# bacpop/PopPUNK

Measured on AMD Instinct MI355X. Metric: genome-pair distances/sec (10k self, s=1024, k=13-29), higher is better.
Workload: dtype u64

## Files before the change

### include/ppk.h

```cpp
#ifndef PPK_H
#define PPK_H

#include <stddef.h>
#include <stdint.h>

#ifdef __cplusplus
extern "C" {
#endif

#define PPK_OK 0
#define PPK_ERR_ARG 1
#define PPK_ERR_HIP 2
#define PPK_ERR_CAPACITY 3
#define PPK_ERR_STATE 4
#define PPK_ERR_INTERRUPTED 5
#define PPK_REFINE_NOT_NESTED 6

#define PPK_FLAG_RANDOM_CORRECT 1
#define PPK_FLAG_JACCARD 2
#define PPK_FLAG_COUNTS 4

const char *ppk_last_error(void);
int ppk_release_scratch(void);
const char *ppk_version(void);
int ppk_device_count(int *n);

int ppk_set_option(const char *name, long long value);
int ppk_get_option(const char *name, long long *value);

int ppk_set_interrupt_check(int (*check)(void));

typedef struct ppk_db ppk_db;

int ppk_db_create(int device_id, const uint64_t *sk, size_t n, size_t nk,
                  size_t sketchsize64, size_t bbits, const uint16_t *clu,
                  int src_on_device, void *stream, ppk_db **out);
void ppk_db_destroy(ppk_db *db);
size_t ppk_db_size(const ppk_db *db);
int ppk_db_rank_planes(const ppk_db *db);
int ppk_db_rank_read(const ppk_db *db, uint64_t *out, size_t words);
int ppk_db_rank_block_planes(const ppk_db *db, uint8_t *out, size_t cap);
int ppk_db_fold_planes(const ppk_db *db);
int ppk_db_fold_block_planes(const ppk_db *db, uint8_t *out, size_t cap);
int ppk_db_fold_read(const ppk_db *db, int which, uint64_t *out, size_t words);
int ppk_db_fold2_planes(const ppk_db *db);
int ppk_db_fold2_block_planes(const ppk_db *db, uint8_t *out, size_t cap);
int ppk_db_fold2_stream_planes(const ppk_db *db, uint8_t *out, size_t cap);
int ppk_db_fold2_position_order(const ppk_db *db, uint32_t *out, size_t cap);
int ppk_db_fold2_read(const ppk_db *db, int which, uint64_t *out, size_t words);
size_t ppk_db_fold2_events(const ppk_db *db, size_t *n_buckets);
int ppk_db_fold2_events_read(const ppk_db *db, uint32_t *off, size_t n_off, uint16_t *ev, size_t n_ev);
size_t ppk_db_rank_counts(const ppk_db *db, uint32_t *out, size_t cap);
unsigned ppk_db_foldh_holders(const ppk_db *db);
int ppk_db_foldh_stream_planes(const ppk_db *db, uint8_t *out, size_t cap);
int ppk_db_foldh_position_order(const ppk_db *db, uint32_t *out, size_t cap);
int ppk_db_foldh_read(const ppk_db *db, int which, uint64_t *out, size_t words);
size_t ppk_db_foldh_entries(const ppk_db *db, size_t *n_buckets);
int ppk_db_foldh_entries_read(const ppk_db *db, uint32_t *off, size_t n_off, uint32_t *ent, size_t n_ent);

size_t ppk_rows_in_band(size_t n_ref, size_t n_qry, size_t q_begin, size_t q_end);
int ppk_band_split(size_t n_ref, size_t n_qry, int n_parts, size_t *bounds);

int ppk_dist_dev(const ppk_db *ref, const ppk_db *qry, const int32_t *kmers,
                 const float *random_tbl, size_t n_clu, int flags,
                 size_t q_begin, size_t q_end, void *d_out,
                 unsigned long long *d_n_failed, void *stream);

int ppk_dist_edges_dev(const ppk_db *ref, const ppk_db *qry, const int32_t *kmers,
                       const float *random_tbl, size_t n_clu, int flags,
                       size_t q_begin, size_t q_end, int slope, float x_max,
                       float y_max, float scale_x, float scale_y, int inclusive,
                       long long *d_edges, size_t cap,
                       unsigned long long *d_n_edges,
                       unsigned long long *d_n_failed, void *stream);

int ppk_dist_pairs_dev(const ppk_db *ref, const ppk_db *qry, const int32_t *kmers, const float *random_tbl,
                       size_t n_clu, int flags, const long long *d_i, const long long *d_j, size_t stride,
                       size_t n_pairs, long long int_offset, void *d_out, unsigned long long *d_n_failed,
                       void *stream);
int ppk_dist_pairs(const ppk_db *ref, const ppk_db *qry, const int32_t *kmers, const float *random_tbl, size_t n_clu,
                   int flags, const long long *i, const long long *j, size_t n_pairs, long long int_offset, void *out,
                   unsigned long long *n_failed);

#define PPK_WINDOW_HANDLE_BYTES 64
int ppk_window_alloc(int device, size_t bytes, void **d_window);
int ppk_window_free(int device, void *d_window);
int ppk_window_export(int device, const void *d_window, unsigned char handle[PPK_WINDOW_HANDLE_BYTES]);
int ppk_window_open(int device, const unsigned char handle[PPK_WINDOW_HANDLE_BYTES], void **d_window);
int ppk_window_close(int device, void *d_window);

int ppk_assign_threshold_dev(const float *d_dist, size_t n_rows, int slope,
                             float x_max, float y_max, float *d_out, void *stream);

int ppk_edge_threshold_dev(const float *d_dist, size_t n_rows, size_t n_ref,
                           int slope, float x_max, float y_max, int inclusive,
                           long long *d_edges, size_t cap,
                           unsigned long long *d_n_edges, void *stream);

int ppk_generate_tuples_dev(const int32_t *d_assign, size_t n_rows, int within_label,
                            int self, size_t num_ref, long long int_offset,
                            long long *d_edges, size_t cap,
                            unsigned long long *d_n_edges, void *stream);

int ppk_generate_all_tuples_dev(size_t num_ref, size_t num_queries, int self, long long int_offset,
                                long long *d_edges, size_t cap, size_t *n_edges, void *stream);

int ppk_qc_edges_dev(const float *d_dist, size_t n_rows, size_t n_ref, int mode, float max_pi,
                     float max_a, long long *d_edges, size_t cap,
                     unsigned long long *d_n_edges, void *stream);

#define PPK_BGMM_MAX_K 16
typedef struct ppk_bgmm {
  int K;
  int within_label;
  int scale_is_f64;
  int n_jitter;
  float scale_f32[2];
  double scale_f64[2];
  double mean[PPK_BGMM_MAX_K][2];
  double chol[PPK_BGMM_MAX_K][3];
  double inv_diag[PPK_BGMM_MAX_K][2];
  double log_const[PPK_BGMM_MAX_K];
  double lin[PPK_BGMM_MAX_K][5];
  int jitter[PPK_BGMM_MAX_K];
} ppk_bgmm;

int ppk_bgmm_prepare(int K, const double *weights, const double *means, const double *covariances,
                     const double *scale, int scale_is_f64, int within_label, ppk_bgmm *out);

int ppk_bgmm_assign_dev(const float *d_dist, size_t n_rows, const ppk_bgmm *model, int32_t *d_labels,
                        float *d_resp, void *stream);

int ppk_bgmm_edges_dev(const float *d_dist, size_t n_rows, size_t n_ref, const ppk_bgmm *model,
                       long long int_offset, long long *d_edges, size_t cap,
                       unsigned long long *d_n_edges, void *stream);

int ppk_dist_bgmm_edges_dev(const ppk_db *ref, const ppk_db *qry, const int32_t *kmers,
                            const float *random_tbl, size_t n_clu, int flags, size_t q_begin, size_t q_end,
                            const ppk_bgmm *model, long long *d_edges, size_t cap,
                            unsigned long long *d_n_edges, unsigned long long *d_n_failed, void *stream);

int ppk_query_bgmm_edges_dbs(const ppk_db *const *refs, const ppk_db *const *qrys, int n_dev,
                             const int32_t *kmers, const float *random_tbl, size_t n_clu, int flags,
                             const ppk_bgmm *model, long long *ij_out, size_t cap, size_t *n_edges,
                             unsigned long long *n_failed);

int ppk_bgmm_assign(const float *dist, size_t n_rows, const ppk_bgmm *model, int device_id, int32_t *labels,
                    float *resp);

#define PPK_BGMM_FIT_STATS 7
#define PPK_BGMM_FIT_MAX_ITER 1024
#define PPK_BGMM_FIT_MAX_INIT 32
#define PPK_BGMM_KMEANS_MAX_ITER 50
typedef struct ppk_bgmm_fit_params {
  int K;
  int max_iter;
  int n_init;
  int reserved;
  double weight_concentration_prior;
  double mean_precision_prior;
  double mean_prior[2];
  double degrees_of_freedom_prior;
  double reg_covar;
  double tol;
} ppk_bgmm_fit_params;
int ppk_bgmm_fit_params_default(int K, ppk_bgmm_fit_params *out);

typedef struct ppk_bgmm_state {
  int K;
  int reserved;
  double weight_conc_a[PPK_BGMM_MAX_K], weight_conc_b[PPK_BGMM_MAX_K];
  double mean_precision[PPK_BGMM_MAX_K];
  double means[PPK_BGMM_MAX_K][2];
  double dof[PPK_BGMM_MAX_K];
  double covariances[PPK_BGMM_MAX_K][4];
  double chol[PPK_BGMM_MAX_K][3];
  double weights[PPK_BGMM_MAX_K];
  double lin[PPK_BGMM_MAX_K][5];
  double log_const[PPK_BGMM_MAX_K];
} ppk_bgmm_state;

typedef struct ppk_bgmm_fit_result {
  ppk_bgmm_state state;
  int n_iter, converged;
  int best_init, n_init_run;
  unsigned long long n_train;
  double lower_bound;
  double cov_prior[4];
  double train_mean[2];
  double init_lower_bound[PPK_BGMM_FIT_MAX_INIT];
  int init_n_iter[PPK_BGMM_FIT_MAX_INIT];
  int kmeans_iter[PPK_BGMM_FIT_MAX_INIT];
  double lower_bounds[PPK_BGMM_FIT_MAX_ITER];
} ppk_bgmm_fit_result;

int ppk_bgmm_fit_struct_sizes(size_t out[3]);

double ppk_bgmm_digamma(double x);

int ppk_bgmm_mstep(const ppk_bgmm_fit_params *params, const double *stats, const double *pivot,
                   const double *cov_prior, ppk_bgmm_state *state_out, double *lower_bound_out);

int ppk_bgmm_stats_dev(const float *d_rows, size_t n_rows, const long long *d_index, size_t n_index,
                       const float *scale, const ppk_bgmm_state *state, double *d_stats, void *stream);

int ppk_bgmm_kmeans_dev(const float *d_rows, size_t n_rows, const long long *d_index, size_t n_index,
// ... 342 lines not shown
```

### poppunk_amd/_lib.py

```python
import ctypes as C
import os

_HERE = os.path.dirname(os.path.abspath(__file__))
SO_PATH = os.environ.get("PPK_LIBRARY") or os.path.join(_HERE, "csrc", "libppk_hip.so")

OK, ERR_ARG, ERR_HIP, ERR_CAPACITY, ERR_STATE, ERR_INTERRUPTED = 0, 1, 2, 3, 4, 5
REFINE_NOT_NESTED = 6
FLAG_RANDOM_CORRECT, FLAG_JACCARD, FLAG_COUNTS = 1, 2, 4
SKETCH_STRAND_PRESERVED = 1
SKETCH_EXACT = 2

_u64p, _f32p, _i32p, _u16p = (C.POINTER(C.c_uint64), C.POINTER(C.c_float), C.POINTER(C.c_int32),
                              C.POINTER(C.c_uint16))
_llp, _ullp, _szp, _intp = (C.POINTER(C.c_longlong), C.POINTER(C.c_ulonglong),
                            C.POINTER(C.c_size_t), C.POINTER(C.c_int))
_vp, _sz = C.c_void_p, C.c_size_t

BGMM_MAX_K = 16


class Bgmm(C.Structure):
    _fields_ = [("K", C.c_int), ("within_label", C.c_int), ("scale_is_f64", C.c_int), ("n_jitter", C.c_int),
                ("scale_f32", C.c_float * 2), ("scale_f64", C.c_double * 2),
                ("mean", (C.c_double * 2) * BGMM_MAX_K), ("chol", (C.c_double * 3) * BGMM_MAX_K),
                ("inv_diag", (C.c_double * 2) * BGMM_MAX_K), ("log_const", C.c_double * BGMM_MAX_K),
                ("lin", (C.c_double * 5) * BGMM_MAX_K),
                ("jitter", C.c_int * BGMM_MAX_K)]


BGMM_FIT_STATS, BGMM_FIT_MAX_ITER, BGMM_FIT_MAX_INIT, BGMM_KMEANS_MAX_ITER = 7, 1024, 32, 50


class BgmmFitParams(C.Structure):
    _fields_ = [("K", C.c_int), ("max_iter", C.c_int), ("n_init", C.c_int), ("reserved", C.c_int),
                ("weight_concentration_prior", C.c_double), ("mean_precision_prior", C.c_double),
                ("mean_prior", C.c_double * 2), ("degrees_of_freedom_prior", C.c_double), ("reg_covar", C.c_double),
                ("tol", C.c_double)]


class BgmmState(C.Structure):
    _fields_ = [("K", C.c_int), ("reserved", C.c_int),
                ("weight_conc_a", C.c_double * BGMM_MAX_K), ("weight_conc_b", C.c_double * BGMM_MAX_K),
                ("mean_precision", C.c_double * BGMM_MAX_K), ("means", (C.c_double * 2) * BGMM_MAX_K),
                ("dof", C.c_double * BGMM_MAX_K), ("covariances", (C.c_double * 4) * BGMM_MAX_K),
                ("chol", (C.c_double * 3) * BGMM_MAX_K), ("weights", C.c_double * BGMM_MAX_K),
                ("lin", (C.c_double * 5) * BGMM_MAX_K), ("log_const", C.c_double * BGMM_MAX_K)]


class BgmmFitResult(C.Structure):
    _fields_ = [("state", BgmmState), ("n_iter", C.c_int), ("converged", C.c_int), ("best_init", C.c_int),
                ("n_init_run", C.c_int), ("n_train", C.c_ulonglong), ("lower_bound", C.c_double),
                ("cov_prior", C.c_double * 4), ("train_mean", C.c_double * 2),
                ("init_lower_bound", C.c_double * BGMM_FIT_MAX_INIT), ("init_n_iter", C.c_int * BGMM_FIT_MAX_INIT),
                ("kmeans_iter", C.c_int * BGMM_FIT_MAX_INIT), ("lower_bounds", C.c_double * BGMM_FIT_MAX_ITER)]


_bgmmp, _f64p = C.POINTER(Bgmm), C.POINTER(C.c_double)
_fitpp, _statep, _fitrp = C.POINTER(BgmmFitParams), C.POINTER(BgmmState), C.POINTER(BgmmFitResult)

SIGNATURES = {
    "ppk_bgmm_prepare": (C.c_int, [C.c_int, _f64p, _f64p, _f64p, _f64p, C.c_int, C.c_int, _bgmmp]),
    "ppk_bgmm_assign_dev": (C.c_int, [_vp, _sz, _bgmmp, _vp, _vp, _vp]),
    "ppk_bgmm_edges_dev": (C.c_int, [_vp, _sz, _sz, _bgmmp, C.c_longlong, _vp, _sz, _vp, _vp]),
    "ppk_dist_bgmm_edges_dev": (C.c_int, [_vp, _vp, _i32p, _f32p, _sz, C.c_int, _sz, _sz, _bgmmp, _vp, _sz, _vp, _vp,
                                          _vp]),
    "ppk_query_bgmm_edges_dbs": (C.c_int, [C.POINTER(_vp), C.POINTER(_vp), C.c_int, _i32p, _f32p, _sz, C.c_int,
                                           _bgmmp, _llp, _sz, _szp, _ullp]),
    "ppk_bgmm_assign": (C.c_int, [_f32p, _sz, _bgmmp, C.c_int, _i32p, _f32p]),
    "ppk_bgmm_fit_params_default": (C.c_int, [C.c_int, _fitpp]),
    "ppk_bgmm_fit_struct_sizes": (C.c_int, [_szp]),
    "ppk_bgmm_digamma": (C.c_double, [C.c_double]),
    "ppk_bgmm_mstep": (C.c_int, [_fitpp, _f64p, _f64p, _f64p, _statep, _f64p]),
    "ppk_bgmm_stats_dev": (C.c_int, [_vp, _sz, _vp, _sz, _f32p, _statep, _vp, _vp]),
    "ppk_bgmm_kmeans_dev": (C.c_int, [_vp, _sz, _vp, _sz, _f32p, C.c_int, _f64p, _vp, _vp, _vp, _vp]),
    "ppk_bgmm_fit_dev": (C.c_int, [_vp, _sz, _vp, _sz, _f32p, _vp, _f64p, _fitpp, _fitrp, _vp]),
    "ppk_bgmm_fit": (C.c_int, [_f32p, _sz, _llp, _sz, _f32p, _i32p, _f64p, _fitpp, C.c_int, _fitrp]),
    "ppk_network_sweep_dev": (C.c_int, [_vp, _vp, _sz, _vp, _sz, _sz, _sz, C.c_longlong, _vp, _vp, _vp]),
    "ppk_network_sweep": (C.c_int, [_llp, _llp, _llp, _sz, _sz, _sz, C.c_int, C.c_longlong, _llp, _i32p]),
    "ppk_network_summary_dev": (C.c_int, [_vp, _vp, _sz, _vp, _sz, _sz, _sz, C.c_longlong, _vp, _vp, _vp, _vp, _vp]),
    "ppk_network_summary": (C.c_int, [_llp, _llp, _llp, _sz, _sz, _sz, C.c_int, C.c_longlong, _llp, _f64p, _llp, _f64p]),
    "ppk_cluster_sweep_dev": (C.c_int, [_vp, _vp, _sz, _vp, _sz, _sz, _sz, _vp, _vp, _vp]),
    "ppk_cluster_sweep": (C.c_int, [_llp, _llp, _llp, _sz, _sz, _sz, C.c_int, _i32p, _i32p]),
    "ppk_cluster_pair_sums_dev": (C.c_int, [_vp, _sz, C.c_int, _vp, _sz, C.c_int, _vp, _vp, _vp]),
    "ppk_cluster_pair_sums": (C.c_int, [_f32p, _sz, C.c_int, _i32p, _sz, C.c_int, C.c_int, _llp, _llp]),
    "ppk_silhouette_dev": (C.c_int, [_vp, _sz, C.c_int, _vp, _sz, C.c_int, _vp, _vp, _vp, _vp, _vp, _vp]),
    "ppk_silhouette": (C.c_int, [_f32p, _sz, C.c_int, _i32p, _sz, C.c_int, C.c_int, _f64p, _f64p, _f64p, _i32p,
                                 _i32p]),
    "ppk_contingency_sums_dev": (C.c_int, [_vp, _sz, _vp, _sz, _sz, _vp, _vp, _vp, _vp, _vp, _vp, _vp]),
    "ppk_contingency_sums": (C.c_int, [_i32p, _sz, _i32p, _sz, _sz, C.c_int, _llp, _llp, _i32p, _i32p, _llp, _llp]),
    "ppk_strain_knn_dev": (C.c_int, [_vp, _sz, C.c_int, _vp, _llp, _sz, _sz, _vp, _vp, _vp, _vp]),
    "ppk_strain_ranks_dev": (C.c_int, [_vp, _vp, _llp, _sz, _sz, _i32p, _sz, C.c_int, C.c_int, C.c_float, _vp, _vp, _vp,
                                       _vp, _vp, _sz, _szp, _vp]),
    "ppk_strain_knn": (C.c_int, [_f32p, _sz, C.c_int, _llp, _llp, _sz, _sz, C.c_int, _llp, _llp, _f32p]),
    "ppk_strain_ranks": (C.c_int, [_llp, _f32p, _llp, _sz, _sz, _i32p, _sz, C.c_int, C.c_int, C.c_float, C.c_int, _i32p,
                                   _llp, _llp, _llp, _f32p, _sz, _szp]),
    "ppk_strain_extend_dev": (C.c_int, [_vp, _llp, _vp, _llp, _sz, _vp, _vp, _vp, _vp, _sz, _sz, C.c_int, C.c_float,
                                        _sz, _vp, _vp, _vp, _vp]),
    "ppk_strain_extend": (C.c_int, [_llp, _llp, _llp, _llp, _sz, _llp, _f32p, _f32p, _f32p, _sz, _sz, C.c_int,
                                    C.c_float, _sz, C.c_int, _llp, _llp, _f32p]),
    "ppk_sketch_dev": (C.c_int, [_vp, _vp, _sz, _i32p, _sz, _sz, _sz, C.c_int, _vp, _vp, _vp, _vp]),
    "ppk_sketch": (C.c_int, [C.POINTER(C.c_uint8), _llp, _sz, _i32p, _sz, _sz, _sz, C.c_int, C.c_int, _u64p, _llp, _i32p]),
    "ppk_sketch_reads_dev": (C.c_int, [_vp, _vp, _sz, _i32p, _sz, _sz, _sz, C.c_int, C.c_int, _vp, _vp, _vp, _vp, _vp]),
    "ppk_sketch_reads": (C.c_int, [C.POINTER(C.c_uint8), _llp, _sz, _i32p, _sz, _sz, _sz, C.c_int, C.c_int, C.c_int, _u64p,
                                   _llp, _llp, _i32p]),
    "ppk_density_kde_dev": (C.c_int, [_vp, _sz, _vp, _sz, _f32p, _f64p, _sz, _f64p, _sz, C.c_double, C.c_int, _vp, _f32p,
                                      _vp]),
    "ppk_density_kde": (C.c_int, [_f32p, _sz, _llp, _sz, _f32p, _f64p, _sz, _f64p, _sz, C.c_double, C.c_int, C.c_int,
                                  _llp, _f32p]),
    "ppk_density_counts_dev": (C.c_int, [_vp, _sz, _vp, C.c_int, C.c_int, C.c_double, C.c_double, _sz, C.c_double,
                                         C.c_double, _sz, _vp, _vp, _vp]),
    "ppk_density_counts": (C.c_int, [_f32p, _sz, _i32p, C.c_int, C.c_int, C.c_double, C.c_double, _sz, C.c_double,
                                     C.c_double, _sz, C.c_int, C.POINTER(C.c_uint32), _llp]),
    "ppk_query_links_dev": (C.c_int, [_vp, _vp, _sz, _sz, _vp, _sz, _sz, C.c_int, _vp, _vp, _vp, _vp]),
    "ppk_query_links": (C.c_int, [_llp, _llp, _sz, _i32p, _sz, _sz, C.c_int, C.c_int, _i32p, _i32p, _i32p]),
    "ppk_cluster_extend_dev": (C.c_int, [_vp, _vp, _sz, _sz, _vp, _sz, _sz, _vp, _vp, _vp]),
    "ppk_cluster_extend": (C.c_int, [_llp, _llp, _sz, _i32p, _sz, _sz, C.c_int, _i32p, _i32p]),
    "ppk_mst_dev": (C.c_int, [_vp, _vp, _sz, _vp, _sz, _sz, _vp, _vp, _vp, _vp]),
    "ppk_mst": (C.c_int, [_llp, _llp, _f32p, _sz, _sz, C.c_int, _llp, _ullp, _i32p]),
    "ppk_edge_weights_dev": (C.c_int, [_vp, _sz, _vp, _vp, _sz, _sz, _sz, C.c_longlong, C.c_int, _vp, _vp]),
    "ppk_row_norms_dev": (C.c_int, [_vp, _sz, _vp, _vp]),
    "ppk_nj_dev": (C.c_int, [_vp, C.c_int, _sz, _sz, _sz, _vp, _vp, _vp]),
    "ppk_nj": (C.c_int, [_f32p, _sz, C.c_int, _llp, _f64p]),
    "ppk_embed_weights_dev": (C.c_int, [_vp, _vp, _vp, _sz, _sz, C.c_double, _vp, _vp, _vp]),
    "ppk_embed_dev": (C.c_int, [_vp, _vp, _vp, _sz, _sz, C.c_ulonglong, C.c_longlong, C.c_int, C.c_double,
                                C.c_longlong, _vp, _vp]),
    "ppk_embed": (C.c_int, [_llp, _llp, _f32p, _sz, _sz, C.c_double, C.c_ulonglong, C.c_longlong, C.c_int,
                            C.c_double, C.c_longlong, C.c_int, _f64p, _f64p]),
    "ppk_dbscan_core_dev": (C.c_int, [_vp, _sz, C.c_int, _vp, _vp]),
    "ppk_dbscan_mst_dev": (C.c_int, [_vp, _vp, _sz, _vp, _vp, _vp, _vp]),
    "ppk_dbscan_fit": (C.c_int, [_f32p, _sz, C.c_int, C.c_int, _f64p, _i32p, _i32p, _f64p]),
    "ppk_dbscan_create": (C.c_int, [_f32p, _f64p, _sz, C.c_int, _i32p, _f64p, _i32p, _f64p, _i32p, _sz, _f64p,
                                    C.c_int, C.c_int, C.c_int, C.POINTER(_vp)]),
    "ppk_dbscan_destroy": (None, [_vp]),
    "ppk_dbscan_assign_dev": (C.c_int, [_vp, _sz, _vp, _vp, _vp]),
    "ppk_dbscan_edges_dev": (C.c_int, [_vp, _sz, _sz, _vp, C.c_longlong, _vp, _sz, _vp, _vp]),
    "ppk_dbscan_assign": (C.c_int, [_f32p, _sz, _vp, _i32p]),
    "ppk_dbscan_stats": (C.c_int, [_vp, _ullp]),
    "ppk_refine_score_dev": (C.c_int, [_vp, _sz, C.c_int, C.c_float, C.c_float, _vp, _vp]),
    "ppk_refine_score": (C.c_int, [_f32p, _sz, C.c_int, C.c_float, C.c_float, C.c_int, _llp]),
    "ppk_refine_local_create_dev": (C.c_int, [_vp, _sz, C.c_int, C.c_float, C.c_float, C.c_float, C.c_float, _vp,
                                              C.POINTER(_vp)]),
    "ppk_refine_local_destroy": (None, [_vp]),
    "ppk_refine_local_stats": (C.c_int, [_vp, _ullp]),
    "ppk_refine_local_eval_dev": (C.c_int, [_vp, C.c_float, C.c_float, _vp, _vp]),
    "ppk_last_error": (C.c_char_p, []),
    "ppk_version": (C.c_char_p, []),
    "ppk_release_scratch": (C.c_int, []),
    "ppk_device_count": (C.c_int, [_intp]),
    "ppk_db_create": (C.c_int, [C.c_int, _vp, _sz, _sz, _sz, _sz, _vp, C.c_int, _vp,
                                C.POINTER(_vp)]),
    "ppk_db_destroy": (None, [_vp]),
    "ppk_db_size": (_sz, [_vp]),
    "ppk_db_rank_planes": (C.c_int, [_vp]),
    "ppk_db_rank_read": (C.c_int, [_vp, _vp, _sz]),
    "ppk_db_rank_block_planes": (C.c_int, [_vp, _vp, _sz]),
    "ppk_db_fold_planes": (C.c_int, [_vp]),
    "ppk_db_fold_block_planes": (C.c_int, [_vp, _vp, _sz]),
    "ppk_db_fold_read": (C.c_int, [_vp, C.c_int, _vp, _sz]),
    "ppk_db_fold2_planes": (C.c_int, [_vp]),
    "ppk_db_fold2_block_planes": (C.c_int, [_vp, _vp, _sz]),
    "ppk_db_fold2_stream_planes": (C.c_int, [_vp, _vp, _sz]),
    "ppk_db_fold2_position_order": (C.c_int, [_vp, _vp, _sz]),
    "ppk_db_fold2_read": (C.c_int, [_vp, C.c_int, _vp, _sz]),
    "ppk_db_fold2_events": (_sz, [_vp, C.POINTER(C.c_size_t)]),
    "ppk_db_fold2_events_read": (C.c_int, [_vp, _vp, _sz, _vp, _sz]),
    "ppk_db_rank_counts": (_sz, [_vp, _vp, _sz]),
    "ppk_db_foldh_holders": (C.c_uint, [_vp]),
    "ppk_db_foldh_stream_planes": (C.c_int, [_vp, _vp, _sz]),
    "ppk_db_foldh_position_order": (C.c_int, [_vp, _vp, _sz]),
    "ppk_db_foldh_read": (C.c_int, [_vp, C.c_int, _vp, _sz]),
    "ppk_db_foldh_entries": (_sz, [_vp, C.POINTER(C.c_size_t)]),
    "ppk_db_foldh_entries_read": (C.c_int, [_vp, _vp, _sz, _vp, _sz]),
    "ppk_rows_in_band": (_sz, [_sz, _sz, _sz, _sz]),
    "ppk_band_split": (C.c_int, [_sz, _sz, C.c_int, _szp]),
    "ppk_dist_dev": (C.c_int, [_vp, _vp, _i32p, _f32p, _sz, C.c_int, _sz, _sz, _vp, _vp, _vp]),
    "ppk_dist_pairs_dev": (C.c_int, [_vp, _vp, _i32p, _f32p, _sz, C.c_int, _vp, _vp, _sz, _sz, C.c_longlong, _vp, _vp,
                                     _vp]),
    "ppk_dist_pairs": (C.c_int, [_vp, _vp, _i32p, _f32p, _sz, C.c_int, _llp, _llp, _sz, C.c_longlong, _vp, _ullp]),
    "ppk_dist_edges_dev": (C.c_int, [_vp, _vp, _i32p, _f32p, _sz, C.c_int, _sz, _sz, C.c_int,
                                     C.c_float, C.c_float, C.c_float, C.c_float, C.c_int, _vp,
                                     _sz, _vp, _vp, _vp]),
    "ppk_assign_threshold_dev": (C.c_int, [_vp, _sz, C.c_int, C.c_float, C.c_float, _vp, _vp]),
    "ppk_edge_threshold_dev": (C.c_int, [_vp, _sz, _sz, C.c_int, C.c_float, C.c_float, C.c_int,
                                         _vp, _sz, _vp, _vp]),
    "ppk_generate_tuples_dev": (C.c_int, [_vp, _sz, C.c_int, C.c_int, _sz, C.c_longlong, _vp,
                                          _sz, _vp, _vp]),
    "ppk_query": (C.c_int, [_u64p, _sz, _u64p, _sz, _i32p, _sz, _sz, _sz, _f32p, _u16p, _u16p,
                            _sz, C.c_int, _intp, C.c_int, _vp, _ullp]),
    "ppk_assign_threshold": (C.c_int, [_f32p, _sz, C.c_int, C.c_float, C.c_float, C.c_int,
                                       _f32p]),
    "ppk_edge_threshold": (C.c_int, [_f32p, _sz, _sz, C.c_int, C.c_float, C.c_float, C.c_int,
                                     C.c_int, _llp, _sz, _szp]),
    "ppk_generate_tuples": (C.c_int, [_i32p, _sz, C.c_int, C.c_int, _sz, C.c_longlong, C.c_int,
                                      _llp, _sz, _szp]),
    "ppk_threshold_iterate_1d_dev": (C.c_int, [_vp, _sz, C.POINTER(C.c_double), _sz, C.c_int,
                                               C.c_float, C.c_float, C.c_float, C.c_float, _vp,
                                               _vp, _vp, _sz, _vp, _vp]),
    "ppk_threshold_iterate_2d_dev": (C.c_int, [_vp, _sz, _f32p, _sz, C.c_float, _vp, _vp, _vp,
                                               _sz, _vp, _vp]),
    "ppk_threshold_iterate_1d": (C.c_int, [_f32p, _sz, C.POINTER(C.c_double), _sz, C.c_int,
                                           C.c_float, C.c_float, C.c_float, C.c_float, C.c_int,
                                           _llp, _llp, _llp, _sz, _szp]),
    "ppk_threshold_iterate_2d": (C.c_int, [_f32p, _sz, _f32p, _sz, C.c_float, C.c_int, _llp,
                                           _llp, _llp, _sz, _szp]),
    "ppk_long_to_square_dev": (C.c_int, [_vp, _sz, _sz, _sz, _vp, _vp]),
    "ppk_long_to_square_multi_dev": (C.c_int, [_vp, _vp, _vp, _sz, _sz, _sz, _sz, _vp, _vp]),
    "ppk_square_to_long_dev": (C.c_int, [_vp, _sz, _vp, _vp]),
    "ppk_knn_dev": (C.c_int, [_vp, _sz, C.c_int, _vp, _vp, _vp, _vp]),
    "ppk_knn_rect_dev": (C.c_int, [_vp, _sz, _sz, _sz, _sz, _sz, C.c_int, _vp, _vp, _vp, _vp]),
    "ppk_knn_sketches_dev": (C.c_int, [_vp, _i32p, _f32p, _sz, C.c_int, C.c_int, C.c_int, _vp, _vp, _vp,
                                       _ullp, _vp]),
    "ppk_knn_candidates_dev": (C.c_int, [_vp, _i32p, _f32p, _sz, C.c_int, C.c_int, C.c_int, _sz, _sz, _vp, _vp,
                                         _sz, _ullp, _vp]),
    "ppk_knn_select_dev": (C.c_int, [_vp, _vp, _sz, _sz, C.c_int, _vp, _vp, _vp, _vp]),
    "ppk_prune_long_dev": (C.c_int, [_vp, _sz, _sz, _vp, _sz, _vp, _vp]),
    "ppk_prune_query_rows_dev": (C.c_int, [_vp, _sz, _sz, _vp, _sz, _vp, _vp]),
    "ppk_prune_long": (C.c_int, [_f32p, _sz, _sz, _llp, _sz, C.c_int, _f32p]),
    "ppk_long_to_square": (C.c_int, [_f32p, _sz, C.c_int, _f32p]),
    "ppk_long_to_square_multi": (C.c_int, [_f32p, _f32p, _f32p, _sz, _sz, C.c_int, _f32p]),
    "ppk_long_to_square2": (C.c_int, [_f32p, _f32p, _f32p, _sz, _sz, C.c_int, _f32p, _f32p]),
    "ppk_square_to_long": (C.c_int, [_f32p, _sz, C.c_int, _f32p]),
    "ppk_knn": (C.c_int, [_f32p, _sz, C.c_int, C.c_int, _llp, _llp, _f32p]),
    "ppk_qc_edges_dev": (C.c_int, [_vp, _sz, _sz, C.c_int, C.c_float, C.c_float, _vp, _sz, _vp, _vp]),
    "ppk_window_alloc": (C.c_int, [C.c_int, _sz, C.POINTER(C.c_void_p)]),
    "ppk_window_free": (C.c_int, [C.c_int, _vp]),
    "ppk_window_export": (C.c_int, [C.c_int, _vp, C.c_char_p]),
    "ppk_window_open": (C.c_int, [C.c_int, C.c_char_p, C.POINTER(C.c_void_p)]),
    "ppk_window_close": (C.c_int, [C.c_int, _vp]),
    "ppk_prof_enable": (C.c_int, [C.c_int]),
    "ppk_prof_read": (C.c_int, [C.POINTER(C.c_double), _llp, C.c_int]),
    "ppk_choose_route": (C.c_int, [C.c_size_t, C.c_size_t, C.c_int, C.c_int, C.c_int, C.c_int, C.c_int, C.c_int, C.c_int,
                                   C.c_int, C.c_int, C.POINTER(C.c_longlong), C.POINTER(C.c_int), C.POINTER(C.c_int),
                                   C.POINTER(C.c_size_t), C.POINTER(C.c_size_t)]),
    "ppk_choose_coding": (C.c_int, [_vp, _sz, _sz, _sz, _sz, _sz, C.c_int, C.POINTER(C.c_longlong), C.POINTER(C.c_int),
                                    C.POINTER(C.c_int), C.POINTER(C.c_size_t), _vp, _vp, _vp, C.POINTER(C.c_size_t),
                                    C.POINTER(C.c_int)]),
    "ppk_choose_holder": (C.c_int, [_vp, _sz, _sz, _sz, _sz, C.c_int, _sz, _sz, C.c_longlong, C.c_longlong,
                                    C.POINTER(C.c_uint), _vp, _vp, C.POINTER(C.c_size_t)]),
    "ppk_sweep_plan": (C.c_int, [C.POINTER(C.c_float), C.POINTER(C.c_float), C.c_size_t, C.c_int, C.c_int, C.POINTER(C.c_int)]),
    "ppk_prof_stages_enable": (C.c_int, [C.c_int]),
    "ppk_prof_stages_read": (C.c_int, [C.c_char_p, C.c_size_t, C.c_int]),
    "ppk_last_kernel_name": (C.c_char_p, []),
    "ppk_set_option": (C.c_int, [C.c_char_p, C.c_longlong]),
    "ppk_get_option": (C.c_int, [C.c_char_p, _llp]),
    "ppk_set_interrupt_check": (C.c_int, [_vp]),
    "ppk_query_db": (C.c_int, [_vp, _vp, _i32p, _f32p, _sz, C.c_int, _vp, _ullp]),
    "ppk_query_dbs": (C.c_int, [C.POINTER(_vp), C.POINTER(_vp), C.c_int, _i32p, _f32p, _sz, C.c_int, _vp, _ullp]),
    "ppk_query_last_stats": (C.c_int, [C.POINTER(C.c_double), C.c_int]),
    "ppk_parked_fetch": (C.c_int, [_llp, _llp, _llp, _sz, _szp]),
    "ppk_generate_all_tuples_dev": (C.c_int, [_sz, _sz, C.c_int, C.c_longlong, _vp, _sz, _szp, _vp]),
    "ppk_generate_all_tuples": (C.c_int, [_sz, _sz, C.c_int, C.c_longlong, C.c_int, _llp, _sz, _szp]),
    "ppk_lower_rank": (C.c_int, [_llp, _llp, _f32p, _sz, _sz, _sz, C.c_int, C.c_int, C.c_float, C.c_int, _llp, _llp,
                                 _f32p, _sz, _szp]),
    "ppk_extend": (C.c_int, [_llp, _llp, _f32p, _sz, _f32p, _f32p, _sz, _sz, _sz, C.c_int, _llp, _llp, _f32p, _sz,
                             _szp]),
    "ppk_query_knn_dbs": (C.c_int, [C.POINTER(_vp), C.c_int, _i32p, _f32p, _sz, C.c_int, C.c_int, C.c_int, _llp, _llp,
                                    _f32p]),
    "ppk_query_knn": (C.c_int, [_u64p, _sz, _i32p, _sz, _sz, _sz, _f32p, _u16p, _sz, C.c_int, C.c_int, C.c_int, _intp,
                                C.c_int, _llp, _llp, _f32p]),
    "ppk_knn_sketches_band_dev": (C.c_int, [_vp, _i32p, _f32p, _sz, C.c_int, C.c_int, C.c_int, _sz, _sz, _vp, _vp, _vp, _ullp,
                                            _vp]),
    "ppk_knn_sketches_rq_dev": (C.c_int, [_vp, _vp, _i32p, _f32p, _sz, C.c_int, C.c_int, C.c_int, _vp, _vp, _vp, _ullp, _vp]),
    "ppk_extend_sketches": (C.c_int, [_llp, _llp, _f32p, _sz, _vp, _vp, _i32p, _f32p, _sz, C.c_int, C.c_int, C.c_int, _llp,
                                      _llp, _f32p, _sz, _szp]),
    "ppk_extend_sketches_dbs": (C.c_int, [_llp, _llp, _f32p, _sz, C.POINTER(_vp), C.POINTER(_vp), C.c_int, _i32p, _f32p, _sz,
                                          C.c_int, C.c_int, C.c_int, _llp, _llp, _f32p, _sz, _szp]),
    "ppk_qc_edges": (C.c_int, [_f32p, _sz, _sz, C.c_int, C.c_float, C.c_float, C.c_int, _llp, _sz, _szp, _szp]),
    "ppk_query_edges_dbs": (C.c_int, [C.POINTER(_vp), C.POINTER(_vp), C.c_int, _i32p, _f32p, _sz, C.c_int,
                                      C.c_int, C.c_float, C.c_float, C.c_float, C.c_float, C.c_int, _llp, _sz,
                                      _szp, _ullp]),
    "ppk_query_edges": (C.c_int, [_u64p, _sz, _u64p, _sz, _i32p, _sz, _sz, _sz, _f32p, _u16p, _u16p, _sz,
                                  C.c_int, C.c_int, C.c_float, C.c_float, C.c_float, C.c_float, C.c_int, _intp,
                                  C.c_int, _llp, _sz, _szp, _ullp]),
    "ppk_h5_set_library": (C.c_int, [C.c_char_p]),
    "ppk_h5_open": (C.c_int, [C.c_char_p, C.c_int, C.POINTER(_vp)]),
    "ppk_h5_close": (None, [_vp]),
    "ppk_h5_backend": (C.c_int, [_vp]),
    "ppk_h5_declined": (C.c_char_p, [_vp]),
    "ppk_h5_has_random": (C.c_int, [_vp]),
    "ppk_h5_count": (_sz, [_vp]),
    "ppk_h5_names": (C.c_int, [_vp, _vp, _sz, _szp]),
    "ppk_h5_params": (C.c_int, [_vp, C.c_char_p, _szp, _szp, _llp, _sz, _szp]),
    "ppk_h5_codon_phased": (C.c_int, [_vp]),
    "ppk_h5_all_params": (C.c_int, [_vp, _sz, _llp, _llp, _llp, _sz, _szp]),
    "ppk_h5_read": (C.c_int, [_vp, C.c_char_p, _sz, _i32p, _sz, _sz, _vp, _vp, _vp, _vp, C.c_int]),
}

_lib = None


def _preload_hip_runtime():
    try:
        import importlib.util
        spec = importlib.util.find_spec("torch")
        if spec is None or not spec.origin:
            return
        cand = os.path.join(os.path.dirname(spec.origin), "lib", "libamdhip64.so")
        if os.path.exists(cand):
            C.CDLL(cand, mode=C.RTLD_GLOBAL)
    except Exception:
        pass


def lib():
    global _lib
    if _lib is None:
        if not os.path.exists(SO_PATH):
            raise RuntimeError(
                "poppunk_amd: HIP extension %s not built (run __graft_entry__.build() / "
                "make -C poppunk_amd/csrc); there is no CPU fallback" % SO_PATH)
        _preload_hip_runtime()
        try:
            handle = C.CDLL(SO_PATH)
        except OSError as e:
            raise RuntimeError("poppunk_amd: cannot load %s: %s" % (SO_PATH, e))
        for name, (res, args) in SIGNATURES.items():
            fn = getattr(handle, name)
            fn.restype = res
            fn.argtypes = args
        _lib = handle
# ... 79 lines not shown
```

### poppunk_amd/csrc/ppk_block_asm.inc

```
#define PPK_BLOCK_ASM_Q32 \
  "ds_read_b128 v[80:83], %[qp] offset:0\n" \
  "ds_read_b128 v[84:87], %[qp] offset:16\n" \
  "ds_read_b128 v[72:75], %[rp] offset:0\n" \
  "ds_read_b128 v[76:79], %[rp] offset:1024\n" \
  "ds_read_b128 v[88:91], %[qp] offset:256\n" \
  "ds_read_b128 v[92:95], %[qp] offset:272\n" \
  "s_waitcnt lgkmcnt(3)\n" \
  "v_xnor_b32 v97, v72, v80\n" \
  "v_xnor_b32 v96, v73, v81\n" \
  "v_xnor_b32 v99, v72, v82\n" \
  "v_xnor_b32 v98, v73, v83\n" \
  "v_xnor_b32 v101, v72, v84\n" \
  "v_xnor_b32 v100, v73, v85\n" \
  "v_xnor_b32 v103, v72, v86\n" \
  "v_xnor_b32 v102, v73, v87\n" \
  "v_xnor_b32 v105, v74, v80\n" \
  "v_xnor_b32 v104, v75, v81\n" \
  "v_xnor_b32 v107, v74, v82\n" \
  "v_xnor_b32 v106, v75, v83\n" \
  "v_xnor_b32 v109, v74, v84\n" \
  "v_xnor_b32 v108, v75, v85\n" \
  "v_xnor_b32 v111, v74, v86\n" \
  "v_xnor_b32 v110, v75, v87\n" \
  "ds_read_b128 v[72:75], %[rp] offset:2048\n" \
// ... 5350 lines not shown
  "v_bitop3_b32 v127, v127, v78, v86 bitop3:0x90\n" \
  "v_bitop3_b32 v126, v126, v79, v87 bitop3:0x90\n" \
  "ds_read_b128 v[76:79], %[rp] offset:7168\n" \
  "ds_read_b128 v[80:83], %[qp] offset:1024\n" \
  "ds_read_b128 v[84:87], %[qp] offset:1040\n" \
  "s_waitcnt lgkmcnt(3)\n" \
  "v_bitop3_b32 v97, v97, v72, v88 bitop3:0x90\n" \
  "v_bitop3_b32 v96, v96, v73, v89 bitop3:0x90\n" \
  "v_bitop3_b32 v99, v99, v72, v90 bitop3:0x90\n" \
  "v_bitop3_b32 v98, v98, v73, v91 bitop3:0x90\n" \
  "v_bitop3_b32 v101, v101, v72, v92 bitop3:0x90\n" \
  "v_bitop3_b32 v100, v100, v73, v93 bitop3:0x90\n" \
  "v_bitop3_b32 v103, v103, v72, v94 bitop3:0x90\n" \
  "v_bitop3_b32 v102, v102, v73, v95 bitop3:0x90\n" \
  "v_bitop3_b32 v105, v105, v74, v88 bitop3:0x90\n" \
  "v_bitop3_b32 v104, v104, v75, v89 bitop3:0x90\n" \
  "v_bitop3_b32 v107, v107, v74, v90 bitop3:0x90\n" \
  "v_bitop3_b32 v106, v106, v75, v91 bitop3:0x90\n" \
  "v_bitop3_b32 v109, v109, v74, v92 bitop3:0x90\n" \
  "v_bitop3_b32 v108, v108, v75, v93 bitop3:0x90\n" \
  "v_bitop3_b32 v111, v111, v74, v94 bitop3:0x90\n" \
  "v_bitop3_b32 v110, v110, v75, v95 bitop3:0x90\n" \
  "ds_read_b128 v[72:75], %[rp] offset:8192\n" \
  "s_waitcnt lgkmcnt(3)\n" \
  "v_bitop3_b32 v113, v113, v76, v88 bitop3:0x90\n" \
  "v_bitop3_b32 v112, v112, v77, v89 bitop3:0x90\n" \
  "v_bitop3_b32 v115, v115, v76, v90 bitop3:0x90\n" \
  "v_bitop3_b32 v114, v114, v77, v91 bitop3:0x90\n" \
  "v_bitop3_b32 v117, v117, v76, v92 bitop3:0x90\n" \
  "v_bitop3_b32 v116, v116, v77, v93 bitop3:0x90\n" \
  "v_bitop3_b32 v119, v119, v76, v94 bitop3:0x90\n" \
  "v_bitop3_b32 v118, v118, v77, v95 bitop3:0x90\n" \
  "v_bitop3_b32 v121, v121, v78, v88 bitop3:0x90\n" \
  "v_bitop3_b32 v120, v120, v79, v89 bitop3:0x90\n" \
  "v_bitop3_b32 v123, v123, v78, v90 bitop3:0x90\n" \
  "v_bitop3_b32 v122, v122, v79, v91 bitop3:0x90\n" \
  "v_bitop3_b32 v125, v125, v78, v92 bitop3:0x90\n" \
  "v_bitop3_b32 v124, v124, v79, v93 bitop3:0x90\n" \
  "v_bitop3_b32 v127, v127, v78, v94 bitop3:0x90\n" \
  "v_bitop3_b32 v126, v126, v79, v95 bitop3:0x90\n" \
  "ds_read_b128 v[76:79], %[rp] offset:9216\n" \
  "s_setprio 1\n" \
  "ds_read_b128 v[88:91], %[qp] offset:1280\n" \
  "ds_read_b128 v[92:95], %[qp] offset:1296\n" \
  "s_waitcnt lgkmcnt(3)\n" \
  "v_bitop3_b32 v97, v97, v72, v80 bitop3:0x90\n" \
  "v_bitop3_b32 v96, v96, v73, v81 bitop3:0x90\n" \
  "v_bitop3_b32 v99, v99, v72, v82 bitop3:0x90\n" \
  "v_bitop3_b32 v98, v98, v73, v83 bitop3:0x90\n" \
  "v_bitop3_b32 v101, v101, v72, v84 bitop3:0x90\n" \
  "v_bitop3_b32 v100, v100, v73, v85 bitop3:0x90\n" \
  "v_bitop3_b32 v103, v103, v72, v86 bitop3:0x90\n" \
  "v_bitop3_b32 v102, v102, v73, v87 bitop3:0x90\n" \
  "v_bitop3_b32 v105, v105, v74, v80 bitop3:0x90\n" \
  "v_bitop3_b32 v104, v104, v75, v81 bitop3:0x90\n" \
  "v_bitop3_b32 v107, v107, v74, v82 bitop3:0x90\n" \
  "v_bitop3_b32 v106, v106, v75, v83 bitop3:0x90\n" \
  "v_bitop3_b32 v109, v109, v74, v84 bitop3:0x90\n" \
  "v_bitop3_b32 v108, v108, v75, v85 bitop3:0x90\n" \
  "v_bitop3_b32 v111, v111, v74, v86 bitop3:0x90\n" \
  "v_bitop3_b32 v110, v110, v75, v87 bitop3:0x90\n" \
  "ds_read_b128 v[72:75], %[rp] offset:10240\n" \
  "s_waitcnt lgkmcnt(3)\n" \
  "v_bitop3_b32 v113, v113, v76, v80 bitop3:0x90\n" \
  "v_bitop3_b32 v112, v112, v77, v81 bitop3:0x90\n" \
  "v_bitop3_b32 v115, v115, v76, v82 bitop3:0x90\n" \
  "v_bitop3_b32 v114, v114, v77, v83 bitop3:0x90\n" \
  "v_bitop3_b32 v117, v117, v76, v84 bitop3:0x90\n" \
  "v_bitop3_b32 v116, v116, v77, v85 bitop3:0x90\n" \
  "v_bitop3_b32 v119, v119, v76, v86 bitop3:0x90\n" \
  "v_bitop3_b32 v118, v118, v77, v87 bitop3:0x90\n" \
  "s_mov_b32 m0, %[m03]\n" \
  "s_mov_b32 exec_lo, %[xblo]\n" \
  "s_mov_b32 exec_hi, %[xbhi]\n" \
  "global_load_lds_dwordx4 %[vob], %[sb2]\n" \
  "s_mov_b64 exec, -1\n" \
  "v_bitop3_b32 v121, v121, v78, v80 bitop3:0x90\n" \
  "v_bitop3_b32 v120, v120, v79, v81 bitop3:0x90\n" \
  "v_bitop3_b32 v123, v123, v78, v82 bitop3:0x90\n" \
  "v_bitop3_b32 v122, v122, v79, v83 bitop3:0x90\n" \
  "v_bitop3_b32 v125, v125, v78, v84 bitop3:0x90\n" \
  "v_bitop3_b32 v124, v124, v79, v85 bitop3:0x90\n" \
  "v_bitop3_b32 v127, v127, v78, v86 bitop3:0x90\n" \
  "v_bitop3_b32 v126, v126, v79, v87 bitop3:0x90\n" \
  "ds_read_b128 v[76:79], %[rp] offset:11264\n" \
  "s_waitcnt lgkmcnt(1)\n" \
  "v_bitop3_b32 v97, v97, v72, v88 bitop3:0x90\n" \
  "v_bitop3_b32 v96, v96, v73, v89 bitop3:0x90\n" \
  "v_bitop3_b32 v99, v99, v72, v90 bitop3:0x90\n" \
  "v_bitop3_b32 v98, v98, v73, v91 bitop3:0x90\n" \
  "v_bitop3_b32 v101, v101, v72, v92 bitop3:0x90\n" \
  "v_bitop3_b32 v100, v100, v73, v93 bitop3:0x90\n" \
  "v_bitop3_b32 v103, v103, v72, v94 bitop3:0x90\n" \
  "v_bitop3_b32 v102, v102, v73, v95 bitop3:0x90\n" \
  "v_bitop3_b32 v105, v105, v74, v88 bitop3:0x90\n" \
  "v_bitop3_b32 v104, v104, v75, v89 bitop3:0x90\n" \
  "v_bitop3_b32 v107, v107, v74, v90 bitop3:0x90\n" \
  "v_bitop3_b32 v106, v106, v75, v91 bitop3:0x90\n" \
  "v_bitop3_b32 v109, v109, v74, v92 bitop3:0x90\n" \
  "v_bitop3_b32 v108, v108, v75, v93 bitop3:0x90\n" \
  "v_bitop3_b32 v111, v111, v74, v94 bitop3:0x90\n" \
  "v_bitop3_b32 v110, v110, v75, v95 bitop3:0x90\n" \
  "s_waitcnt lgkmcnt(0)\n" \
  "v_bitop3_b32 v113, v113, v76, v88 bitop3:0x90\n" \
  "v_bitop3_b32 v112, v112, v77, v89 bitop3:0x90\n" \
  "v_bitop3_b32 v115, v115, v76, v90 bitop3:0x90\n" \
  "v_bitop3_b32 v114, v114, v77, v91 bitop3:0x90\n" \
  "v_bitop3_b32 v117, v117, v76, v92 bitop3:0x90\n" \
  "v_bitop3_b32 v116, v116, v77, v93 bitop3:0x90\n" \
  "v_bitop3_b32 v119, v119, v76, v94 bitop3:0x90\n" \
  "v_bitop3_b32 v118, v118, v77, v95 bitop3:0x90\n" \
  "v_bitop3_b32 v121, v121, v78, v88 bitop3:0x90\n" \
  "v_bitop3_b32 v120, v120, v79, v89 bitop3:0x90\n" \
  "v_bitop3_b32 v123, v123, v78, v90 bitop3:0x90\n" \
  "v_bitop3_b32 v122, v122, v79, v91 bitop3:0x90\n" \
  "v_bitop3_b32 v125, v125, v78, v92 bitop3:0x90\n" \
  "v_bitop3_b32 v124, v124, v79, v93 bitop3:0x90\n" \
  "v_bitop3_b32 v127, v127, v78, v94 bitop3:0x90\n" \
  "v_bitop3_b32 v126, v126, v79, v95 bitop3:0x90\n" \
  "v_bcnt_u32_b32 %[c0], v97, %[c0]\n" \
  "v_bcnt_u32_b32 %[c0], v96, %[c0]\n" \
  "v_bcnt_u32_b32 %[c1], v99, %[c1]\n" \
  "v_bcnt_u32_b32 %[c1], v98, %[c1]\n" \
  "v_bcnt_u32_b32 %[c2], v101, %[c2]\n" \
  "v_bcnt_u32_b32 %[c2], v100, %[c2]\n" \
  "v_bcnt_u32_b32 %[c3], v103, %[c3]\n" \
  "v_bcnt_u32_b32 %[c3], v102, %[c3]\n" \
  "v_bcnt_u32_b32 %[c4], v105, %[c4]\n" \
  "v_bcnt_u32_b32 %[c4], v104, %[c4]\n" \
  "v_bcnt_u32_b32 %[c5], v107, %[c5]\n" \
  "v_bcnt_u32_b32 %[c5], v106, %[c5]\n" \
  "v_bcnt_u32_b32 %[c6], v109, %[c6]\n" \
  "v_bcnt_u32_b32 %[c6], v108, %[c6]\n" \
  "v_bcnt_u32_b32 %[c7], v111, %[c7]\n" \
  "v_bcnt_u32_b32 %[c7], v110, %[c7]\n" \
  "v_bcnt_u32_b32 %[c8], v113, %[c8]\n" \
  "v_bcnt_u32_b32 %[c8], v112, %[c8]\n" \
  "v_bcnt_u32_b32 %[c9], v115, %[c9]\n" \
  "v_bcnt_u32_b32 %[c9], v114, %[c9]\n" \
  "v_bcnt_u32_b32 %[c10], v117, %[c10]\n" \
  "v_bcnt_u32_b32 %[c10], v116, %[c10]\n" \
  "v_bcnt_u32_b32 %[c11], v119, %[c11]\n" \
  "v_bcnt_u32_b32 %[c11], v118, %[c11]\n" \
  "v_bcnt_u32_b32 %[c12], v121, %[c12]\n" \
  "v_bcnt_u32_b32 %[c12], v120, %[c12]\n" \
  "v_bcnt_u32_b32 %[c13], v123, %[c13]\n" \
  "v_bcnt_u32_b32 %[c13], v122, %[c13]\n" \
  "v_bcnt_u32_b32 %[c14], v125, %[c14]\n" \
  "v_bcnt_u32_b32 %[c14], v124, %[c14]\n" \
  "v_bcnt_u32_b32 %[c15], v127, %[c15]\n" \
  "v_bcnt_u32_b32 %[c15], v126, %[c15]\n" \
  ".Lppk_done_%=:\n" \
  ""
#define PPK_BLOCK_DMA_SELH_ASM_Q32_P8 \
  "s_bitcmp1_b32 %[sh2], %[bk]\n" \
  "s_cbranch_scc1 .Lppk_two_%=\n" \
  "s_bitcmp1_b32 %[sh], %[bk]\n" \
  "s_cbranch_scc1 .Lppk_three_%=\n" \
  "ds_read_b128 v[80:83], %[qp] offset:0\n" \
  "ds_read_b128 v[84:87], %[qp] offset:16\n" \
  "ds_read_b128 v[72:75], %[rp] offset:0\n" \
  "ds_read_b128 v[76:79], %[rp] offset:1024\n" \
  "s_setprio 3\n" \
  "ds_read_b128 v[88:91], %[qp] offset:256\n" \
  "ds_read_b128 v[92:95], %[qp] offset:272\n" \
  "s_waitcnt lgkmcnt(3)\n" \
  "v_xnor_b32 v97, v72, v80\n" \
  "v_xnor_b32 v96, v73, v81\n" \
  "v_xnor_b32 v99, v72, v82\n" \
  "v_xnor_b32 v98, v73, v83\n" \
  "v_xnor_b32 v101, v72, v84\n" \
  "v_xnor_b32 v100, v73, v85\n" \
  "v_xnor_b32 v103, v72, v86\n" \
  "v_xnor_b32 v102, v73, v87\n" \
  "v_xnor_b32 v105, v74, v80\n" \
  "v_xnor_b32 v104, v75, v81\n" \
  "v_xnor_b32 v107, v74, v82\n" \
  "v_xnor_b32 v106, v75, v83\n" \
  "v_xnor_b32 v109, v74, v84\n" \
  "v_xnor_b32 v108, v75, v85\n" \
  "v_xnor_b32 v111, v74, v86\n" \
  "v_xnor_b32 v110, v75, v87\n" \
  "ds_read_b128 v[72:75], %[rp] offset:2048\n" \
  "s_waitcnt lgkmcnt(3)\n" \
  "v_xnor_b32 v113, v76, v80\n" \
  "v_xnor_b32 v112, v77, v81\n" \
  "v_xnor_b32 v115, v76, v82\n" \
  "v_xnor_b32 v114, v77, v83\n" \
  "v_xnor_b32 v117, v76, v84\n" \
  "v_xnor_b32 v116, v77, v85\n" \
  "v_xnor_b32 v119, v76, v86\n" \
  "v_xnor_b32 v118, v77, v87\n" \
  "v_xnor_b32 v121, v78, v80\n" \
  "v_xnor_b32 v120, v79, v81\n" \
  "v_xnor_b32 v123, v78, v82\n" \
  "v_xnor_b32 v122, v79, v83\n" \
  "v_xnor_b32 v125, v78, v84\n" \
  "v_xnor_b32 v124, v79, v85\n" \
  "v_xnor_b32 v127, v78, v86\n" \
  "v_xnor_b32 v126, v79, v87\n" \
  "ds_read_b128 v[76:79], %[rp] offset:3072\n" \
  "s_setprio 2\n" \
  "ds_read_b128 v[80:83], %[qp] offset:512\n" \
  "ds_read_b128 v[84:87], %[qp] offset:528\n" \
  "s_waitcnt lgkmcnt(3)\n" \
  "v_bitop3_b32 v97, v97, v72, v88 bitop3:0x90\n" \
  "v_bitop3_b32 v96, v96, v73, v89 bitop3:0x90\n" \
  "v_bitop3_b32 v99, v99, v72, v90 bitop3:0x90\n" \
  "v_bitop3_b32 v98, v98, v73, v91 bitop3:0x90\n" \
  "v_bitop3_b32 v101, v101, v72, v92 bitop3:0x90\n" \
  "v_bitop3_b32 v100, v100, v73, v93 bitop3:0x90\n" \
  "v_bitop3_b32 v103, v103, v72, v94 bitop3:0x90\n" \
  "v_bitop3_b32 v102, v102, v73, v95 bitop3:0x90\n" \
  "v_bitop3_b32 v105, v105, v74, v88 bitop3:0x90\n" \
  "v_bitop3_b32 v104, v104, v75, v89 bitop3:0x90\n" \
  "v_bitop3_b32 v107, v107, v74, v90 bitop3:0x90\n" \
  "v_bitop3_b32 v106, v106, v75, v91 bitop3:0x90\n" \
  "v_bitop3_b32 v109, v109, v74, v92 bitop3:0x90\n" \
  "v_bitop3_b32 v108, v108, v75, v93 bitop3:0x90\n" \
  "v_bitop3_b32 v111, v111, v74, v94 bitop3:0x90\n" \
  "v_bitop3_b32 v110, v110, v75, v95 bitop3:0x90\n" \
  "ds_read_b128 v[72:75], %[rp] offset:4096\n" \
  "s_waitcnt lgkmcnt(3)\n" \
  "v_bitop3_b32 v113, v113, v76, v88 bitop3:0x90\n" \
  "v_bitop3_b32 v112, v112, v77, v89 bitop3:0x90\n" \
  "v_bitop3_b32 v115, v115, v76, v90 bitop3:0x90\n" \
  "v_bitop3_b32 v114, v114, v77, v91 bitop3:0x90\n" \
  "v_bitop3_b32 v117, v117, v76, v92 bitop3:0x90\n" \
  "v_bitop3_b32 v116, v116, v77, v93 bitop3:0x90\n" \
  "v_bitop3_b32 v119, v119, v76, v94 bitop3:0x90\n" \
  "v_bitop3_b32 v118, v118, v77, v95 bitop3:0x90\n" \
  "s_mov_b32 m0, %[m00]\n" \
  "s_nop 0\n" \
  "global_load_lds_dwordx4 %[voa], %[sb0]\n" \
  "v_bitop3_b32 v121, v121, v78, v88 bitop3:0x90\n" \
  "v_bitop3_b32 v120, v120, v79, v89 bitop3:0x90\n" \
  "v_bitop3_b32 v123, v123, v78, v90 bitop3:0x90\n" \
  "v_bitop3_b32 v122, v122, v79, v91 bitop3:0x90\n" \
  "v_bitop3_b32 v125, v125, v78, v92 bitop3:0x90\n" \
  "v_bitop3_b32 v124, v124, v79, v93 bitop3:0x90\n" \
  "v_bitop3_b32 v127, v127, v78, v94 bitop3:0x90\n" \
  "v_bitop3_b32 v126, v126, v79, v95 bitop3:0x90\n" \
  "ds_read_b128 v[76:79], %[rp] offset:5120\n" \
  "s_setprio 1\n" \
  "ds_read_b128 v[88:91], %[qp] offset:768\n" \
  "ds_read_b128 v[92:95], %[qp] offset:784\n" \
  "s_waitcnt lgkmcnt(3)\n" \
  "v_bitop3_b32 v97, v97, v72, v80 bitop3:0x90\n" \
  "v_bitop3_b32 v96, v96, v73, v81 bitop3:0x90\n" \
  "v_bitop3_b32 v99, v99, v72, v82 bitop3:0x90\n" \
  "v_bitop3_b32 v98, v98, v73, v83 bitop3:0x90\n" \
  "v_bitop3_b32 v101, v101, v72, v84 bitop3:0x90\n" \
  "v_bitop3_b32 v100, v100, v73, v85 bitop3:0x90\n" \
  "v_bitop3_b32 v103, v103, v72, v86 bitop3:0x90\n" \
  "v_bitop3_b32 v102, v102, v73, v87 bitop3:0x90\n" \
  "v_bitop3_b32 v105, v105, v74, v80 bitop3:0x90\n" \
  "v_bitop3_b32 v104, v104, v75, v81 bitop3:0x90\n" \
  "v_bitop3_b32 v107, v107, v74, v82 bitop3:0x90\n" \
  "v_bitop3_b32 v106, v106, v75, v83 bitop3:0x90\n" \
  "v_bitop3_b32 v109, v109, v74, v84 bitop3:0x90\n" \
  "v_bitop3_b32 v108, v108, v75, v85 bitop3:0x90\n" \
  "v_bitop3_b32 v111, v111, v74, v86 bitop3:0x90\n" \
  "v_bitop3_b32 v110, v110, v75, v87 bitop3:0x90\n" \
  "ds_read_b128 v[72:75], %[rp] offset:6144\n" \
  "s_waitcnt lgkmcnt(3)\n" \
  "v_bitop3_b32 v113, v113, v76, v80 bitop3:0x90\n" \
  "v_bitop3_b32 v112, v112, v77, v81 bitop3:0x90\n" \
  "v_bitop3_b32 v115, v115, v76, v82 bitop3:0x90\n" \
  "v_bitop3_b32 v114, v114, v77, v83 bitop3:0x90\n" \
  "v_bitop3_b32 v117, v117, v76, v84 bitop3:0x90\n" \
  "v_bitop3_b32 v116, v116, v77, v85 bitop3:0x90\n" \
  "v_bitop3_b32 v119, v119, v76, v86 bitop3:0x90\n" \
  "v_bitop3_b32 v118, v118, v77, v87 bitop3:0x90\n" \
  "s_add_u32 m0, %[m00], 8192\n" \
  "s_nop 0\n" \
  "global_load_lds_dwordx4 %[voa], %[sb1]\n" \
  "v_bitop3_b32 v121, v121, v78, v80 bitop3:0x90\n" \
  "v_bitop3_b32 v120, v120, v79, v81 bitop3:0x90\n" \
  "v_bitop3_b32 v123, v123, v78, v82 bitop3:0x90\n" \
  "v_bitop3_b32 v122, v122, v79, v83 bitop3:0x90\n" \
  "v_bitop3_b32 v125, v125, v78, v84 bitop3:0x90\n" \
  "v_bitop3_b32 v124, v124, v79, v85 bitop3:0x90\n" \
  "v_bitop3_b32 v127, v127, v78, v86 bitop3:0x90\n" \
  "v_bitop3_b32 v126, v126, v79, v87 bitop3:0x90\n" \
  "ds_read_b128 v[76:79], %[rp] offset:7168\n" \
  "s_setprio 0\n" \
  "s_waitcnt lgkmcnt(1)\n" \
  "v_bitop3_b32 v97, v97, v72, v88 bitop3:0x90\n" \
  "v_bitop3_b32 v96, v96, v73, v89 bitop3:0x90\n" \
  "v_bitop3_b32 v99, v99, v72, v90 bitop3:0x90\n" \
  "v_bitop3_b32 v98, v98, v73, v91 bitop3:0x90\n" \
  "v_bitop3_b32 v101, v101, v72, v92 bitop3:0x90\n" \
  "v_bitop3_b32 v100, v100, v73, v93 bitop3:0x90\n" \
  "v_bitop3_b32 v103, v103, v72, v94 bitop3:0x90\n" \
  "v_bitop3_b32 v102, v102, v73, v95 bitop3:0x90\n" \
  "v_bitop3_b32 v105, v105, v74, v88 bitop3:0x90\n" \
  "v_bitop3_b32 v104, v104, v75, v89 bitop3:0x90\n" \
  "v_bitop3_b32 v107, v107, v74, v90 bitop3:0x90\n" \
  "v_bitop3_b32 v106, v106, v75, v91 bitop3:0x90\n" \
  "v_bitop3_b32 v109, v109, v74, v92 bitop3:0x90\n" \
  "v_bitop3_b32 v108, v108, v75, v93 bitop3:0x90\n" \
  "v_bitop3_b32 v111, v111, v74, v94 bitop3:0x90\n" \
  "v_bitop3_b32 v110, v110, v75, v95 bitop3:0x90\n" \
  "s_waitcnt lgkmcnt(0)\n" \
  "v_bitop3_b32 v113, v113, v76, v88 bitop3:0x90\n" \
  "v_bitop3_b32 v112, v112, v77, v89 bitop3:0x90\n" \
  "v_bitop3_b32 v115, v115, v76, v90 bitop3:0x90\n" \
  "v_bitop3_b32 v114, v114, v77, v91 bitop3:0x90\n" \
  "v_bitop3_b32 v117, v117, v76, v92 bitop3:0x90\n" \
  "v_bitop3_b32 v116, v116, v77, v93 bitop3:0x90\n" \
  "v_bitop3_b32 v119, v119, v76, v94 bitop3:0x90\n" \
  "v_bitop3_b32 v118, v118, v77, v95 bitop3:0x90\n" \
  "s_mov_b32 m0, %[m03]\n" \
  "s_mov_b32 exec_lo, %[xblo]\n" \
  "s_mov_b32 exec_hi, %[xbhi]\n" \
  "global_load_lds_dwordx4 %[vob], %[sb2]\n" \
  "s_mov_b64 exec, -1\n" \
  "v_bitop3_b32 v121, v121, v78, v88 bitop3:0x90\n" \
  "v_bitop3_b32 v120, v120, v79, v89 bitop3:0x90\n" \
  "v_bitop3_b32 v123, v123, v78, v90 bitop3:0x90\n" \
  "v_bitop3_b32 v122, v122, v79, v91 bitop3:0x90\n" \
  "v_bitop3_b32 v125, v125, v78, v92 bitop3:0x90\n" \
  "v_bitop3_b32 v124, v124, v79, v93 bitop3:0x90\n" \
  "v_bitop3_b32 v127, v127, v78, v94 bitop3:0x90\n" \
  "v_bitop3_b32 v126, v126, v79, v95 bitop3:0x90\n" \
  "v_bcnt_u32_b32 %[c0], v97, %[c0]\n" \
  "v_bcnt_u32_b32 %[c0], v96, %[c0]\n" \
  "v_bcnt_u32_b32 %[c1], v99, %[c1]\n" \
  "v_bcnt_u32_b32 %[c1], v98, %[c1]\n" \
  "v_bcnt_u32_b32 %[c2], v101, %[c2]\n" \
  "v_bcnt_u32_b32 %[c2], v100, %[c2]\n" \
  "v_bcnt_u32_b32 %[c3], v103, %[c3]\n" \
  "v_bcnt_u32_b32 %[c3], v102, %[c3]\n" \
  "v_bcnt_u32_b32 %[c4], v105, %[c4]\n" \
  "v_bcnt_u32_b32 %[c4], v104, %[c4]\n" \
  "v_bcnt_u32_b32 %[c5], v107, %[c5]\n" \
  "v_bcnt_u32_b32 %[c5], v106, %[c5]\n" \
  "v_bcnt_u32_b32 %[c6], v109, %[c6]\n" \
  "v_bcnt_u32_b32 %[c6], v108, %[c6]\n" \
  "v_bcnt_u32_b32 %[c7], v111, %[c7]\n" \
  "v_bcnt_u32_b32 %[c7], v110, %[c7]\n" \
  "v_bcnt_u32_b32 %[c8], v113, %[c8]\n" \
  "v_bcnt_u32_b32 %[c8], v112, %[c8]\n" \
  "v_bcnt_u32_b32 %[c9], v115, %[c9]\n" \
  "v_bcnt_u32_b32 %[c9], v114, %[c9]\n" \
  "v_bcnt_u32_b32 %[c10], v117, %[c10]\n" \
  "v_bcnt_u32_b32 %[c10], v116, %[c10]\n" \
  "v_bcnt_u32_b32 %[c11], v119, %[c11]\n" \
  "v_bcnt_u32_b32 %[c11], v118, %[c11]\n" \
  "v_bcnt_u32_b32 %[c12], v121, %[c12]\n" \
  "v_bcnt_u32_b32 %[c12], v120, %[c12]\n" \
  "v_bcnt_u32_b32 %[c13], v123, %[c13]\n" \
  "v_bcnt_u32_b32 %[c13], v122, %[c13]\n" \
  "v_bcnt_u32_b32 %[c14], v125, %[c14]\n" \
  "v_bcnt_u32_b32 %[c14], v124, %[c14]\n" \
  "v_bcnt_u32_b32 %[c15], v127, %[c15]\n" \
  "v_bcnt_u32_b32 %[c15], v126, %[c15]\n" \
  "s_branch .Lppk_done_%=\n" \
  ".Lppk_three_%=:\n" \
  "ds_read_b128 v[80:83], %[qp] offset:0\n" \
  "ds_read_b128 v[84:87], %[qp] offset:16\n" \
  "ds_read_b128 v[72:75], %[rp] offset:0\n" \
  "ds_read_b128 v[76:79], %[rp] offset:1024\n" \
  "s_setprio 3\n" \
  "ds_read_b128 v[88:91], %[qp] offset:256\n" \
  "ds_read_b128 v[92:95], %[qp] offset:272\n" \
  "s_waitcnt lgkmcnt(3)\n" \
  "v_xnor_b32 v97, v72, v80\n" \
  "v_xnor_b32 v96, v73, v81\n" \
  "v_xnor_b32 v99, v72, v82\n" \
  "v_xnor_b32 v98, v73, v83\n" \
  "v_xnor_b32 v101, v72, v84\n" \
  "v_xnor_b32 v100, v73, v85\n" \
  "v_xnor_b32 v103, v72, v86\n" \
  "v_xnor_b32 v102, v73, v87\n" \
  "v_xnor_b32 v105, v74, v80\n" \
  "v_xnor_b32 v104, v75, v81\n" \
  "v_xnor_b32 v107, v74, v82\n" \
  "v_xnor_b32 v106, v75, v83\n" \
  "v_xnor_b32 v109, v74, v84\n" \
  "v_xnor_b32 v108, v75, v85\n" \
  "v_xnor_b32 v111, v74, v86\n" \
  "v_xnor_b32 v110, v75, v87\n" \
  "ds_read_b128 v[72:75], %[rp] offset:2048\n" \
  "s_waitcnt lgkmcnt(3)\n" \
  "v_xnor_b32 v113, v76, v80\n" \
  "v_xnor_b32 v112, v77, v81\n" \
  "v_xnor_b32 v115, v76, v82\n" \
  "v_xnor_b32 v114, v77, v83\n" \
  "v_xnor_b32 v117, v76, v84\n" \
  "v_xnor_b32 v116, v77, v85\n" \
  "v_xnor_b32 v119, v76, v86\n" \
  "v_xnor_b32 v118, v77, v87\n" \
  "s_mov_b32 m0, %[m00]\n" \
  "s_nop 0\n" \
  "global_load_lds_dwordx4 %[voa], %[sb0]\n" \
  "v_xnor_b32 v121, v78, v80\n" \
  "v_xnor_b32 v120, v79, v81\n" \
  "v_xnor_b32 v123, v78, v82\n" \
  "v_xnor_b32 v122, v79, v83\n" \
  "v_xnor_b32 v125, v78, v84\n" \
  "v_xnor_b32 v124, v79, v85\n" \
  "v_xnor_b32 v127, v78, v86\n" \
  "v_xnor_b32 v126, v79, v87\n" \
  "ds_read_b128 v[76:79], %[rp] offset:3072\n" \
  "s_setprio 2\n" \
  "ds_read_b128 v[80:83], %[qp] offset:512\n" \
  "ds_read_b128 v[84:87], %[qp] offset:528\n" \
  "s_waitcnt lgkmcnt(3)\n" \
  "v_bitop3_b32 v97, v97, v72, v88 bitop3:0x90\n" \
  "v_bitop3_b32 v96, v96, v73, v89 bitop3:0x90\n" \
  "v_bitop3_b32 v99, v99, v72, v90 bitop3:0x90\n" \
  "v_bitop3_b32 v98, v98, v73, v91 bitop3:0x90\n" \
  "v_bitop3_b32 v101, v101, v72, v92 bitop3:0x90\n" \
  "v_bitop3_b32 v100, v100, v73, v93 bitop3:0x90\n" \
  "v_bitop3_b32 v103, v103, v72, v94 bitop3:0x90\n" \
  "v_bitop3_b32 v102, v102, v73, v95 bitop3:0x90\n" \
  "v_bitop3_b32 v105, v105, v74, v88 bitop3:0x90\n" \
  "v_bitop3_b32 v104, v104, v75, v89 bitop3:0x90\n" \
  "v_bitop3_b32 v107, v107, v74, v90 bitop3:0x90\n" \
  "v_bitop3_b32 v106, v106, v75, v91 bitop3:0x90\n" \
  "v_bitop3_b32 v109, v109, v74, v92 bitop3:0x90\n" \
  "v_bitop3_b32 v108, v108, v75, v93 bitop3:0x90\n" \
  "v_bitop3_b32 v111, v111, v74, v94 bitop3:0x90\n" \
  "v_bitop3_b32 v110, v110, v75, v95 bitop3:0x90\n" \
  "ds_read_b128 v[72:75], %[rp] offset:4096\n" \
  "s_waitcnt lgkmcnt(3)\n" \
  "v_bitop3_b32 v113, v113, v76, v88 bitop3:0x90\n" \
  "v_bitop3_b32 v112, v112, v77, v89 bitop3:0x90\n" \
  "v_bitop3_b32 v115, v115, v76, v90 bitop3:0x90\n" \
  "v_bitop3_b32 v114, v114, v77, v91 bitop3:0x90\n" \
  "v_bitop3_b32 v117, v117, v76, v92 bitop3:0x90\n" \
  "v_bitop3_b32 v116, v116, v77, v93 bitop3:0x90\n" \
  "v_bitop3_b32 v119, v119, v76, v94 bitop3:0x90\n" \
  "v_bitop3_b32 v118, v118, v77, v95 bitop3:0x90\n" \
  "s_add_u32 m0, %[m00], 8192\n" \
  "s_nop 0\n" \
  "global_load_lds_dwordx4 %[voa], %[sb1]\n" \
  "v_bitop3_b32 v121, v121, v78, v88 bitop3:0x90\n" \
  "v_bitop3_b32 v120, v120, v79, v89 bitop3:0x90\n" \
  "v_bitop3_b32 v123, v123, v78, v90 bitop3:0x90\n" \
  "v_bitop3_b32 v122, v122, v79, v91 bitop3:0x90\n" \
  "v_bitop3_b32 v125, v125, v78, v92 bitop3:0x90\n" \
  "v_bitop3_b32 v124, v124, v79, v93 bitop3:0x90\n" \
  "v_bitop3_b32 v127, v127, v78, v94 bitop3:0x90\n" \
  "v_bitop3_b32 v126, v126, v79, v95 bitop3:0x90\n" \
  "ds_read_b128 v[76:79], %[rp] offset:5120\n" \
  "s_setprio 1\n" \
  "s_waitcnt lgkmcnt(1)\n" \
  "v_bitop3_b32 v97, v97, v72, v80 bitop3:0x90\n" \
  "v_bitop3_b32 v96, v96, v73, v81 bitop3:0x90\n" \
  "v_bitop3_b32 v99, v99, v72, v82 bitop3:0x90\n" \
  "v_bitop3_b32 v98, v98, v73, v83 bitop3:0x90\n" \
  "v_bitop3_b32 v101, v101, v72, v84 bitop3:0x90\n" \
  "v_bitop3_b32 v100, v100, v73, v85 bitop3:0x90\n" \
  "v_bitop3_b32 v103, v103, v72, v86 bitop3:0x90\n" \
  "v_bitop3_b32 v102, v102, v73, v87 bitop3:0x90\n" \
  "v_bitop3_b32 v105, v105, v74, v80 bitop3:0x90\n" \
  "v_bitop3_b32 v104, v104, v75, v81 bitop3:0x90\n" \
  "v_bitop3_b32 v107, v107, v74, v82 bitop3:0x90\n" \
  "v_bitop3_b32 v106, v106, v75, v83 bitop3:0x90\n" \
  "v_bitop3_b32 v109, v109, v74, v84 bitop3:0x90\n" \
  "v_bitop3_b32 v108, v108, v75, v85 bitop3:0x90\n" \
  "v_bitop3_b32 v111, v111, v74, v86 bitop3:0x90\n" \
  "v_bitop3_b32 v110, v110, v75, v87 bitop3:0x90\n" \
  "s_waitcnt lgkmcnt(0)\n" \
  "v_bitop3_b32 v113, v113, v76, v80 bitop3:0x90\n" \
  "v_bitop3_b32 v112, v112, v77, v81 bitop3:0x90\n" \
  "v_bitop3_b32 v115, v115, v76, v82 bitop3:0x90\n" \
  "v_bitop3_b32 v114, v114, v77, v83 bitop3:0x90\n" \
  "v_bitop3_b32 v117, v117, v76, v84 bitop3:0x90\n" \
  "v_bitop3_b32 v116, v116, v77, v85 bitop3:0x90\n" \
  "v_bitop3_b32 v119, v119, v76, v86 bitop3:0x90\n" \
  "v_bitop3_b32 v118, v118, v77, v87 bitop3:0x90\n" \
  "s_mov_b32 m0, %[m03]\n" \
  "s_mov_b32 exec_lo, %[xblo]\n" \
  "s_mov_b32 exec_hi, %[xbhi]\n" \
  "global_load_lds_dwordx4 %[vob], %[sb2]\n" \
  "s_mov_b64 exec, -1\n" \
  "v_bitop3_b32 v121, v121, v78, v80 bitop3:0x90\n" \
  "v_bitop3_b32 v120, v120, v79, v81 bitop3:0x90\n" \
  "v_bitop3_b32 v123, v123, v78, v82 bitop3:0x90\n" \
  "v_bitop3_b32 v122, v122, v79, v83 bitop3:0x90\n" \
  "v_bitop3_b32 v125, v125, v78, v84 bitop3:0x90\n" \
  "v_bitop3_b32 v124, v124, v79, v85 bitop3:0x90\n" \
  "v_bitop3_b32 v127, v127, v78, v86 bitop3:0x90\n" \
  "v_bitop3_b32 v126, v126, v79, v87 bitop3:0x90\n" \
  "s_setprio 0\n" \
  "v_bcnt_u32_b32 %[c0], v97, %[c0]\n" \
  "v_bcnt_u32_b32 %[c0], v96, %[c0]\n" \
  "v_bcnt_u32_b32 %[c1], v99, %[c1]\n" \
  "v_bcnt_u32_b32 %[c1], v98, %[c1]\n" \
  "v_bcnt_u32_b32 %[c2], v101, %[c2]\n" \
  "v_bcnt_u32_b32 %[c2], v100, %[c2]\n" \
  "v_bcnt_u32_b32 %[c3], v103, %[c3]\n" \
  "v_bcnt_u32_b32 %[c3], v102, %[c3]\n" \
  "v_bcnt_u32_b32 %[c4], v105, %[c4]\n" \
  "v_bcnt_u32_b32 %[c4], v104, %[c4]\n" \
  "v_bcnt_u32_b32 %[c5], v107, %[c5]\n" \
  "v_bcnt_u32_b32 %[c5], v106, %[c5]\n" \
  "v_bcnt_u32_b32 %[c6], v109, %[c6]\n" \
  "v_bcnt_u32_b32 %[c6], v108, %[c6]\n" \
  "v_bcnt_u32_b32 %[c7], v111, %[c7]\n" \
  "v_bcnt_u32_b32 %[c7], v110, %[c7]\n" \
  "v_bcnt_u32_b32 %[c8], v113, %[c8]\n" \
  "v_bcnt_u32_b32 %[c8], v112, %[c8]\n" \
  "v_bcnt_u32_b32 %[c9], v115, %[c9]\n" \
  "v_bcnt_u32_b32 %[c9], v114, %[c9]\n" \
  "v_bcnt_u32_b32 %[c10], v117, %[c10]\n" \
  "v_bcnt_u32_b32 %[c10], v116, %[c10]\n" \
  "v_bcnt_u32_b32 %[c11], v119, %[c11]\n" \
  "v_bcnt_u32_b32 %[c11], v118, %[c11]\n" \
  "v_bcnt_u32_b32 %[c12], v121, %[c12]\n" \
  "v_bcnt_u32_b32 %[c12], v120, %[c12]\n" \
  "v_bcnt_u32_b32 %[c13], v123, %[c13]\n" \
  "v_bcnt_u32_b32 %[c13], v122, %[c13]\n" \
  "v_bcnt_u32_b32 %[c14], v125, %[c14]\n" \
  "v_bcnt_u32_b32 %[c14], v124, %[c14]\n" \
  "v_bcnt_u32_b32 %[c15], v127, %[c15]\n" \
  "v_bcnt_u32_b32 %[c15], v126, %[c15]\n" \
  "s_branch .Lppk_done_%=\n" \
  ".Lppk_two_%=:\n" \
  "ds_read_b128 v[80:83], %[qp] offset:0\n" \
  "ds_read_b128 v[84:87], %[qp] offset:16\n" \
  "ds_read_b128 v[72:75], %[rp] offset:0\n" \
  "ds_read_b128 v[76:79], %[rp] offset:1024\n" \
  "s_setprio 3\n" \
  "ds_read_b128 v[88:91], %[qp] offset:256\n" \
  "ds_read_b128 v[92:95], %[qp] offset:272\n" \
  "s_waitcnt lgkmcnt(3)\n" \
  "v_xnor_b32 v97, v72, v80\n" \
  "v_xnor_b32 v96, v73, v81\n" \
  "v_xnor_b32 v99, v72, v82\n" \
  "v_xnor_b32 v98, v73, v83\n" \
  "v_xnor_b32 v101, v72, v84\n" \
  "v_xnor_b32 v100, v73, v85\n" \
  "v_xnor_b32 v103, v72, v86\n" \
  "v_xnor_b32 v102, v73, v87\n" \
  "v_xnor_b32 v105, v74, v80\n" \
  "v_xnor_b32 v104, v75, v81\n" \
  "v_xnor_b32 v107, v74, v82\n" \
  "v_xnor_b32 v106, v75, v83\n" \
  "v_xnor_b32 v109, v74, v84\n" \
  "v_xnor_b32 v108, v75, v85\n" \
  "v_xnor_b32 v111, v74, v86\n" \
  "v_xnor_b32 v110, v75, v87\n" \
  "ds_read_b128 v[72:75], %[rp] offset:2048\n" \
  "s_waitcnt lgkmcnt(3)\n" \
  "v_xnor_b32 v113, v76, v80\n" \
  "v_xnor_b32 v112, v77, v81\n" \
  "v_xnor_b32 v115, v76, v82\n" \
  "v_xnor_b32 v114, v77, v83\n" \
  "v_xnor_b32 v117, v76, v84\n" \
  "v_xnor_b32 v116, v77, v85\n" \
  "v_xnor_b32 v119, v76, v86\n" \
  "v_xnor_b32 v118, v77, v87\n" \
  "s_mov_b32 m0, %[m00]\n" \
  "s_nop 0\n" \
  "global_load_lds_dwordx4 %[voa], %[sb0]\n" \
  "v_xnor_b32 v121, v78, v80\n" \
  "v_xnor_b32 v120, v79, v81\n" \
  "v_xnor_b32 v123, v78, v82\n" \
  "v_xnor_b32 v122, v79, v83\n" \
  "v_xnor_b32 v125, v78, v84\n" \
  "v_xnor_b32 v124, v79, v85\n" \
  "v_xnor_b32 v127, v78, v86\n" \
  "v_xnor_b32 v126, v79, v87\n" \
  "ds_read_b128 v[76:79], %[rp] offset:3072\n" \
  "s_setprio 2\n" \
  "s_waitcnt lgkmcnt(1)\n" \
  "v_bitop3_b32 v97, v97, v72, v88 bitop3:0x90\n" \
  "v_bitop3_b32 v96, v96, v73, v89 bitop3:0x90\n" \
  "v_bitop3_b32 v99, v99, v72, v90 bitop3:0x90\n" \
  "v_bitop3_b32 v98, v98, v73, v91 bitop3:0x90\n" \
  "v_bitop3_b32 v101, v101, v72, v92 bitop3:0x90\n" \
  "v_bitop3_b32 v100, v100, v73, v93 bitop3:0x90\n" \
  "v_bitop3_b32 v103, v103, v72, v94 bitop3:0x90\n" \
  "v_bitop3_b32 v102, v102, v73, v95 bitop3:0x90\n" \
  "s_add_u32 m0, %[m00], 8192\n" \
  "s_nop 0\n" \
  "global_load_lds_dwordx4 %[voa], %[sb1]\n" \
  "v_bitop3_b32 v105, v105, v74, v88 bitop3:0x90\n" \
  "v_bitop3_b32 v104, v104, v75, v89 bitop3:0x90\n" \
  "v_bitop3_b32 v107, v107, v74, v90 bitop3:0x90\n" \
  "v_bitop3_b32 v106, v106, v75, v91 bitop3:0x90\n" \
  "v_bitop3_b32 v109, v109, v74, v92 bitop3:0x90\n" \
  "v_bitop3_b32 v108, v108, v75, v93 bitop3:0x90\n" \
  "v_bitop3_b32 v111, v111, v74, v94 bitop3:0x90\n" \
  "v_bitop3_b32 v110, v110, v75, v95 bitop3:0x90\n" \
  "s_waitcnt lgkmcnt(0)\n" \
  "v_bitop3_b32 v113, v113, v76, v88 bitop3:0x90\n" \
  "v_bitop3_b32 v112, v112, v77, v89 bitop3:0x90\n" \
  "v_bitop3_b32 v115, v115, v76, v90 bitop3:0x90\n" \
  "v_bitop3_b32 v114, v114, v77, v91 bitop3:0x90\n" \
  "v_bitop3_b32 v117, v117, v76, v92 bitop3:0x90\n" \
  "v_bitop3_b32 v116, v116, v77, v93 bitop3:0x90\n" \
  "v_bitop3_b32 v119, v119, v76, v94 bitop3:0x90\n" \
  "v_bitop3_b32 v118, v118, v77, v95 bitop3:0x90\n" \
  "s_mov_b32 m0, %[m03]\n" \
  "s_mov_b32 exec_lo, %[xblo]\n" \
  "s_mov_b32 exec_hi, %[xbhi]\n" \
  "global_load_lds_dwordx4 %[vob], %[sb2]\n" \
  "s_mov_b64 exec, -1\n" \
  "v_bitop3_b32 v121, v121, v78, v88 bitop3:0x90\n" \
  "v_bitop3_b32 v120, v120, v79, v89 bitop3:0x90\n" \
  "v_bitop3_b32 v123, v123, v78, v90 bitop3:0x90\n" \
  "v_bitop3_b32 v122, v122, v79, v91 bitop3:0x90\n" \
  "v_bitop3_b32 v125, v125, v78, v92 bitop3:0x90\n" \
  "v_bitop3_b32 v124, v124, v79, v93 bitop3:0x90\n" \
  "v_bitop3_b32 v127, v127, v78, v94 bitop3:0x90\n" \
  "v_bitop3_b32 v126, v126, v79, v95 bitop3:0x90\n" \
  "v_bcnt_u32_b32 %[c0], v97, %[c0]\n" \
  "v_bcnt_u32_b32 %[c0], v96, %[c0]\n" \
  "v_bcnt_u32_b32 %[c1], v99, %[c1]\n" \
  "v_bcnt_u32_b32 %[c1], v98, %[c1]\n" \
  "v_bcnt_u32_b32 %[c2], v101, %[c2]\n" \
  "v_bcnt_u32_b32 %[c2], v100, %[c2]\n" \
  "v_bcnt_u32_b32 %[c3], v103, %[c3]\n" \
  "v_bcnt_u32_b32 %[c3], v102, %[c3]\n" \
  "v_bcnt_u32_b32 %[c4], v105, %[c4]\n" \
  "v_bcnt_u32_b32 %[c4], v104, %[c4]\n" \
  "v_bcnt_u32_b32 %[c5], v107, %[c5]\n" \
  "v_bcnt_u32_b32 %[c5], v106, %[c5]\n" \
  "v_bcnt_u32_b32 %[c6], v109, %[c6]\n" \
  "v_bcnt_u32_b32 %[c6], v108, %[c6]\n" \
  "v_bcnt_u32_b32 %[c7], v111, %[c7]\n" \
  "v_bcnt_u32_b32 %[c7], v110, %[c7]\n" \
  "v_bcnt_u32_b32 %[c8], v113, %[c8]\n" \
  "v_bcnt_u32_b32 %[c8], v112, %[c8]\n" \
  "v_bcnt_u32_b32 %[c9], v115, %[c9]\n" \
  "v_bcnt_u32_b32 %[c9], v114, %[c9]\n" \
  "v_bcnt_u32_b32 %[c10], v117, %[c10]\n" \
  "v_bcnt_u32_b32 %[c10], v116, %[c10]\n" \
  "v_bcnt_u32_b32 %[c11], v119, %[c11]\n" \
  "v_bcnt_u32_b32 %[c11], v118, %[c11]\n" \
  "v_bcnt_u32_b32 %[c12], v121, %[c12]\n" \
  "v_bcnt_u32_b32 %[c12], v120, %[c12]\n" \
  "v_bcnt_u32_b32 %[c13], v123, %[c13]\n" \
  "v_bcnt_u32_b32 %[c13], v122, %[c13]\n" \
  "v_bcnt_u32_b32 %[c14], v125, %[c14]\n" \
  "v_bcnt_u32_b32 %[c14], v124, %[c14]\n" \
  "v_bcnt_u32_b32 %[c15], v127, %[c15]\n" \
  "v_bcnt_u32_b32 %[c15], v126, %[c15]\n" \
  ".Lppk_done_%=:\n" \
  ""
#define PPK_BLOCK_HALF_H4_ASM_Q32_P8 \
  "ds_read_b128 v[80:83], %[qp] offset:0\n" \
  "ds_read_b128 v[84:87], %[qp] offset:16\n" \
  "ds_read_b128 v[76:79], %[rp] offset:1024\n" \
  "ds_read_b128 v[88:91], %[qp] offset:256\n" \
  "ds_read_b128 v[92:95], %[qp] offset:272\n" \
  "s_waitcnt lgkmcnt(2)\n" \
  "v_xnor_b32 v113, v76, v80\n" \
  "v_xnor_b32 v112, v77, v81\n" \
  "v_xnor_b32 v115, v76, v82\n" \
  "v_xnor_b32 v114, v77, v83\n" \
  "v_xnor_b32 v117, v76, v84\n" \
  "v_xnor_b32 v116, v77, v85\n" \
  "v_xnor_b32 v119, v76, v86\n" \
  "v_xnor_b32 v118, v77, v87\n" \
  "v_xnor_b32 v121, v78, v80\n" \
  "v_xnor_b32 v120, v79, v81\n" \
  "v_xnor_b32 v123, v78, v82\n" \
  "v_xnor_b32 v122, v79, v83\n" \
  "v_xnor_b32 v125, v78, v84\n" \
  "v_xnor_b32 v124, v79, v85\n" \
  "v_xnor_b32 v127, v78, v86\n" \
  "v_xnor_b32 v126, v79, v87\n" \
  "ds_read_b128 v[76:79], %[rp] offset:3072\n" \
  "ds_read_b128 v[80:83], %[qp] offset:512\n" \
  "ds_read_b128 v[84:87], %[qp] offset:528\n" \
  "s_waitcnt lgkmcnt(2)\n" \
  "v_bitop3_b32 v113, v113, v76, v88 bitop3:0x90\n" \
  "v_bitop3_b32 v112, v112, v77, v89 bitop3:0x90\n" \
  "v_bitop3_b32 v115, v115, v76, v90 bitop3:0x90\n" \
  "v_bitop3_b32 v114, v114, v77, v91 bitop3:0x90\n" \
  "v_bitop3_b32 v117, v117, v76, v92 bitop3:0x90\n" \
  "v_bitop3_b32 v116, v116, v77, v93 bitop3:0x90\n" \
  "v_bitop3_b32 v119, v119, v76, v94 bitop3:0x90\n" \
  "v_bitop3_b32 v118, v118, v77, v95 bitop3:0x90\n" \
  "v_bitop3_b32 v121, v121, v78, v88 bitop3:0x90\n" \
  "v_bitop3_b32 v120, v120, v79, v89 bitop3:0x90\n" \
  "v_bitop3_b32 v123, v123, v78, v90 bitop3:0x90\n" \
  "v_bitop3_b32 v122, v122, v79, v91 bitop3:0x90\n" \
  "v_bitop3_b32 v125, v125, v78, v92 bitop3:0x90\n" \
  "v_bitop3_b32 v124, v124, v79, v93 bitop3:0x90\n" \
  "v_bitop3_b32 v127, v127, v78, v94 bitop3:0x90\n" \
  "v_bitop3_b32 v126, v126, v79, v95 bitop3:0x90\n" \
  "ds_read_b128 v[76:79], %[rp] offset:5120\n" \
  "ds_read_b128 v[88:91], %[qp] offset:768\n" \
  "ds_read_b128 v[92:95], %[qp] offset:784\n" \
  "s_waitcnt lgkmcnt(2)\n" \
  "v_bitop3_b32 v113, v113, v76, v80 bitop3:0x90\n" \
  "v_bitop3_b32 v112, v112, v77, v81 bitop3:0x90\n" \
  "v_bitop3_b32 v115, v115, v76, v82 bitop3:0x90\n" \
  "v_bitop3_b32 v114, v114, v77, v83 bitop3:0x90\n" \
  "v_bitop3_b32 v117, v117, v76, v84 bitop3:0x90\n" \
  "v_bitop3_b32 v116, v116, v77, v85 bitop3:0x90\n" \
  "v_bitop3_b32 v119, v119, v76, v86 bitop3:0x90\n" \
  "v_bitop3_b32 v118, v118, v77, v87 bitop3:0x90\n" \
  "v_bitop3_b32 v121, v121, v78, v80 bitop3:0x90\n" \
  "v_bitop3_b32 v120, v120, v79, v81 bitop3:0x90\n" \
  "v_bitop3_b32 v123, v123, v78, v82 bitop3:0x90\n" \
  "v_bitop3_b32 v122, v122, v79, v83 bitop3:0x90\n" \
  "v_bitop3_b32 v125, v125, v78, v84 bitop3:0x90\n" \
  "v_bitop3_b32 v124, v124, v79, v85 bitop3:0x90\n" \
  "v_bitop3_b32 v127, v127, v78, v86 bitop3:0x90\n" \
  "v_bitop3_b32 v126, v126, v79, v87 bitop3:0x90\n" \
  "ds_read_b128 v[76:79], %[rp] offset:7168\n" \
  "s_waitcnt lgkmcnt(0)\n" \
  "v_bitop3_b32 v113, v113, v76, v88 bitop3:0x90\n" \
  "v_bitop3_b32 v112, v112, v77, v89 bitop3:0x90\n" \
  "v_bitop3_b32 v115, v115, v76, v90 bitop3:0x90\n" \
  "v_bitop3_b32 v114, v114, v77, v91 bitop3:0x90\n" \
  "v_bitop3_b32 v117, v117, v76, v92 bitop3:0x90\n" \
  "v_bitop3_b32 v116, v116, v77, v93 bitop3:0x90\n" \
  "v_bitop3_b32 v119, v119, v76, v94 bitop3:0x90\n" \
  "v_bitop3_b32 v118, v118, v77, v95 bitop3:0x90\n" \
  "v_bitop3_b32 v121, v121, v78, v88 bitop3:0x90\n" \
  "v_bitop3_b32 v120, v120, v79, v89 bitop3:0x90\n" \
  "v_bitop3_b32 v123, v123, v78, v90 bitop3:0x90\n" \
  "v_bitop3_b32 v122, v122, v79, v91 bitop3:0x90\n" \
  "v_bitop3_b32 v125, v125, v78, v92 bitop3:0x90\n" \
  "v_bitop3_b32 v124, v124, v79, v93 bitop3:0x90\n" \
  "v_bitop3_b32 v127, v127, v78, v94 bitop3:0x90\n" \
  "v_bitop3_b32 v126, v126, v79, v95 bitop3:0x90\n" \
  "v_bcnt_u32_b32 %[c8], v113, %[c8]\n" \
  "v_bcnt_u32_b32 %[c8], v112, %[c8]\n" \
  "v_bcnt_u32_b32 %[c9], v115, %[c9]\n" \
  "v_bcnt_u32_b32 %[c9], v114, %[c9]\n" \
  "v_bcnt_u32_b32 %[c10], v117, %[c10]\n" \
  "v_bcnt_u32_b32 %[c10], v116, %[c10]\n" \
  "v_bcnt_u32_b32 %[c11], v119, %[c11]\n" \
  "v_bcnt_u32_b32 %[c11], v118, %[c11]\n" \
  "v_bcnt_u32_b32 %[c12], v121, %[c12]\n" \
  "v_bcnt_u32_b32 %[c12], v120, %[c12]\n" \
  "v_bcnt_u32_b32 %[c13], v123, %[c13]\n" \
  "v_bcnt_u32_b32 %[c13], v122, %[c13]\n" \
  "v_bcnt_u32_b32 %[c14], v125, %[c14]\n" \
  "v_bcnt_u32_b32 %[c14], v124, %[c14]\n" \
  "v_bcnt_u32_b32 %[c15], v127, %[c15]\n" \
  "v_bcnt_u32_b32 %[c15], v126, %[c15]\n" \
  ""
```

### poppunk_amd/csrc/ppk_coding.hip

```cpp
#include <algorithm>

#include "ppk_internal.h"

constexpr int RANK_BMW = (1 << RANK_BB) / 32;
struct Fold2Emit {
  unsigned long long *raw;
  unsigned *count;
  unsigned *bucket;
  unsigned cap, rt;
};
template <bool WRITE, bool FOLD = false, bool FOLD2 = false>
__global__ void __launch_bounds__(256)
rank_code_kernel(const uint64_t *__restrict__ skT, uint8_t *__restrict__ out, uint8_t *__restrict__ out_q,
                 unsigned *__restrict__ max_distinct, size_t n, size_t npad, int s64, int pl, const Fold2Emit ev,
                 uint8_t *__restrict__ bytes = nullptr) {
  static_assert(!FOLD2 || (WRITE && FOLD), "the two-holder pair is a folded pair");
  constexpr bool TWICE = !WRITE || FOLD;
  constexpr bool THRICE = !WRITE || FOLD2;
  constexpr int SLOTS = PPK_FOLD2_SLOTS;
  __shared__ uint32_t bitmap[8][RANK_BMW];
  __shared__ uint32_t twice[TWICE ? 8 : 1][RANK_BMW];
  __shared__ uint32_t thrice[THRICE ? 8 : 1][RANK_BMW];
  __shared__ uint16_t before[WRITE ? 8 : 1][RANK_BMW];
  __shared__ uint16_t before2[FOLD2 ? 8 : 1][RANK_BMW];
// ... 454 lines not shown
  }
  const uint32_t total = part[255];
  if (total == 0) return;
  if (threadIdx.x == 0) {
    base_s = atomicAdd(ev.count, (unsigned long long)total);
    ev.bucket[(size_t)(q0 >> 5) * ev.rt + blockIdx.x] = total;
  }
  __syncthreads();
  unsigned long long at = base_s + (part[threadIdx.x] - mine);
  if (rf < n && mine)
    for (size_t qq = q0; qq < q1 && qq < rf; ++qq) {
      const uint32_t *c = counts + (qq * n - (qq * (qq + 1)) / 2 + (rf - qq - 1) - row_base) * (size_t)nk;
      for (int k = 0; k < nk; ++k)
        if (c[k] != 0) {
          if (at < ev.cap)
            ev.raw[at] = (unsigned long long)rf | ((unsigned long long)qq << 24) | ((unsigned long long)k << 48) |
                         ((unsigned long long)(c[k] & 4095u) << 52);
          ++at;
        }
    }
}
__global__ void __launch_bounds__(256)
foldh_scatter_kernel(const unsigned long long *__restrict__ raw, size_t total, const unsigned *__restrict__ off,
                     unsigned *__restrict__ cursor, uint32_t *__restrict__ ent, unsigned rt) {
  const size_t i = (size_t)blockIdx.x * 256 + threadIdx.x;
  if (i >= total) return;
  const unsigned long long e = raw[i];
  const uint32_t hi = (uint32_t)e & 0xffffffu, lo = (uint32_t)(e >> 24) & 0xffffffu, k = (uint32_t)(e >> 48) & 7u, c = (uint32_t)(e >> 52);
  const size_t b = (size_t)(lo >> 5) * rt + (hi >> 8);
  const unsigned at = off[b] + atomicAdd(cursor + b, 1u);
  if (at < off[b + 1]) ent[at] = (hi & 255u) | ((lo & 31u) << 8) | (k << 13) | (c << 16);
}

int ppk_launch_rank_count(const uint64_t *d_skT, size_t n, size_t npad, size_t nk, size_t s64, unsigned *d_max, hipStream_t s) {
  PPK_HIP(hipMemsetAsync(d_max, 0, (3 * (1 + nk * s64) + PPK_RANK_EXTRA + nk * s64 * 64) * sizeof(unsigned), s));
  hipLaunchKernelGGL((rank_code_kernel<false>), dim3((unsigned)(nk * s64 * 8)), dim3(256), 0, s, d_skT, nullptr, nullptr, d_max,
                     n, npad, (int)s64, 0, Fold2Emit{});
  PPK_HIP(hipGetLastError());
  return PPK_OK;
}
int ppk_launch_rank_codes(const uint64_t *d_skT, uint64_t *d_out, uint64_t *d_out_q, size_t n, size_t npad, size_t nk,
                          size_t s64, int planes, hipStream_t s) {
  const dim3 grid((unsigned)(nk * s64 * 8)), block(256);
  if (d_out_q)
    hipLaunchKernelGGL((rank_code_kernel<true, true>), grid, block, 0, s, d_skT, reinterpret_cast<uint8_t *>(d_out),
                       reinterpret_cast<uint8_t *>(d_out_q), nullptr, n, npad, (int)s64, planes, Fold2Emit{});
  else
    hipLaunchKernelGGL((rank_code_kernel<true, false>), grid, block, 0, s, d_skT, reinterpret_cast<uint8_t *>(d_out), nullptr,
                       nullptr, n, npad, (int)s64, planes, Fold2Emit{});
  PPK_HIP(hipGetLastError());
  return PPK_OK;
}
int ppk_build_fold2(ppk_db *db, int planes, size_t n_two, const std::vector<unsigned> *order, bool *overflow, hipStream_t s) {
  *overflow = false;
  const size_t copy_bytes = db->npad * db->nk * db->s64 * (size_t)planes * sizeof(uint64_t);
  const unsigned qt = (unsigned)(db->npad / 32), rt = (unsigned)(db->npad / 256);
  const size_t nb = (size_t)qt * rt, cap = n_two ? n_two : 1;
  unsigned long long *d_raw = nullptr;
  unsigned *d_cnt = nullptr;
  uint8_t *d_bytes = nullptr;
  unsigned *d_order = nullptr;
  const size_t n_pos = db->nk * db->s64 * 64;
  PpkCoding &c = db->coding[PPK_CODING_FOLD2];
  auto drop = [&]() {
    (void)hipGetLastError();
    ppk_coding_free(c);
  };
  auto done = [&](int rc) {
    if (d_raw) (void)hipFree(d_raw);
    if (d_cnt) (void)hipFree(d_cnt);
    if (d_bytes) (void)hipFree(d_bytes);
    if (d_order) (void)hipFree(d_order);
    return rc;
  };
  hipError_t e = hipMalloc(reinterpret_cast<void **>(&c.d_ref), copy_bytes);
  if (e == hipSuccess) e = hipMalloc(reinterpret_cast<void **>(&c.d_qry), copy_bytes);
  if (e == hipSuccess) e = hipMalloc(reinterpret_cast<void **>(&c.d_list), cap * sizeof(uint16_t));
  if (e == hipSuccess) e = hipMalloc(reinterpret_cast<void **>(&c.d_off), (nb + 1) * sizeof(unsigned));
  if (e == hipSuccess) e = hipMalloc(reinterpret_cast<void **>(&d_raw), cap * sizeof(unsigned long long));
  if (e == hipSuccess) e = hipMalloc(reinterpret_cast<void **>(&d_cnt), (nb + 2) * sizeof(unsigned));
  if (e == hipSuccess) e = hipMemsetAsync(d_cnt, 0, (nb + 2) * sizeof(unsigned), s);
  if (order && order->size() != n_pos) order = nullptr;
  if (e == hipSuccess && order) e = hipMalloc(reinterpret_cast<void **>(&d_bytes), n_pos * db->npad);
  if (e == hipSuccess && order) e = hipMalloc(reinterpret_cast<void **>(&d_order), n_pos * sizeof(unsigned));
  if (e == hipSuccess && order) e = hipMemcpyAsync(d_order, order->data(), n_pos * sizeof(unsigned), hipMemcpyHostToDevice, s);
  if (e != hipSuccess) {
    drop();
    return done(PPK_OK);
  }
  const Fold2Emit ev = {d_raw, d_cnt + nb, d_cnt, (unsigned)cap, rt};
  hipLaunchKernelGGL((rank_code_kernel<true, true, true>), dim3((unsigned)(db->nk * db->s64 * 8)), dim3(256), 0, s, db->d_skT,
                     reinterpret_cast<uint8_t *>(c.d_ref), reinterpret_cast<uint8_t *>(c.d_qry), nullptr, db->n,
                     db->npad, (int)db->s64, planes, ev, d_bytes);
  if (order)
    hipLaunchKernelGGL(fold2_slice_kernel, dim3((unsigned)(db->nk * db->s64 * 8), (unsigned)(db->npad / 256)), dim3(256), 0, s,
                       d_bytes, d_order, reinterpret_cast<uint8_t *>(c.d_ref), reinterpret_cast<uint8_t *>(c.d_qry),
                       db->n, db->npad, (int)db->s64, planes);
  hipLaunchKernelGGL(fold2_scan_kernel, dim3(1), dim3(1024), 0, s, d_cnt, c.d_off, nb);
  hipLaunchKernelGGL(fold2_scatter_kernel, dim3((unsigned)((cap + 255) / 256)), dim3(256), 0, s, d_raw, d_cnt + nb, (unsigned)cap,
                     c.d_off, d_cnt, static_cast<uint16_t *>(c.d_list), rt);
  hipLaunchKernelGGL(fold2_check_kernel, dim3((unsigned)nb), dim3(256), 0, s, static_cast<const uint16_t *>(c.d_list), c.d_off, d_cnt + nb + 1);
  unsigned tail[2] = {0, 0};
  e = hipGetLastError();
  if (e == hipSuccess) e = hipMemcpyAsync(tail, d_cnt + nb, sizeof(tail), hipMemcpyDeviceToHost, s);
  if (e == hipSuccess) e = hipStreamSynchronize(s);
  if (e != hipSuccess) {
    drop();
    return done(ppk_fail(PPK_ERR_HIP, std::string("two-holder pair: ") + hipGetErrorString(e)));
  }
  if (tail[1] || tail[0] != n_two) {
    *overflow = true;
    drop();
    return done(PPK_OK);
  }
  c.planes = c.stream_planes = planes;
  c.list_elem = sizeof(uint16_t);
  c.qt = qt;
  c.rt = rt;
  c.list_count = n_two;
  return done(PPK_OK);
}
int ppk_foldh_count(const ppk_db *db, const unsigned *ladder, unsigned **d_twice, uint16_t **d_holders, std::vector<unsigned> *pos_e,
                    hipStream_t s) {
  const size_t n_pos = db->nk * db->s64 * 64;
  unsigned *d_e = nullptr;
  *d_twice = nullptr;
  *d_holders = nullptr;
  pos_e->assign(n_pos * PPK_FOLDH_LADDER, 0u);
  hipError_t e = hipMalloc(reinterpret_cast<void **>(d_twice), n_pos * RANK_BMW * sizeof(unsigned));
  if (e == hipSuccess) e = hipMalloc(reinterpret_cast<void **>(d_holders), n_pos * PPK_FOLDH_SLOTS * sizeof(uint16_t));
  if (e == hipSuccess) e = hipMalloc(reinterpret_cast<void **>(&d_e), pos_e->size() * sizeof(unsigned));
  if (e == hipSuccess) {
    FoldhLadder l;
    for (int i = 0; i < PPK_FOLDH_LADDER; ++i) l.h[i] = ladder[i];
    hipLaunchKernelGGL(foldh_count_kernel, dim3((unsigned)(db->nk * db->s64 * 8)), dim3(256), 0, s, db->d_skT, *d_twice, *d_holders,
                       d_e, db->n, db->npad, l);
    e = hipGetLastError();
  }
  if (e == hipSuccess) e = hipMemcpyAsync(pos_e->data(), d_e, pos_e->size() * sizeof(unsigned), hipMemcpyDeviceToHost, s);
  if (e == hipSuccess) e = hipStreamSynchronize(s);
  if (d_e) (void)hipFree(d_e);
  if (e != hipSuccess) {
    (void)hipGetLastError();
    if (*d_twice) (void)hipFree(*d_twice);
    if (*d_holders) (void)hipFree(*d_holders);
    *d_twice = nullptr;
    *d_holders = nullptr;
    pos_e->clear();
  }
  return PPK_OK;
}
int ppk_build_foldh(ppk_db *db, unsigned H, const unsigned *d_twice, const uint16_t *d_holders, size_t max_entries, hipStream_t s) {
  const size_t n = db->n, npad = db->npad, n_pos = db->nk * db->s64 * 64, n_kb = db->nk * db->s64;
  const size_t copy_bytes = npad * n_kb * 8 * sizeof(uint64_t), tmp_bytes = npad * n_kb * (size_t)RANK_BB * sizeof(uint64_t);
  const unsigned qt = (unsigned)(npad / 32), rt = (unsigned)(npad / 256);
  const size_t nb = (size_t)qt * rt, cap = max_entries ? max_entries : 1;
  size_t band_q = ((size_t)512 << 20) / (n * db->nk * 4) / 256 * 256;
  if (band_q < 256) band_q = 256;
  if (band_q > ppk_rows_per_dispatch(db)) band_q = ppk_rows_per_dispatch(db);
  const size_t band_rows = ppk_rows_in_band(n, 0, 0, band_q < n ? band_q : n);
  PpkCoding &c = db->coding[PPK_CODING_FOLDH];
  uint8_t *d_kept = nullptr;
  uint16_t *d_owed = nullptr;
  unsigned *d_order = nullptr, *d_cnt = nullptr;
  uint64_t *d_tr = nullptr, *d_tq = nullptr;
  unsigned long long *d_raw = nullptr;
  void *d_band = nullptr;
  auto done = [&](int rc, bool keep) {
    for (void *ptr : {(void *)d_kept, (void *)d_owed, (void *)d_order, (void *)d_cnt, (void *)d_tr, (void *)d_tq, (void *)d_raw, d_band})
      if (ptr) (void)hipFree(ptr);
    if (!keep) {
      (void)hipGetLastError();
      ppk_coding_free(c);
    }
    return rc;
  };
  hipError_t e = hipMalloc(reinterpret_cast<void **>(&c.d_ref), copy_bytes);
  if (e == hipSuccess) e = hipMalloc(reinterpret_cast<void **>(&c.d_qry), copy_bytes);
  if (e == hipSuccess) e = hipMalloc(reinterpret_cast<void **>(&c.d_off), (nb + 1) * sizeof(unsigned));
  if (e == hipSuccess) e = hipMalloc(reinterpret_cast<void **>(&d_kept), n_pos * npad);
  if (e == hipSuccess) e = hipMalloc(reinterpret_cast<void **>(&d_owed), n_pos * npad * sizeof(uint16_t));
  if (e == hipSuccess) e = hipMalloc(reinterpret_cast<void **>(&d_order), n_pos * sizeof(unsigned));
  if (e == hipSuccess) e = hipMalloc(reinterpret_cast<void **>(&d_cnt), (nb + 2) * sizeof(unsigned) + 8);
  if (e == hipSuccess) e = hipMalloc(reinterpret_cast<void **>(&d_tr), tmp_bytes);
  if (e == hipSuccess) e = hipMalloc(reinterpret_cast<void **>(&d_tq), tmp_bytes);
  if (e == hipSuccess) e = hipMalloc(reinterpret_cast<void **>(&d_raw), cap * sizeof(unsigned long long));
  if (e == hipSuccess) e = hipMalloc(&d_band, band_rows * db->nk * 4 + 256);
  if (e == hipSuccess) e = hipMemsetAsync(d_cnt, 0, (nb + 2) * sizeof(unsigned) + 8, s);
  if (e == hipSuccess) e = hipMemcpyAsync(d_order, c.order.data(), n_pos * sizeof(unsigned), hipMemcpyHostToDevice, s);
  if (e != hipSuccess) return done(PPK_OK, false);
  const dim3 grid_pos((unsigned)(n_kb * 8)), grid_slice((unsigned)(n_kb * 8), (unsigned)(npad / 256));
  hipLaunchKernelGGL(foldh_code_kernel, grid_pos, dim3(256), 0, s, db->d_skT, d_twice, d_holders, d_kept, d_owed, n, npad, H);
  hipLaunchKernelGGL(fold2_slice_kernel, grid_slice, dim3(256), 0, s, d_kept, d_order, reinterpret_cast<uint8_t *>(c.d_ref),
                     reinterpret_cast<uint8_t *>(c.d_qry), n, npad, (int)db->s64, 8);
  hipLaunchKernelGGL(foldh_slice14_kernel, grid_slice, dim3(256), 0, s, d_owed, reinterpret_cast<uint8_t *>(d_tr),
                     reinterpret_cast<uint8_t *>(d_tq), n, npad);
  e = hipGetLastError();
  unsigned long long *d_total = reinterpret_cast<unsigned long long *>(d_cnt + ((nb + 2) & ~(size_t)1));
  const FoldhEmit ev = {d_raw, d_total, d_cnt, (unsigned long long)cap, rt};
  for (size_t lo = 0; e == hipSuccess && lo + 1 < n; lo += band_q) {
    const size_t hi = lo + band_q < n ? lo + band_q : n;
    if (ppk_rows_in_band(n, 0, lo, hi) == 0) continue;
    const int rc = ppk_counts_band_raw(db, d_tr, d_tq, lo, hi, d_band, s);
    if (rc != PPK_OK) return done(rc, false);
    hipLaunchKernelGGL(foldh_emit_kernel, dim3((unsigned)((n + 255) / 256), (unsigned)((hi - lo + 31) / 32)), dim3(256), 0, s,
                       static_cast<const uint32_t *>(d_band), n, lo, hi, lo * n - (lo * (lo + 1)) / 2, (int)db->nk, ev);
    e = hipGetLastError();
  }
  unsigned long long total = 0;
  if (e == hipSuccess) e = hipMemcpyAsync(&total, d_total, sizeof(total), hipMemcpyDeviceToHost, s);
  if (e == hipSuccess) e = hipStreamSynchronize(s);
  if (e != hipSuccess) return done(ppk_fail(PPK_ERR_HIP, std::string("holder pair: ") + hipGetErrorString(e)), false);
  if (total > max_entries || total >= ((unsigned long long)1 << 32)) return done(PPK_OK, false);
  e = hipMalloc(reinterpret_cast<void **>(&c.d_list), (total ? total : 1) * sizeof(uint32_t));
  if (e != hipSuccess) return done(PPK_OK, false);
  hipLaunchKernelGGL(fold2_scan_kernel, dim3(1), dim3(1024), 0, s, d_cnt, c.d_off, nb);
  if (total)
    hipLaunchKernelGGL(foldh_scatter_kernel, dim3((unsigned)((total + 255) / 256)), dim3(256), 0, s, d_raw, (size_t)total,
                       c.d_off, d_cnt, static_cast<uint32_t *>(c.d_list), rt);
  e = hipGetLastError();
  if (e == hipSuccess) e = hipStreamSynchronize(s);
  if (e != hipSuccess) return done(ppk_fail(PPK_ERR_HIP, std::string("holder pair: ") + hipGetErrorString(e)), false);
  c.planes = 8;
  c.stream_planes = 4;
  c.holders = H;
  c.list_elem = sizeof(uint32_t);
  c.qt = qt;
  c.rt = rt;
  c.list_count = (size_t)total;
  return done(PPK_OK, true);
}

void ppk_coding_free(PpkCoding &c) {
  for (void *ptr : {(void *)c.d_ref, c.d_qry != c.d_ref ? (void *)c.d_qry : nullptr, c.d_list, (void *)c.d_off})
    if (ptr) (void)hipFree(ptr);
  const PpkCodingKind kind = c.kind;
  c = PpkCoding();
  c.kind = kind;
}

bool ppk_coding_enabled(int kind) {
  const PpkConfig &cfg = ppk_config();
  const std::atomic<long long> *const option[PPK_CODINGS] = {&cfg.rank_planes, &cfg.rank_fold, &cfg.rank_fold2, &cfg.rank_foldh};
  return option[kind]->load() != 0;
}

void ppk_coding_launch_flags(const PpkCoding &c, unsigned *less1, unsigned *less2) {
  const long long min_planes = c.kind == PPK_CODING_FOLD2   ? ppk_config().fold2_min_planes.load()
                               : c.kind == PPK_CODING_FOLDH ? ppk_config().foldh_min_planes.load()
                                                            : 0;
  const bool use1 = ppk_config().rank_short.load() != 0 && !(c.kind == PPK_CODING_FOLDH && min_planes > 3);
  const bool use2 = use1 && min_planes <= c.stream_planes - 2;
  for (int k = 0; k < PPK_RANK_SHORT_WORDS; ++k) {
    less1[k] = use1 ? c.less1[k] : 0u;
    less2[k] = use2 ? c.less2[k] : 0u;
  }
}

static int planes_for(unsigned codes) { return codes <= 256 ? 8 : codes <= 1024 ? 10 : codes <= 4096 ? 12 : 0; }
static bool flags_fit(size_t nk, size_t s64) { return nk < PPK_RANK_SHORT_WORDS && s64 <= 32; }
static size_t short_flags(const unsigned *block_max, int planes, size_t nk, size_t s64, size_t bbits, unsigned *flags) {
  size_t sum = 0;
  for (size_t k = 0; k < nk; ++k)
    for (size_t b = 0; b < s64; ++b) {
      const bool is_short = planes && flags_fit(nk, s64) && block_max[k * s64 + b] <= (1u << (planes - 1));
      if (is_short) flags[k] |= 1u << b;
      sum += planes ? (size_t)(planes - (is_short ? 1 : 0)) : bbits;
    }
  return sum;
}
static void sort_by_span(const unsigned *e, size_t stride, size_t k, size_t nbins, bool sorted, unsigned *ord) {
  for (size_t i = 0; i < nbins; ++i) ord[i] = (unsigned)i;
  if (sorted)
    std::stable_sort(ord, ord + nbins, [&](unsigned a, unsigned b) { return e[(k * nbins + a) * stride] > e[(k * nbins + b) * stride]; });
}
static unsigned widest_of(const unsigned *e, size_t stride, size_t k, size_t nbins, const unsigned *ord, size_t b) {
  unsigned widest = 0;
  for (size_t i = 0; i < 64; ++i) widest = std::max(widest, e[(k * nbins + ord[b * 64 + i]) * stride]);
  return widest;
}
static uint8_t stream_planes_for(unsigned widest, int top) {
  return (uint8_t)(widest <= (1u << (top - 2)) ? top - 2 : widest <= (1u << (top - 1)) ? top - 1 : top);
}
static void stream_flags(const uint8_t *stream, int top, size_t nk, size_t s64, unsigned *less1, unsigned *less2) {
  for (size_t k = 0; k < nk; ++k)
    for (size_t b = 0; b < s64; ++b) {
      if (stream[k * s64 + b] <= top - 1) less1[k] |= 1u << b;
      if (stream[k * s64 + b] <= top - 2) less2[k] |= 1u << b;
    }
}
static bool four_rounds(size_t n, int tile_slots) {
  const size_t npad = (n + PPK_NPAD - 1) / PPK_NPAD * PPK_NPAD;
  return (npad / 256) * (npad / 32) / 2 >= 4 * (size_t)tile_slots;
}

PpkCodingPlan ppk_plan_codings(const unsigned *counts, size_t n, size_t nk, size_t s64, size_t bbits, int tile_slots,
                               long long rank_fold, long long rank_fold2, long long fold2_sort, long long rank_foldh) {
  PpkCodingPlan pl = {};
  const size_t n_blocks = nk * s64, nbins = s64 * 64;
  const unsigned *extra = counts + 3 * (1 + n_blocks), *pos_e2 = extra + PPK_RANK_EXTRA;
  for (int c = 0; c < 3; ++c) {
    const unsigned *figure = counts + c * (1 + n_blocks);
    pl.planes[c] = planes_for(figure[0]);
    pl.sum[c] = short_flags(figure + 1, pl.planes[c], nk, s64, bbits, pl.less1[c]);
  }
  const size_t sum_d = pl.sum[0], sum_e = pl.sum[1], sum_e2 = pl.sum[2];
  const bool fold2_fits = pl.planes[2] == 8 && nk <= PPK_FOLD2_MAX_NK && extra[0] <= PPK_FOLD2_SLOTS && n < ((size_t)1 << 28);
  const bool fold2_pays = rank_fold != 0 && sum_e2 < sum_d && sum_e2 < (pl.planes[1] ? sum_e : (size_t)-1) && four_rounds(n, tile_slots);
  int *next = pl.chain;
  if (fold2_fits && rank_fold2 != 0 && (rank_fold2 == 2 || fold2_pays)) *next++ = PPK_CODING_FOLD2;
  if (pl.planes[1] && rank_fold != 0 && (rank_fold == 2 || sum_e < sum_d)) *next++ = PPK_CODING_FOLD;
  if (pl.planes[0]) *next++ = PPK_CODING_RANK;
  *next = -1;
  if (pl.chain[0] != PPK_CODING_FOLD2) return pl;
  pl.sorted = fold2_sort != 0;
  pl.order.resize(nk * nbins);
  pl.stream.resize(n_blocks);
  for (size_t k = 0; k < nk; ++k) {
    sort_by_span(pos_e2, 1, k, nbins, pl.sorted, pl.order.data() + k * nbins);
    for (size_t b = 0; b < s64; ++b) {
      pl.stream[k * s64 + b] = flags_fit(nk, s64) ? stream_planes_for(widest_of(pos_e2, 1, k, nbins, pl.order.data() + k * nbins, b), 8) : 8;
      pl.stream_sum += pl.stream[k * s64 + b];
    }
  }
  if (flags_fit(nk, s64)) stream_flags(pl.stream.data(), 8, nk, s64, pl.seven, pl.six);
  pl.try_holder = rank_foldh != 0 && flags_fit(nk, s64);
  return pl;
}

int ppk_holder_ladder(size_t n, size_t nk, size_t s64, size_t most_shared, long long foldh_holders, unsigned *ladder) {
  if (nk > PPK_FOLD2_MAX_NK || s64 > 32 || nk >= PPK_RANK_SHORT_WORDS || n >= ((size_t)1 << 24) || most_shared > PPK_FOLDH_SLOTS) return 0;
  for (int i = 0; i < PPK_FOLDH_LADDER; ++i) ladder[i] = 4u << i;
  if (foldh_holders > 0) ladder[0] = (unsigned)(foldh_holders < 65534 ? foldh_holders : 65534);
  return foldh_holders > 0 ? 1 : PPK_FOLDH_LADDER;
}
PpkHolderChoice ppk_choose_holder_impl(const unsigned *pos_e, const unsigned *ladder, int rungs, size_t n, size_t nk, size_t s64,
                                  int tile_slots, size_t fold2_sum, long long rank_foldh) {
  PpkHolderChoice c;
  const size_t nbins = s64 * 64;
  c.order.resize(nk * nbins);
  c.block_planes.resize(nk * s64);
  const bool take_any = rank_foldh == 2;
  for (int i = 0; i < rungs; ++i) {
    bool fits = true;
    size_t sum = 0;
    for (size_t k = 0; k < nk && fits; ++k) {
      unsigned *ord = c.order.data() + k * nbins;
// ... 15 lines not shown
}

extern "C" int ppk_choose_coding(const uint32_t *counts, size_t n_counts, size_t n, size_t nk, size_t sketchsize64, size_t bbits,
                                 int tile_slots, const long long *options, int *first, int *fallback, size_t *plane_sums,
                                 uint32_t *order, uint32_t *flags, uint8_t *stream_planes, size_t *stream_sum, int *try_holder) {
  if (!counts || !options || !first || !fallback || !plane_sums) return ppk_fail(PPK_ERR_ARG, "ppk_choose_coding: NULL argument");
  if (n < 1 || nk < 1 || sketchsize64 < 1 || tile_slots < 1 || n_counts != 3 * (1 + nk * sketchsize64) + PPK_RANK_EXTRA + nk * sketchsize64 * 64)
    return ppk_fail(PPK_ERR_ARG, "ppk_choose_coding: bad shape");
  const PpkCodingPlan pl = ppk_plan_codings(counts, n, nk, sketchsize64, bbits, tile_slots, options[0], options[1], options[2], options[3]);
  *first = pl.chain[0];
  *fallback = pl.chain[0] < 0 ? -1 : pl.chain[1];
  for (int c = 0; c < 3; ++c) plane_sums[c] = pl.sum[c];
  if (order) std::copy(pl.order.begin(), pl.order.end(), order);
  if (stream_planes) std::copy(pl.stream.begin(), pl.stream.end(), stream_planes);
  for (int k = 0; flags && k < PPK_RANK_SHORT_WORDS; ++k) flags[k] = pl.seven[k], flags[PPK_RANK_SHORT_WORDS + k] = pl.six[k];
  if (stream_sum) *stream_sum = pl.stream_sum;
  if (try_holder) *try_holder = pl.try_holder ? 1 : 0;
  return PPK_OK;
}
extern "C" int ppk_choose_holder(const uint32_t *pos_e, size_t n_pos_e, size_t n, size_t nk, size_t sketchsize64, int tile_slots,
                                 size_t most_shared, size_t fold2_sum, long long rank_foldh, long long foldh_holders,
                                 unsigned *holders, uint32_t *order, uint8_t *block_planes, size_t *max_entries) {
  if (!pos_e || !holders) return ppk_fail(PPK_ERR_ARG, "ppk_choose_holder: NULL argument");
  if (n < 1 || nk < 1 || sketchsize64 < 1 || tile_slots < 1 || n_pos_e != nk * sketchsize64 * 64 * PPK_FOLDH_LADDER)
    return ppk_fail(PPK_ERR_ARG, "ppk_choose_holder: bad shape");
  unsigned ladder[PPK_FOLDH_LADDER];
  const int rungs = rank_foldh != 0 ? ppk_holder_ladder(n, nk, sketchsize64, most_shared, foldh_holders, ladder) : 0;
  PpkHolderChoice c;
  if (rungs) c = ppk_choose_holder_impl(pos_e, ladder, rungs, n, nk, sketchsize64, tile_slots, fold2_sum, rank_foldh);
  *holders = c.H;
  if (c.H && order) std::copy(c.order.begin(), c.order.end(), order);
  if (c.H && block_planes) std::copy(c.block_planes.begin(), c.block_planes.end(), block_planes);
  if (max_entries) *max_entries = c.max_entries;
  return PPK_OK;
}

static int build_copies(const ppk_db *db, PpkCoding &c, int planes, hipStream_t s) {
  const size_t bytes = db->npad * db->nk * db->s64 * (size_t)planes * sizeof(uint64_t);
  const bool pair = c.kind == PPK_CODING_FOLD;
  hipError_t e = hipMalloc(reinterpret_cast<void **>(&c.d_ref), bytes);
  if (e == hipSuccess && pair) e = hipMalloc(reinterpret_cast<void **>(&c.d_qry), bytes);
  if (e != hipSuccess) {
    (void)hipGetLastError();
    if (c.d_ref) (void)hipFree(c.d_ref);
    c.d_ref = c.d_qry = nullptr;
    return PPK_OK;
  }
  if (!pair) c.d_qry = c.d_ref;
  return ppk_launch_rank_codes(db->d_skT, c.d_ref, pair ? c.d_qry : nullptr, db->n, db->npad, db->nk, db->s64, planes, s);
}
static int try_holder(ppk_db *db, size_t most_shared, size_t fold2_sum, int tile_slots, hipStream_t s) {
  unsigned ladder[PPK_FOLDH_LADDER];
  const long long opt = ppk_config().rank_foldh.load();
  const int rungs = ppk_holder_ladder(db->n, db->nk, db->s64, most_shared, ppk_config().foldh_holders.load(), ladder);
  if (!rungs) return PPK_OK;
  unsigned *d_twice = nullptr;
  uint16_t *d_holders = nullptr;
  std::vector<unsigned> pos_e;
  int rc = ppk_foldh_count(db, ladder, &d_twice, &d_holders, &pos_e, s);
  if (rc != PPK_OK || pos_e.empty()) return rc;
  PpkHolderChoice choice = ppk_choose_holder_impl(pos_e.data(), ladder, rungs, db->n, db->nk, db->s64, tile_slots, fold2_sum, opt);
  if (choice.H) {
    PpkCoding &c = db->coding[PPK_CODING_FOLDH];
    c.order.swap(choice.order);
    rc = ppk_build_foldh(db, choice.H, d_twice, d_holders, choice.max_entries, s);
    if (rc == PPK_OK && c.planes) stream_flags(choice.block_planes.data(), 4, db->nk, db->s64, c.less1, c.less2);
  }
  (void)hipFree(d_twice);
  (void)hipFree(d_holders);
  return rc;
}

int ppk_db_build_codings(ppk_db *db, hipStream_t s) {
  if (!ppk_coding_enabled(PPK_CODING_RANK) || !ppk_self_job_takes_tiles(db)) return PPK_OK;
  const size_t n_blocks = db->nk * db->s64;
  std::vector<unsigned> counts(3 * (1 + n_blocks) + PPK_RANK_EXTRA + n_blocks * 64, 0u);
  unsigned *d_max = nullptr;
  if (hipMalloc(reinterpret_cast<void **>(&d_max), counts.size() * sizeof(unsigned)) != hipSuccess) {
    (void)hipGetLastError();
    return PPK_OK;
  }
  int rc = ppk_launch_rank_count(db->d_skT, db->n, db->npad, db->nk, db->s64, d_max, s);
  if (rc == PPK_OK) {
    hipError_t e = hipMemcpyAsync(counts.data(), d_max, counts.size() * sizeof(unsigned), hipMemcpyDeviceToHost, s);
    if (e == hipSuccess) e = hipStreamSynchronize(s);
    if (e != hipSuccess) rc = ppk_fail(PPK_ERR_HIP, std::string("rank codes: ") + hipGetErrorString(e));
  }
  (void)hipFree(d_max);
  if (rc != PPK_OK) return rc;
  const PpkConfig &cfg = ppk_config();
  const int tile_slots = ppk_geometry(db->device).tile_slots;
  const PpkCodingPlan plan = ppk_plan_codings(counts.data(), db->n, db->nk, db->s64, db->bbits, tile_slots, cfg.rank_fold.load(),
                                              cfg.rank_fold2.load(), cfg.fold2_sort.load(), cfg.rank_foldh.load());
  unsigned *extra = counts.data() + 3 * (1 + n_blocks);
  bool built = false;
  for (const int *kind = plan.chain; rc == PPK_OK && !built && *kind >= 0; ++kind) {
    PpkCoding &c = db->coding[*kind];
    if (*kind == PPK_CODING_FOLD2) {
      bool overflow = false;
      rc = ppk_build_fold2(db, plan.planes[2], extra[1], plan.sorted ? &plan.order : nullptr, &overflow, s);
      extra[2] = overflow ? 1u : 0u;
      if (rc == PPK_OK && c.planes) {
        c.order = plan.order;
        std::copy(plan.seven, plan.seven + PPK_RANK_SHORT_WORDS, c.less1);
        std::copy(plan.six, plan.six + PPK_RANK_SHORT_WORDS, c.less2);
      }
      if (rc == PPK_OK && plan.try_holder) rc = try_holder(db, counts[1 + n_blocks] - 2u, plan.stream_sum, tile_slots, s);
    } else {
      rc = build_copies(db, c, plan.planes[*kind], s);
      if (*kind == PPK_CODING_FOLD && c.d_ref) {
        c.planes = c.stream_planes = plan.planes[1];
        std::copy(plan.less1[1], plan.less1[1] + PPK_RANK_SHORT_WORDS, c.less1);
      }
    }
    built = c.d_ref != nullptr;
  }
  bool any = false;
  for (const PpkCoding &c : db->coding) any = any || c.d_ref != nullptr;
  if (any) {
    PpkCoding &injective = db->coding[PPK_CODING_RANK];
    injective.planes = injective.stream_planes = plan.planes[0];
    std::copy(plan.less1[0], plan.less1[0] + PPK_RANK_SHORT_WORDS, injective.less1);
  }
  if (rc == PPK_OK) db->rank_counts.assign(counts.begin(), counts.begin() + 3 * (1 + n_blocks) + PPK_RANK_EXTRA);
  return rc;
}

static int ppk_db_build_injective(ppk_db *db) {
  PpkCoding &c = db->coding[PPK_CODING_RANK];
  if (c.d_ref) return PPK_OK;
  int rc = build_copies(db, c, c.planes, nullptr);
  if (rc == PPK_OK && !c.d_ref) return ppk_fail(PPK_ERR_HIP, "rank codes: the device has no room for the copy");
  hipError_t e = rc == PPK_OK ? hipDeviceSynchronize() : hipSuccess;
  if (rc == PPK_OK && e != hipSuccess) rc = ppk_fail(PPK_ERR_HIP, std::string("rank codes: ") + hipGetErrorString(e));
  if (rc != PPK_OK) {
    (void)hipFree(c.d_ref);
    c.d_ref = c.d_qry = nullptr;
  }
  return rc;
}

static const char *const kNoun[PPK_CODINGS] = {"rank-coded copy", "folded pair", "two-holder pair", "holder pair"};
static const char *const kListNoun[PPK_CODINGS] = {"", "", "events (ppk_db_fold2_events)", "entries (ppk_db_foldh_entries)"};
static int fail_in(const char *fn, int code, const std::string &what) { return ppk_fail(code, std::string(fn) + ": " + what); }
static int coding_check(const char *fn, const ppk_db *db, const void *out, int kind, int which = 0) {
  if (!db || !out) return fail_in(fn, PPK_ERR_ARG, "NULL argument");
  if (which != 0 && which != 1) return fail_in(fn, PPK_ERR_ARG, "`which` is 0 (ref side) or 1 (query side)");
  if (!db->coding[kind].planes) return fail_in(fn, PPK_ERR_STATE, std::string("the database has no ") + kNoun[kind]);
  return PPK_OK;
}
static int coding_read(const char *fn, const ppk_db *db, int kind, int which, uint64_t *out, size_t words) {
  if (int rc = coding_check(fn, db, out, kind, which)) return rc;
  const PpkCoding &c = db->coding[kind];
  if (words != db->nk * db->s64 * (size_t)c.planes * db->npad)
    return fail_in(fn, PPK_ERR_ARG, std::string("`words` is not nk * sketchsize64 * ") + (kind == PPK_CODING_FOLDH ? "8" : "planes") + " * padded samples");
  PPK_ENTER_DEVICE(guard, db->device);
  PPK_HIP(hipDeviceSynchronize());
  if (kind == PPK_CODING_RANK)
    if (int rc = ppk_db_build_injective(const_cast<ppk_db *>(db))) return rc;
  PPK_HIP(hipMemcpy(out, which ? c.d_qry : c.d_ref, words * sizeof(uint64_t), hipMemcpyDeviceToHost));
  return PPK_OK;
}
static int coding_block_planes(const char *fn, const ppk_db *db, int kind, uint8_t *out, size_t cap) {
  if (int rc = coding_check(fn, db, out, kind)) return rc;
  if (cap < db->nk * db->s64) return fail_in(fn, PPK_ERR_ARG, "`cap` is below nk * sketchsize64");
  unsigned flags[PPK_RANK_SHORT_WORDS] = {};
  const int planes = db->coding[kind].planes;
  short_flags(db->rank_counts.data() + kind * (1 + db->nk * db->s64) + 1, planes, db->nk, db->s64, db->bbits, flags);
  for (size_t k = 0; k < db->nk; ++k)
    for (size_t b = 0; b < db->s64; ++b) {
      const bool is_short = k < PPK_RANK_SHORT_WORDS && b < 32 && ((flags[k] >> b) & 1u);
      out[k * db->s64 + b] = (uint8_t)(planes - (is_short ? 1 : 0));
    }
  return PPK_OK;
}
static int coding_stream_planes(const char *fn, const ppk_db *db, int kind, uint8_t *out, size_t cap) {
  if (int rc = coding_check(fn, db, out, kind)) return rc;
  if (cap < db->nk * db->s64) return fail_in(fn, PPK_ERR_ARG, "`cap` is below nk * sketchsize64");
  const PpkCoding &c = db->coding[kind];
  unsigned less1[PPK_RANK_SHORT_WORDS], less2[PPK_RANK_SHORT_WORDS];
  ppk_coding_launch_flags(c, less1, less2);
  for (size_t k = 0; k < db->nk; ++k)
    for (size_t b = 0; b < db->s64; ++b) {
      const bool fits = k < PPK_RANK_SHORT_WORDS && b < 32;
      const bool one = fits && ((less1[k] >> b) & 1u), two = fits && ((less2[k] >> b) & 1u);
      out[k * db->s64 + b] = (uint8_t)(c.stream_planes - (two ? 2 : one ? 1 : 0));
    }
  return PPK_OK;
}
static int coding_position_order(const char *fn, const ppk_db *db, int kind, uint32_t *out, size_t cap) {
  if (int rc = coding_check(fn, db, out, kind)) return rc;
  const std::vector<unsigned> &order = db->coding[kind].order;
  if (cap < order.size()) return fail_in(fn, PPK_ERR_ARG, "`cap` is below nk * 64 * sketchsize64");
  std::copy(order.begin(), order.end(), out);
  return PPK_OK;
}
static size_t coding_list_size(const ppk_db *db, int kind, size_t *n_buckets) {
  const PpkCoding *c = db && db->coding[kind].planes ? &db->coding[kind] : nullptr;
  if (n_buckets) *n_buckets = c ? (size_t)c->qt * c->rt : 0;
  return c ? c->list_count : 0;
}
static int coding_list_read(const char *fn, const ppk_db *db, int kind, uint32_t *off, size_t n_off, void *list, size_t n_list) {
  if (int rc = coding_check(fn, db, off, kind)) return rc;
  const PpkCoding &c = db->coding[kind];
  if (n_off != (size_t)c.qt * c.rt + 1 || n_list != c.list_count || (n_list && !list))
    return fail_in(fn, PPK_ERR_ARG, std::string("sizes are buckets + 1 and ") + kListNoun[kind]);
  PPK_ENTER_DEVICE(guard, db->device);
  PPK_HIP(hipDeviceSynchronize());
  PPK_HIP(hipMemcpy(off, c.d_off, n_off * sizeof(uint32_t), hipMemcpyDeviceToHost));
  if (n_list) PPK_HIP(hipMemcpy(list, c.d_list, n_list * c.list_elem, hipMemcpyDeviceToHost));
  return PPK_OK;
}

extern "C" int ppk_db_rank_planes(const ppk_db *db) { return db ? db->coding[PPK_CODING_RANK].planes : 0; }
extern "C" int ppk_db_rank_read(const ppk_db *db, uint64_t *out, size_t words) { return coding_read(__func__, db, PPK_CODING_RANK, 0, out, words); }
extern "C" int ppk_db_rank_block_planes(const ppk_db *db, uint8_t *out, size_t cap) { return coding_block_planes(__func__, db, PPK_CODING_RANK, out, cap); }
extern "C" size_t ppk_db_rank_counts(const ppk_db *db, uint32_t *out, size_t cap) {
  if (!db) return 0;
  if (out && cap >= db->rank_counts.size()) std::copy(db->rank_counts.begin(), db->rank_counts.end(), out);
  return db->rank_counts.size();
}
extern "C" int ppk_db_fold_planes(const ppk_db *db) { return db ? db->coding[PPK_CODING_FOLD].planes : 0; }
extern "C" int ppk_db_fold_read(const ppk_db *db, int which, uint64_t *out, size_t words) { return coding_read(__func__, db, PPK_CODING_FOLD, which, out, words); }
extern "C" int ppk_db_fold_block_planes(const ppk_db *db, uint8_t *out, size_t cap) { return coding_block_planes(__func__, db, PPK_CODING_FOLD, out, cap); }
extern "C" int ppk_db_fold2_planes(const ppk_db *db) { return db ? db->coding[PPK_CODING_FOLD2].planes : 0; }
extern "C" int ppk_db_fold2_read(const ppk_db *db, int which, uint64_t *out, size_t words) { return coding_read(__func__, db, PPK_CODING_FOLD2, which, out, words); }
extern "C" int ppk_db_fold2_block_planes(const ppk_db *db, uint8_t *out, size_t cap) { return coding_block_planes(__func__, db, PPK_CODING_FOLD2, out, cap); }
extern "C" int ppk_db_fold2_stream_planes(const ppk_db *db, uint8_t *out, size_t cap) { return coding_stream_planes(__func__, db, PPK_CODING_FOLD2, out, cap); }
extern "C" int ppk_db_fold2_position_order(const ppk_db *db, uint32_t *out, size_t cap) { return coding_position_order(__func__, db, PPK_CODING_FOLD2, out, cap); }
extern "C" size_t ppk_db_fold2_events(const ppk_db *db, size_t *n_buckets) { return coding_list_size(db, PPK_CODING_FOLD2, n_buckets); }
extern "C" int ppk_db_fold2_events_read(const ppk_db *db, uint32_t *off, size_t n_off, uint16_t *ev, size_t n_ev) {
  return coding_list_read(__func__, db, PPK_CODING_FOLD2, off, n_off, ev, n_ev);
}
extern "C" unsigned ppk_db_foldh_holders(const ppk_db *db) { return db ? db->coding[PPK_CODING_FOLDH].holders : 0u; }
extern "C" int ppk_db_foldh_read(const ppk_db *db, int which, uint64_t *out, size_t words) { return coding_read(__func__, db, PPK_CODING_FOLDH, which, out, words); }
extern "C" int ppk_db_foldh_stream_planes(const ppk_db *db, uint8_t *out, size_t cap) { return coding_stream_planes(__func__, db, PPK_CODING_FOLDH, out, cap); }
extern "C" int ppk_db_foldh_position_order(const ppk_db *db, uint32_t *out, size_t cap) { return coding_position_order(__func__, db, PPK_CODING_FOLDH, out, cap); }
extern "C" size_t ppk_db_foldh_entries(const ppk_db *db, size_t *n_buckets) { return coding_list_size(db, PPK_CODING_FOLDH, n_buckets); }
extern "C" int ppk_db_foldh_entries_read(const ppk_db *db, uint32_t *off, size_t n_off, uint32_t *ent, size_t n_ent) {
  return coding_list_read(__func__, db, PPK_CODING_FOLDH, off, n_off, ent, n_ent);
}
```

### poppunk_amd/csrc/ppk_dist_tile.inc

```
  static_assert(NW == 8, "the product tile is 256 refs x 32 queries (8 wavefronts)");
  static_assert(PL == V2_BB || (PL >= 8 && PL < V2_BB && PL % 2 == 0 && W == 2 && !KSPLIT && !WIDE && !EXP &&
                                (MODE == MODE_DIST || ppk_is_mask(MODE))),
                "rank-coded planes: the two-dword whole-tile kernel only");
  static_assert(!WIDE || (KSPLIT ? (W == 2 && (MODE == MODE_DIST || ppk_is_mask(MODE)))
                                 : (W == 4 && (MODE == MODE_DIST || ppk_is_mask(MODE) || MODE == MODE_KNN))),
                "the wide instantiations");
  constexpr bool WIDE_TILE = WIDE && !KSPLIT;
  const int ablate = EXP ? p.ablate : 0;
  constexpr int R = V2_R, TQ = V2_TQ, BB = V2_BB;
  constexpr int V2_QT = NW * TQ;
  constexpr int REF_U4 = PL * 128;
  constexpr int QRY_U4 = PL * (V2_QT / 2);
  constexpr int CHUNK_U4 = REF_U4 + QRY_U4;
  constexpr int LPP = V2_QT / 2;
  constexpr int PPP = 64 / LPP;
  constexpr int NQP = (PL + PPP - 1) / PPP;
  constexpr int NPIECE = 2 * PL + NQP;
  constexpr int PW = (NPIECE + NW - 1) / NW;
  constexpr bool LDS_TABLE = NW == 8 && W == 2 && !WIDE && (MODE == MODE_DIST || ppk_is_mask(MODE) || MODE == MODE_KNN);
  constexpr int TAB_U4 = 5 * 1024;
  constexpr bool KS_FUSED = KSPLIT && (MODE == MODE_DIST || ppk_is_mask(MODE));
  constexpr bool KS_MEM = KS_FUSED && WIDE;
  constexpr int KS_SLOT = 2 * CHUNK_U4;
  __shared__ u32x4 lds[LDS_TABLE && TAB_U4 > 2 * CHUNK_U4 + 1 ? TAB_U4 : 2 * CHUNK_U4 + (KS_FUSED || WIDE ? 1 : 0)];

  const int lane = threadIdx.x & 63;
  const int wave = __builtin_amdgcn_readfirstlane(threadIdx.x >> 6);
  size_t rt, qt;
  const bool strip = blockIdx.x < p.n_strip;
  size_t qb = p.q_begin, qe = p.q_end, q_tile0 = p.q_tile0;
  if (strip) {
    rt = p.strip_rt0 + blockIdx.x % p.strip_r_tiles;
    qt = blockIdx.x / p.strip_r_tiles;
    qb = p.strip_begin;
    qe = p.n_ref;
    q_tile0 = p.strip_begin / V2_QT;
  } else {
    if (blockIdx.x < p.n_strip_pad) return;
    const unsigned b = blockIdx.x - p.n_strip_pad;
    if (!EXP || p.xcd_map == 0) {
      const unsigned x = b & ((1u << p.xcd_shift) - 1u), j = b >> p.xcd_shift;
      const unsigned g = x * p.tiles_per_xcd + j;
      if (j >= p.tiles_per_xcd || g >= p.n_tiles) return;
      unsigned lo = 0, hi = p.r_tiles - 1;
      while (lo < hi) {
        const unsigned mid = (lo + hi + 1) >> 1;
        if (tiles_before(mid, p.self, p.q_tiles, p.tri_m, p.tri_c0) <= g) lo = mid;
        else hi = mid - 1;
      }
      rt = lo;
      qt = g - tiles_before(lo, p.self, p.q_tiles, p.tri_m, p.tri_c0);
    } else if (p.xcd_map == 1) {
      const unsigned xcd = b & 7u, j = b >> 3;
      if (xcd >= p.r_tiles) return;
      const unsigned nloc = (p.r_tiles - xcd + 7u) >> 3;
      qt = j / nloc;
      rt = xcd + 8u * (j % nloc);
      if (qt >= p.q_tiles) return;
    } else {
      qt = b / p.r_tiles;
      rt = p.self ? (b % p.r_tiles + qt) % p.r_tiles : b % p.r_tiles;
    }
  }
  const size_t r0 = rt * V2_RT;
  const size_t q0 = (q_tile0 + qt) * V2_QT;
  const size_t qw0 = q0 + (size_t)wave * TQ;
  const bool tri = p.self && !strip;
  if (tri && r0 + (V2_RT - 1) <= q0) return;
  const bool half = NW == 8 && tri && q0 >= r0 + 128;
  const bool wave_active = !(tri && r0 + (V2_RT - 1) <= qw0) && qw0 < qe && qw0 + TQ > qb;
  int lane_late = lane;
  auto ref_of = [&](int r) -> size_t { return r0 + 2 * lane_late + (r & 1) + (r >> 1) * 128; };

  if constexpr (WIDE_TILE) {
    if (threadIdx.x == 0) {
      const unsigned mask = p.wide_nslots - 1u;
      unsigned sl = (blockIdx.x * 37u) & mask;
      for (;;) {
        const unsigned bit = 1u << (sl & 31u);
        const unsigned old = __hip_atomic_fetch_or(p.wide_bitmap + (sl >> 5), bit, __ATOMIC_ACQUIRE, __HIP_MEMORY_SCOPE_AGENT);
        if (!(old & bit)) break;
        sl = (sl + 1u) & mask;
        if ((sl & 31u) == 0) __builtin_amdgcn_s_sleep(8);
      }
      u32x4 pos;
      pos.x = sl;
      pos.y = pos.z = pos.w = 0;
      lds[KS_SLOT] = pos;
    }
  }
  const int k_first = KSPLIT ? (int)blockIdx.y : 0;
  const int ublocks = KSPLIT ? p.ks_blocks : p.s64;
  const int total = KSPLIT ? ublocks : p.nk * p.s64;
  if constexpr (KS_FUSED) {
    if (threadIdx.x == 0) {
      u32x4 pos;
      pos.x = blockIdx.x;
      pos.y = blockIdx.y;
      pos.z = pos.w = 0;
      lds[KS_SLOT] = pos;
    }
  }

  const char *dbase[PW];
  size_t dstep[PW];
  int doff[PW];
  int dkind[PW];
#pragma unroll
  for (int t = 0; t < PW; ++t) {
    const int i = wave + NW * t;
    dbase[t] = nullptr;
    dstep[t] = 0;
    doff[t] = 0;
    if (i < 2 * PL) {
      dkind[t] = 0;
      dbase[t] = reinterpret_cast<const char *>(refT + ((size_t)k_first * ublocks * PL + (size_t)(i >> 1)) * p.npad_r + r0 + (i & 1) * 128);
      dstep[t] = (size_t)PL * p.npad_r * 8;
      doff[t] = i * 64;
    } else if (i < NPIECE) {
      const int j = i - 2 * PL;
      dkind[t] = 1;
      dbase[t] = reinterpret_cast<const char *>(qryT + ((size_t)k_first * ublocks * PL + (size_t)(PPP * j)) * p.npad_q + q0);
      dstep[t] = (size_t)PL * p.npad_q * 8;
      doff[t] = REF_U4 + j * 64;
    } else {
      dkind[t] = 2;
    }
  }
  const uint32_t voff_ref = lane * 16;
  const uint32_t voff_qry = (uint32_t)((lane / LPP) * p.npad_q * 8) + (lane % LPP) * 16;
  const bool qlane_ok = (PPP * (NQP - 1) + lane / LPP) < PL;
  auto issue_dma = [&](int buf, bool skip_first_half) {
    u32x4 *base = lds + buf * CHUNK_U4;
#pragma unroll
    for (int t = 0; t < PW; ++t) {
      if (dkind[t] == 0) {
        if (!(skip_first_half && (wave & 1) == 0))
          __builtin_amdgcn_global_load_lds(PPK_GPTR(dbase[t] + voff_ref), PPK_LPTR(base + doff[t]), 16, 0, 0);
      } else if (dkind[t] == 1 && (wave + NW * t != NPIECE - 1 || qlane_ok)) {
        __builtin_amdgcn_global_load_lds(PPK_GPTR(dbase[t] + voff_qry), PPK_LPTR(base + doff[t]), 16, 0, 0);
      }
      dbase[t] += dstep[t];
    }
  };

  using PackT = PackW<W>;
  uint32_t pw[W][R][TQ];
#pragma unroll
  for (int i = 0; i < W; ++i)
#pragma unroll
    for (int r = 0; r < R; ++r)
#pragma unroll
      for (int q = 0; q < TQ; ++q) pw[i][r][q] = 0;

  typedef const __attribute__((address_space(4))) DistParams LateParams;
  auto wide_park = [&](int g) __attribute__((always_inline)) {
    if constexpr (WIDE_TILE) {
      const char __attribute__((address_space(4))) *ka =
          (const char __attribute__((address_space(4))) *)__builtin_amdgcn_kernarg_segment_ptr();
      asm volatile("" : "+s"(ka));
      LateParams &pl = *reinterpret_cast<LateParams *>(ka + V2_PARAMS_KERNARG_OFFSET);
      const uint32_t slot = __builtin_amdgcn_readfirstlane(*(volatile __attribute__((address_space(3))) uint32_t *)(__attribute__((address_space(3))) void *)(lds + KS_SLOT));
      const char *dst = reinterpret_cast<const char *>(pl.wide_slots + ((size_t)slot * (size_t)pl.wide_groups + (size_t)g) * WIDE_GROUP_U64);
      const uint32_t voff = (uint32_t)wave * 256u + (voff_ref >> 2);
#pragma unroll
      for (int q = 0; q < TQ; ++q)
#pragma unroll
        for (int r = 0; r < R; ++r)
#pragma unroll
          for (int i = 0; i < W; ++i) {
            const char *d = dst + (size_t)(((q * R + r) * 4 + i) * 2048);
            asm volatile("global_store_dword %0, %1, %2 sc1" ::"v"(voff), "v"(pw[i][r][q]), "s"(d) : "memory");
          }
    }
  };

  auto rank_short_word = [&](int kk) __attribute__((always_inline)) -> uint32_t {
    const char __attribute__((address_space(4))) *ka =
        (const char __attribute__((address_space(4))) *)__builtin_amdgcn_kernarg_segment_ptr();
    asm volatile("" : "+s"(ka));
    LateParams &pl = *reinterpret_cast<LateParams *>(ka + V2_PARAMS_KERNARG_OFFSET);
    return pl.rank_short[kk];
  };
  auto fold2_six_word = [&](int kk) __attribute__((always_inline)) -> uint32_t {
    const char __attribute__((address_space(4))) *ka =
        (const char __attribute__((address_space(4))) *)__builtin_amdgcn_kernarg_segment_ptr();
    asm volatile("" : "+s"(ka));
    LateParams &pl = *reinterpret_cast<LateParams *>(ka + V2_PARAMS_KERNARG_OFFSET);
    return pl.fold2_six[kk];
  };

  issue_dma(0, half);
  if (!(ablate & 16)) {
    asm volatile("s_waitcnt vmcnt(0)" ::: "memory");
    __builtin_amdgcn_s_barrier();
  }

  auto compare_loop = [&](auto half_tag) {
  constexpr bool HALF = decltype(half_tag)::value;
  int k = k_first, blk = 0;
  constexpr bool SHORT_BLOCKS = PL < V2_BB && !HALF;
  uint32_t short_w = 0;
  if constexpr (SHORT_BLOCKS) short_w = rank_short_word(k);
  uint32_t six_w = 0;
  if constexpr (SHORT_BLOCKS && FOLD2) six_w = fold2_six_word(k);
  for (int g = 0; g < total; ++g) {
    const int buf = g & 1;
    constexpr bool DMA_IN_STREAM = NW == 8 && W >= 2 && !HALF;
    if (g + 1 < total && !(ablate & 4) && !(DMA_IN_STREAM && wave_active)) issue_dma(buf ^ 1, HALF);

    if (wave_active && !(ablate & 2)) {
      const uint32_t rp =
          (uint32_t)(size_t)(__attribute__((address_space(3))) void *)(lds + buf * CHUNK_U4) + voff_ref;
      const uint32_t qp = (uint32_t)(size_t)(__attribute__((address_space(3))) void *)(
          lds + buf * CHUNK_U4 + REF_U4 + wave * 2);
#define PPK_BLOCK_OPERANDS                                                                   \
  [c0] "+{v58}"(pw[0][0][0]), [c1] "+{v56}"(pw[0][0][1]), [c2] "+{v59}"(pw[0][0][2]), [c3] "+{v57}"(pw[0][0][3]), \
      [c4] "+{v62}"(pw[0][1][0]), [c5] "+{v60}"(pw[0][1][1]), [c6] "+{v63}"(pw[0][1][2]), [c7] "+{v61}"(pw[0][1][3]), \
      [c8] "+{v66}"(pw[0][2][0]), [c9] "+{v64}"(pw[0][2][1]), [c10] "+{v67}"(pw[0][2][2]), [c11] "+{v65}"(pw[0][2][3]), \
      [c12] "+{v70}"(pw[0][3][0]), [c13] "+{v68}"(pw[0][3][1]), [c14] "+{v71}"(pw[0][3][2]), [c15] "+{v69}"(pw[0][3][3])
#define PPK_BLOCK_BY_PLANES(STMT)                     \
  if constexpr (PL == 14) { STMT() }                  \
  else if constexpr (PL == 12) { STMT(_P12) }         \
  else if constexpr (PL == 10) { STMT(_P10) }         \
  else { static_assert(PL == 14 || PL == 12 || PL == 10 || PL == 8, "plane counts with a generated stream"); STMT(_P8) }
      if constexpr (NW == 8) {
        if constexpr (HALF) {
#define PPK_HALF_STMT(SUF)                                                                                  \
  asm volatile(PPK_BLOCK_HALF_ASM_Q32##SUF : PPK_BLOCK_OPERANDS : [rp] "v"(rp), [qp] "v"(qp) \
               : "memory", PPK_BLOCK_CLOBBERS);
          if constexpr (FOLDH) {
            asm volatile(PPK_BLOCK_HALF_H4_ASM_Q32_P8 : PPK_BLOCK_OPERANDS : [rp] "v"(rp), [qp] "v"(qp)
                         : "memory", PPK_BLOCK_CLOBBERS);
          } else {
            PPK_BLOCK_BY_PLANES(PPK_HALF_STMT)
          }
#undef PPK_HALF_STMT
        } else if constexpr (DMA_IN_STREAM) {
          static_assert(NW != 8 || PW == (PL >= 12 ? 4 : 3), "DMA pieces per wavefront of the generated stream");
          static_assert(2 * PL >= NW * (PW - 1), "every piece but a wavefront's last is a ref piece");
          constexpr int LT = PW - 1;
          const uint32_t lbase =
              (uint32_t)(size_t)(__attribute__((address_space(3))) void *)(lds + (buf ^ 1) * CHUNK_U4);
          const uint32_t m00 = __builtin_amdgcn_readfirstlane(lbase + (uint32_t)doff[0] * 16u);
          const uint32_t m03 = __builtin_amdgcn_readfirstlane(lbase + (uint32_t)doff[LT] * 16u);
          constexpr bool LAST_MAY_BE_EMPTY = NW * PW > NPIECE;
          const uint64_t xb = (LAST_MAY_BE_EMPTY && dkind[LT] == 2) ? 0ull : (wave + NW * LT == NPIECE - 1) ? __ballot(qlane_ok) : ~0ull;
          const uint32_t xblo = __builtin_amdgcn_readfirstlane((uint32_t)xb),
                         xbhi = __builtin_amdgcn_readfirstlane((uint32_t)(xb >> 32));
          const uint32_t vob = dkind[LT] == 0 ? voff_ref : voff_qry;
#define PPK_DMA_SEL_STMT(SUF, SB2)                                                                                \
  asm volatile(PPK_BLOCK_DMA_SEL_ASM_Q32##SUF                                                                     \
               : PPK_BLOCK_OPERANDS                                                                               \
               : [rp] "v"(rp), [qp] "v"(qp), [m00] "s"(m00), [m03] "s"(m03), [sb0] "s"(dbase[0]),                 \
                 [sb1] "s"(dbase[1]), [sb2] "s"(dbase[SB2]), [sb3] "s"(dbase[LT]), [voa] "v"(voff_ref),           \
                 [vob] "v"(vob), [xblo] "s"(xblo), [xbhi] "s"(xbhi), [sh] "s"(short_w), [bk] "s"(blk)             \
               : "memory", "scc", PPK_BLOCK_CLOBBERS);
#define PPK_DMA_SEL3_STMT(SUF, SB2) PPK_DMA_SEL3_STMT_OF(PPK_BLOCK_DMA_SEL3_ASM_Q32##SUF, SB2)
#define PPK_DMA_SEL3_STMT_OF(STREAM, SB2)                                                                         \
  asm volatile(STREAM                                                                                             \
               : PPK_BLOCK_OPERANDS                                                                               \
               : [rp] "v"(rp), [qp] "v"(qp), [m00] "s"(m00), [m03] "s"(m03), [sb0] "s"(dbase[0]),                 \
                 [sb1] "s"(dbase[1]), [sb2] "s"(dbase[SB2]), [sb3] "s"(dbase[LT]), [voa] "v"(voff_ref),           \
                 [vob] "v"(vob), [xblo] "s"(xblo), [xbhi] "s"(xbhi), [sh] "s"(short_w), [sh2] "s"(six_w),         \
                 [bk] "s"(blk)                                                                                    \
               : "memory", "scc", PPK_BLOCK_CLOBBERS);
          if constexpr (PL < V2_BB) {
            if constexpr (PL == 12) { PPK_DMA_SEL_STMT(_P12, 2) }
            else if constexpr (PL == 10) { PPK_DMA_SEL_STMT(_P10, LT) }
            else if constexpr (FOLDH) { PPK_DMA_SEL3_STMT_OF(PPK_BLOCK_DMA_SELH_ASM_Q32_P8, LT) }
            else if constexpr (FOLD2) { PPK_DMA_SEL3_STMT(_P8, LT) }
            else { PPK_DMA_SEL_STMT(_P8, LT) }
          } else {
            asm volatile(PPK_BLOCK_DMA_ASM_Q32
                         : PPK_BLOCK_OPERANDS
                         : [rp] "v"(rp), [qp] "v"(qp), [m00] "s"(m00), [m03] "s"(m03), [sb0] "s"(dbase[0]),
                           [sb1] "s"(dbase[1]), [sb2] "s"(dbase[2]), [sb3] "s"(dbase[3]), [voa] "v"(voff_ref),
                           [vob] "v"(vob), [xblo] "s"(xblo), [xbhi] "s"(xbhi)
                         : "memory", "scc", PPK_BLOCK_CLOBBERS);
          }
#undef PPK_DMA_SEL_STMT
#undef PPK_DMA_SEL3_STMT
#undef PPK_DMA_SEL3_STMT_OF
          if (g + 2 < total) {
#pragma unroll
            for (int t = 0; t < PW; ++t) dbase[t] += dstep[t];
          }
        } else {
          static_assert(PL == V2_BB, "the unpacked modes compare raw planes");
          asm volatile(PPK_BLOCK_ASM_Q32 : PPK_BLOCK_OPERANDS : [rp] "v"(rp), [qp] "v"(qp)
                       : "memory", PPK_BLOCK_CLOBBERS);
        }
      }
#undef PPK_BLOCK_BY_PLANES
#undef PPK_BLOCK_OPERANDS

      if constexpr (KS_FUSED) {
      } else if (blk == ublocks - 1) {
        if constexpr (MODE == MODE_DIST || ppk_is_mask(MODE) || MODE == MODE_KNN) {
          bool parked = false;
          if constexpr (WIDE_TILE) {
            int kpg = p.wide_kpg;
            asm volatile("" : "+s"(kpg));
            if (k + 1 < p.nk && (k + 1) % kpg == 0) {
              wide_park((k + 1) / kpg - 1);
#pragma unroll
              for (int i = 0; i < W; ++i)
#pragma unroll
                for (int r = 0; r < R; ++r)
#pragma unroll
                  for (int q = 0; q < TQ; ++q) pw[i][r][q] = 0;
              parked = true;
            }
          }
          if (k + 1 < p.nk && !parked) {
            const int up = 32 - p.cnt_bits;
#pragma unroll
            for (int r = 0; r < R; ++r)
#pragma unroll
              for (int q = 0; q < TQ; ++q) {
#pragma unroll
                for (int i = W - 1; i > 0; --i)
                  pw[i][r][q] = __builtin_amdgcn_alignbit(pw[i][r][q], pw[i - 1][r][q], up);
                pw[0][r][q] <<= p.cnt_bits;
              }
          }
        } else {
#pragma unroll
        for (int r = 0; r < R; ++r)
#pragma unroll
          for (int q = 0; q < TQ; ++q) {
            {
              const size_t qq = qw0 + q, rf = ref_of(r);
              const bool valid = rf < p.r_limit && qq >= qb && qq < qe && (!p.self || rf > qq);
              if (valid) {
                const size_t row = (p.self ? qq * p.n_ref - (qq * (qq + 1)) / 2 + (rf - qq - 1)
                                           : qq * p.n_ref + rf) - p.row_base;
                if constexpr (MODE == MODE_COUNTS && KSPLIT) {
                  static_cast<uint32_t *>(out)[(size_t)k * p.ks_rows + row] = pw[0][r][q];
                } else if constexpr (MODE == MODE_COUNTS) {
                  static_cast<uint32_t *>(out)[row * p.nk + k] = pw[0][r][q];
                } else {
                  double jr = 0.0;
                  if (p.random_correct) {
                    const int cr = ref_clu ? ref_clu[rf] : 0;
                    const int cq = qry_clu ? qry_clu[qq] : 0;
                    jr = (double)rtab[((size_t)k * p.n_clu + cr) * p.n_clu + cq];
                  }
                  static_cast<float *>(out)[row * p.nk + k] =
                      (float)observed_excess(jaccard_obs(pw[0][r][q], p.s64, BB, p.ext_adjust), jr);
                }
              }
            }
            pw[0][r][q] = 0;
          }
        }
      }
    }
    if constexpr (!KS_FUSED) {
      if (++blk == ublocks) {
        blk = 0;
        ++k;
        if constexpr (SHORT_BLOCKS) short_w = rank_short_word(k);
        if constexpr (SHORT_BLOCKS && FOLD2) six_w = fold2_six_word(k);
      }
    }
    if (!(ablate & 8)) {
      asm volatile("s_waitcnt vmcnt(0)" ::: "memory");
      __builtin_amdgcn_s_barrier();
    }
  }
  };
  if (half)
    compare_loop(std::true_type{});
  else
    compare_loop(std::false_type{});

  if constexpr (MODE == MODE_DIST || ppk_is_mask(MODE) || MODE == MODE_KNN) {
    if (ablate & 1) return;
    if (!FOLD2 && !KS_FUSED && !WIDE_TILE && MODE != MODE_KNN && !wave_active) return;
    __builtin_amdgcn_s_setprio(3);
#pragma unroll
    for (int i = 0; i < W; ++i)
#pragma unroll
      for (int r = 0; r < R; ++r)
#pragma unroll
        for (int q = 0; q < TQ; ++q) {
          uint32_t t;
          asm volatile("v_mov_b32 %0, %1" : "=v"(t) : "v"(pw[i][r][q]));
          pw[i][r][q] = t;
        }
    {
      uint32_t t = voff_ref;
      asm volatile("" : "+v"(t));
      lane_late = (int)(t >> 4);
    }
    const char __attribute__((address_space(4))) *ka =
        (const char __attribute__((address_space(4))) *)__builtin_amdgcn_kernarg_segment_ptr();
    asm volatile("" : "+s"(ka));
    LateParams &p_late = *reinterpret_cast<LateParams *>(ka + V2_PARAMS_KERNARG_OFFSET);
    if constexpr (FOLDH) {
      static_assert(FOLD2 && PL == 8 && W == 2 && !KSPLIT && !WIDE, "the holder pair is an 8-plane whole-tile kernel");
      static_assert(sizeof(lds) >= 8 * 512 * sizeof(u32x4), "one 64-bit word per pair of the tile");
      const uint32_t tid = (uint32_t)wave * 64u + (uint32_t)lane_late;
      unsigned long long *corr = reinterpret_cast<unsigned long long *>(lds);
      u32x4 zero4;
      zero4.x = zero4.y = zero4.z = zero4.w = 0;
#pragma unroll
      for (int i = 0; i < 2 * TQ; ++i) lds[tid + 512u * i] = zero4;
      __syncthreads();
      {
        const unsigned *off = p_late.fold2_off;
        const uint32_t *ents = reinterpret_cast<const uint32_t *>(p_late.fold2_ev);
        const uint32_t frt = p_late.fold2_rt;
        const uint32_t q_sub = (uint32_t)(q0 >> 5) & 7u;
        const int n_buckets = strip ? 8 : 1;
        for (int i = 0; i < n_buckets; ++i) {
          const uint32_t b = strip ? ((uint32_t)(r0 >> 5) + (uint32_t)i) * frt + (uint32_t)(q0 >> 8)
                                   : (uint32_t)(q0 >> 5) * frt + (uint32_t)rt;
          const uint32_t e1 = off[b + 1];
          for (uint32_t e = off[b] + tid; e < e1; e += 512u) {
            const uint32_t ev = ents[e], kk = (ev >> 13) & 7u;
            uint32_t ref_l = ev & 255u, qry_l = (ev >> 8) & 31u;
// ... 732 lines not shown
```

### poppunk_amd/csrc/ppk_internal.h

```cpp
#pragma once

#include <sys/mman.h>

#include <atomic>
#include <functional>
#include <cstdlib>
#include <initializer_list>
#include <memory>
#include <thread>
#include <vector>
#include <hip/hip_runtime.h>
#include <stddef.h>
#include <stdint.h>

#include <string>

#include "../../include/ppk.h"

#define PPK_MAX_NK 128
#define PPK_LANES 64
#define PPK_NPAD 256
#define PPK_RANK_SHORT_WORDS 16
constexpr int PPK_MAX_DEVICES = 64;

#include "ppk_device.h"

enum PpkCodingKind {
  PPK_CODING_RANK = 0,
  PPK_CODING_FOLD = 1,
  PPK_CODING_FOLD2 = 2,
  PPK_CODING_FOLDH = 3,
  PPK_CODINGS = 4
};
struct PpkCoding {
  PpkCodingKind kind = PPK_CODING_RANK;
  uint64_t *d_ref = nullptr, *d_qry = nullptr;
  int planes = 0;
  int stream_planes = 0;
  unsigned holders = 0;
  unsigned less1[PPK_RANK_SHORT_WORDS] = {}, less2[PPK_RANK_SHORT_WORDS] = {};
  std::vector<unsigned> order;
  void *d_list = nullptr;
  unsigned *d_off = nullptr;
  unsigned list_elem = 0, qt = 0, rt = 0;
  size_t list_count = 0;
};
void ppk_coding_free(PpkCoding &c);

struct ppk_db {
  int device = 0;
  size_t n = 0, npad = 0, nk = 0, s64 = 0, bbits = 0, words = 0;
  uint64_t *d_skT = nullptr;
  uint16_t *d_clu = nullptr;
  PpkCoding coding[PPK_CODINGS] = {{PPK_CODING_RANK}, {PPK_CODING_FOLD}, {PPK_CODING_FOLD2}, {PPK_CODING_FOLDH}};
  std::vector<unsigned> rank_counts;
};
constexpr int RANK_BB = 14;
#define PPK_RANK_EXTRA 3
#define PPK_FOLD2_SLOTS 256
#define PPK_FOLD2_MAX_PER_PAIR 63
#define PPK_FOLDH_SLOTS 1024
#define PPK_FOLDH_LADDER 7
#define PPK_FOLDH_MAX_CODES 16
#define PPK_FOLD2_MAX_NK 5

inline bool ppk_unfused(const ppk_db *db) {
  int bits = 1;
  while (((size_t)1 << bits) <= db->s64 * 64) ++bits;
  return db->nk > PPK_MAX_NK || (db->nk * (size_t)bits > 128 && db->bbits != 14);
}

struct PpkConfig {
#ifdef PPK_EXPERIMENTS
  std::atomic<long long> ablate{0};
  std::atomic<long long> map{0};
  std::atomic<long long> strip{1};
  std::atomic<long long> edge_list_keep{1};
#endif
  std::atomic<long long> rank_planes{1};
  std::atomic<long long> rank_fold{1};
  std::atomic<long long> rank_fold2{1};
  std::atomic<long long> fold2_sort{1};
  std::atomic<long long> fold2_min_planes{6};
  std::atomic<long long> rank_foldh{1};
  std::atomic<long long> foldh_holders{0};
  std::atomic<long long> foldh_min_planes{2};
  std::atomic<long long> rank_short{1};
  std::atomic<long long> lds_table{1};
  std::atomic<long long> ksplit{1200};
  std::atomic<long long> ksplit_wide{215};
  std::atomic<long long> ksplit_long{1};
  std::atomic<long long> ksplit_fused{1};
  std::atomic<long long> wide_kpg{0};
  std::atomic<long long> ksplit_slices{0};
  std::atomic<long long> chunk_rows{8ll << 20};
  std::atomic<long long> prefault_threads{8};
  std::atomic<long long> db_cache{1};
  std::atomic<long long> progress{1};
  std::atomic<long long> host_trace{0};
  std::atomic<long long> launch_tiles{8000000};
  std::atomic<long long> knn_warm{32};
  std::atomic<long long> knn_cut{4};
  std::atomic<long long> ksplit_scratch_mb{2048};
  std::atomic<long long> ks_grid_pad{0};
  std::atomic<long long> knn_lane_lists{0};
  std::atomic<long long> sweep_window{1};
  std::atomic<long long> net_window{0};
  std::atomic<long long> bt_lds_max{0};
  std::atomic<long long> bt_small_max{64};
  std::atomic<long long> dbscan_search{0};
  std::atomic<long long> refine_local{1};
  std::atomic<long long> density_hot_table{1};
  std::atomic<long long> density_kde_presum{0};
  std::atomic<long long> pairs_scratch_mb{1024};
  std::atomic<long long> pairs_chunk{0};
  std::atomic<long long> silhouette_scratch_mb{1024};
  std::atomic<long long> silhouette_band{0};
  std::atomic<long long> silhouette_window{0};
  std::atomic<long long> rand_scratch_mb{1024};
  std::atomic<long long> rand_batch{0};
  std::atomic<long long> rand_wave_max{64};
  std::atomic<long long> rand_window{0};
  std::atomic<long long> lineage_scratch_mb{1024};
  std::atomic<long long> lineage_lds_keys{0};
  std::atomic<long long> sketch_lds_bins{0};
  std::atomic<long long> sketch_batch_mb{1024};
  std::atomic<long long> sketch_batch{0};
  std::atomic<long long> sketch_count_bits{0};
  std::atomic<long long> sketch_exact_rounds{64};
  std::atomic<long long> knn_list{0};
  std::atomic<long long> host_parts_rows{16 << 20};
  std::atomic<long long> host_parts{2};
  std::atomic<long long> ext_collision_adjust{0};
  std::atomic<long long> ext_fit_skip{0};
};
PpkConfig &ppk_config();

void ppk_set_error(const std::string &msg);
const std::string &ppk_error();
int ppk_fail(int code, const std::string &msg);

int ppk_check_device(int dev);
int ppk_check_arch(int device_id);
int ppk_check_pair(const ppk_db *ref, const ppk_db *qry, const int32_t *kmers, size_t q_begin, size_t q_end);
bool ppk_interrupted();

#define PPK_HIP(call)                                                              \
  do {                                                                             \
    hipError_t e_ = (call);                                                        \
    if (e_ != hipSuccess)                                                          \
      return ppk_fail(PPK_ERR_HIP, std::string(#call) + ": " + hipGetErrorString(e_)); \
  } while (0)

struct DeviceGuard {
  int prev = -1;
  bool ok = true;
  explicit DeviceGuard(int dev) {
    if (hipGetDevice(&prev) != hipSuccess) prev = -1;
    if (prev != dev) ok = (hipSetDevice(dev) == hipSuccess);
  }
  ~DeviceGuard() {
    if (prev >= 0) (void)hipSetDevice(prev);
  }
};

#define PPK_ENTER_DEVICE(guard, dev)                             \
  if (int rc_dev_ = ppk_check_device(dev)) return rc_dev_;       \
  DeviceGuard guard(dev);                                        \
  if (!guard.ok) return ppk_fail(PPK_ERR_HIP, "cannot select device " + std::to_string(dev))

struct PpkDeviceVisit {
  explicit PpkDeviceVisit(int d) : dev(d) {}
  void enter();
  const int dev;
  std::unique_ptr<DeviceGuard> guard;
};
void ppk_host_bufs_release(PpkDeviceVisit &visit);
void ppk_db_cache_clear();

struct PpkGeometry {
  int cus;
  unsigned xcd_shift;
  int tile_slots;
};
const PpkGeometry &ppk_geometry(int dev);
PpkGeometry ppk_measure_geometry(int dev);

enum PpkRoute {
  PPK_ROUTE_TILE = 0,
  PPK_ROUTE_KSPLIT_ONE_LAUNCH = 1,
  PPK_ROUTE_KSPLIT_TWO_PASS = 2,
// ... 374 lines not shown
```

### poppunk_amd/engine.py

```python
import ctypes as C

import numpy as np

from . import _lib

FLAG_RANDOM_CORRECT = _lib.FLAG_RANDOM_CORRECT
FLAG_JACCARD = _lib.FLAG_JACCARD
FLAG_COUNTS = _lib.FLAG_COUNTS


def _torch():
    import torch
    return torch


def _stream_ptr(device):
    torch = _torch()
    return C.c_void_p(torch.cuda.current_stream(device).cuda_stream)


def rows_in_band(n_ref, n_qry, q_begin, q_end):
    return int(_lib.lib().ppk_rows_in_band(n_ref, n_qry, q_begin, q_end))


# ... 19 lines not shown
            q = int((b - disc ** 0.5) / 2.0)
        else:
            q = int(target / float(n_ref))
        q = (q + 32) // 64 * 64
        bounds.append(max(min(q, nq), bounds[-1]))
    bounds.append(nq)
    return bounds


class SketchDB:

    def __init__(self, sketches, sketchsize64, bbits, clusters=None, device=0):
        lib = _lib.lib()
        torch = _torch()
        self.device = int(device)
        self.sketchsize64 = int(sketchsize64)
        self.bbits = int(bbits)
        self._h = C.c_void_p()
        on_dev = hasattr(sketches, "is_cuda")
        if on_dev:
            if not sketches.is_cuda or sketches.dtype != torch.int64 or not sketches.is_contiguous():
                raise ValueError("device sketches must be a contiguous int64 CUDA tensor")
            if sketches.device.index != self.device:
                raise ValueError("sketch tensor is on a different device")
            n, nk, words = sketches.shape
            src = C.c_void_p(sketches.data_ptr())
        else:
            sketches = np.ascontiguousarray(sketches, dtype=np.uint64)
            if sketches.ndim != 3:
                raise ValueError("sketches must be [n, nk, sketchsize64*bbits]")
            n, nk, words = sketches.shape
            src = C.c_void_p(sketches.ctypes.data)
        if words != self.sketchsize64 * self.bbits:
            raise ValueError("sketch word count %d != sketchsize64*bbits = %d"
                             % (words, self.sketchsize64 * self.bbits))
        self.n, self.nk = int(n), int(nk)
        clu_ptr = None
        self._clu_keep = None
        if clusters is not None:
            if on_dev:
                c = clusters.to(device="cuda:%d" % self.device, dtype=torch.int16).contiguous()
                clu_ptr = C.c_void_p(c.data_ptr())
            else:
                c = np.ascontiguousarray(clusters, dtype=np.uint16)
                if c.shape != (n,):
                    raise ValueError("clusters must be [n]")
                clu_ptr = C.c_void_p(c.ctypes.data)
            self._clu_keep = c
        with torch.cuda.device(self.device):
            rc = lib.ppk_db_create(self.device, src, n, nk, self.sketchsize64, self.bbits, clu_ptr,
                                   1 if on_dev else 0, _stream_ptr(self.device), C.byref(self._h))
            _lib.check(rc, "ppk_db_create")
            if on_dev:
                torch.cuda.current_stream(self.device).synchronize()

    def close(self):
        if getattr(self, "_h", None) is not None and self._h.value:
            _lib.lib().ppk_db_destroy(self._h)
            self._h = C.c_void_p()

    def __del__(self):
        try:
            self.close()
        except Exception:
            pass

    def __len__(self):
        return self.n

    @property
    def rank_planes(self):
        return int(_lib.lib().ppk_db_rank_planes(self._h))

    def rank_block_planes(self):
        return self._per_block("ppk_db_rank_block_planes")

    def _per_block(self, fn, per_block=1, dtype=np.uint8):
        out = np.empty((self.nk, per_block * self.sketchsize64), dtype=dtype)
        _lib.check(getattr(_lib.lib(), fn)(self._h, C.c_void_p(out.ctypes.data), out.size), fn)
        return out

    def _codes(self, fn, planes, which=None, order=None):
        npad = (self.n + 255) // 256 * 256
        raw = np.empty((self.nk, self.sketchsize64, max(planes, 1), npad), dtype=np.uint64)
        args = (C.c_void_p(raw.ctypes.data), self.nk * self.sketchsize64 * planes * npad)
        _lib.check(getattr(_lib.lib(), fn)(self._h, *(args if which is None else (int(which),) + args)), fn)
        slots = self._unslice_codes(raw, planes)
        if order is None:
            return slots
        codes = np.empty_like(slots)
        for k in range(self.nk):
            codes[:, k, order[k]] = slots[:, k]
        return codes

    def _bucketed(self, size_fn, read_fn, dtype):
        nb = C.c_size_t(0)
        count = int(getattr(_lib.lib(), size_fn)(self._h, C.byref(nb)))
        off = np.zeros(nb.value + 1, dtype=np.uint32)
        items = np.zeros(count, dtype=dtype)
        _lib.check(getattr(_lib.lib(), read_fn)(self._h, C.c_void_p(off.ctypes.data), off.size,
                                                C.c_void_p(items.ctypes.data) if count else None, count), read_fn)
        return off, items

    def _unslice_codes(self, raw, planes):
        bits = np.unpackbits(raw[..., :self.n].view(np.uint8).reshape(self.nk, self.sketchsize64, planes, self.n, 8),
                             axis=-1, bitorder="little")
        codes = np.zeros((self.nk, self.sketchsize64, self.n, 64), dtype=np.uint16)
        for b in range(planes):
            codes |= bits[:, :, b].astype(np.uint16) << b
        return np.ascontiguousarray(codes.transpose(2, 0, 1, 3)).reshape(self.n, self.nk, 64 * self.sketchsize64)

    def rank_codes(self):
        return self._codes("ppk_db_rank_read", self.rank_planes)

    @property
    def fold_planes(self):
        return int(_lib.lib().ppk_db_fold_planes(self._h))

    def fold_block_planes(self):
        return self._per_block("ppk_db_fold_block_planes")

    def fold_codes(self, which):
        return self._codes("ppk_db_fold_read", self.fold_planes, which)

    @property
    def fold2_planes(self):
        return int(_lib.lib().ppk_db_fold2_planes(self._h))

    def fold2_block_planes(self):
        return self._per_block("ppk_db_fold2_block_planes")

    def fold2_stream_planes(self):
        return self._per_block("ppk_db_fold2_stream_planes")

    def fold2_position_order(self):
        return self._per_block("ppk_db_fold2_position_order", 64, np.uint32)

    def fold2_codes(self, which):
        return self._codes("ppk_db_fold2_read", self.fold2_planes, which, self.fold2_position_order())

    def fold2_events(self):
        return self._bucketed("ppk_db_fold2_events", "ppk_db_fold2_events_read", np.uint16)

    def foldh_holders(self):
        return int(_lib.lib().ppk_db_foldh_holders(self._h))

    def foldh_stream_planes(self):
        return self._per_block("ppk_db_foldh_stream_planes")

    def foldh_position_order(self):
        return self._per_block("ppk_db_foldh_position_order", 64, np.uint32)

    def foldh_codes(self, which):
        return self._codes("ppk_db_foldh_read", 8, which, self.foldh_position_order())

    def foldh_entries(self):
        return self._bucketed("ppk_db_foldh_entries", "ppk_db_foldh_entries_read", np.uint32)

    def rank_counts(self):
        words = int(_lib.lib().ppk_db_rank_counts(self._h, None, 0))
        if not words:
            return None
        raw = np.zeros(words, dtype=np.uint32)
        _lib.lib().ppk_db_rank_counts(self._h, C.c_void_p(raw.ctypes.data), raw.size)
        seg = 1 + self.nk * self.sketchsize64
        out = {}
        for i, name in enumerate(("D", "E", "E2")):
            out[name] = int(raw[i * seg])
            out["block_" + name] = raw[i * seg + 1:(i + 1) * seg].reshape(self.nk, self.sketchsize64).copy()
        out["two_max"], out["two_total"], out["pair_cap_hit"] = (int(x) for x in raw[3 * seg:3 * seg + 3])
        return out


def _prep_tables(kmers, random_tbl, nk):
    kmers = np.ascontiguousarray(kmers, dtype=np.int32)
    if kmers.shape != (nk,):
        raise ValueError("klist length %d does not match the sketches' %d k-mer lengths"
                         % (kmers.size, nk))
    n_clu = 0
    tbl_ptr = None
    if random_tbl is not None:
        random_tbl = np.ascontiguousarray(random_tbl, dtype=np.float32)
        if random_tbl.ndim != 3 or random_tbl.shape[0] != nk or random_tbl.shape[1] != random_tbl.shape[2]:
            raise ValueError("random table must be [nk, n_clu, n_clu]")
        n_clu = random_tbl.shape[1]
        tbl_ptr = random_tbl.ctypes.data_as(C.POINTER(C.c_float))
    return kmers, random_tbl, tbl_ptr, n_clu


def _check_pair(ref, qry):
    if qry is not None and (qry.nk != ref.nk or qry.sketchsize64 != ref.sketchsize64
                            or qry.bbits != ref.bbits or qry.device != ref.device):
        raise ValueError("ref and query databases are incompatible")


def dist(ref, qry=None, kmers=None, random_tbl=None, random_correct=True, jaccard=False,
         counts=False, q_begin=0, q_end=None, out=None, n_failed=None):
    torch = _torch()
    lib = _lib.lib()
    _check_pair(ref, qry)
    nq = qry.n if qry is not None else ref.n
    q_end = nq if q_end is None else int(q_end)
    kmers, random_tbl, tbl_ptr, n_clu = _prep_tables(kmers, random_tbl, ref.nk)
    rows = rows_in_band(ref.n, qry.n if qry is not None else 0, q_begin, q_end)
    flags = (FLAG_RANDOM_CORRECT if random_correct else 0) | (FLAG_JACCARD if jaccard else 0) \
        | (FLAG_COUNTS if counts else 0)
    cols = ref.nk if (jaccard or counts) else 2
    dev = "cuda:%d" % ref.device
    with torch.cuda.device(ref.device):
        if out is None:
            out = torch.empty((rows, cols), dtype=torch.int32 if counts else torch.float32,
                              device=dev)
        elif out.numel() != rows * cols or not out.is_contiguous() or out.element_size() != 4:
            raise ValueError("out has the wrong size")
        if n_failed is None:
            n_failed = torch.zeros(1, dtype=torch.int64, device=dev)
        rc = lib.ppk_dist_dev(ref._h, qry._h if qry is not None else None,
                              kmers.ctypes.data_as(C.POINTER(C.c_int32)), tbl_ptr, n_clu, flags,
                              q_begin, q_end, C.c_void_p(out.data_ptr()),
                              C.c_void_p(n_failed.data_ptr()), _stream_ptr(ref.device))
        _lib.check(rc, "ppk_dist_dev")
    return out, n_failed


def _fused_edges(ref, qry, kmers, random_tbl, random_correct, q_begin, q_end, cap, what, launch):
    torch = _torch()
    _check_pair(ref, qry)
    nq = qry.n if qry is not None else ref.n
    q_end = nq if q_end is None else int(q_end)
    kmers, random_tbl, tbl_ptr, n_clu = _prep_tables(kmers, random_tbl, ref.nk)
    rows = rows_in_band(ref.n, qry.n if qry is not None else 0, q_begin, q_end)
    flags = FLAG_RANDOM_CORRECT if random_correct else 0
    dev = torch.device("cuda:%d" % ref.device)
    if cap is None:
        cap = min(rows, max(1 << 20, rows // 8))
    n_failed = torch.zeros(1, dtype=torch.int64, device=dev)

    def call(edges, c, n_edges):
        n_failed.zero_()
        return launch(ref._h, qry._h if qry is not None else None, kmers.ctypes.data_as(C.POINTER(C.c_int32)), tbl_ptr,
                      n_clu, flags, q_begin, q_end, C.c_void_p(edges.data_ptr()), c, C.c_void_p(n_edges.data_ptr()),
                      C.c_void_p(n_failed.data_ptr()), _stream_ptr(ref.device))
    return _edges_dev(call, what, dev, cap), n_failed


def dist_edges(ref, qry=None, kmers=None, random_tbl=None, random_correct=True, slope=2,
               x_max=0.0, y_max=0.0, scale=(1.0, 1.0), inclusive=True, q_begin=0, q_end=None,
               cap=None):
    lib = _lib.lib()
    return _fused_edges(ref, qry, kmers, random_tbl, random_correct, q_begin, q_end, cap, "ppk_dist_edges_dev",
                        lambda r, q, k, t, nc, fl, qb, qe, e, c, ne, nf, st: lib.ppk_dist_edges_dev(
                            r, q, k, t, nc, fl, qb, qe, int(slope), float(x_max), float(y_max), float(scale[0]),
                            float(scale[1]), 1 if inclusive else 0, e, c, ne, nf, st))


def _host_edges(refs, qrys, kmers, random_tbl, random_correct, cap, what, launch):
    lib = _lib.lib()
    refs = [refs] if isinstance(refs, SketchDB) else list(refs)
    if qrys is not None:
        qrys = [qrys] if isinstance(qrys, SketchDB) else list(qrys)
        if len(qrys) != len(refs):
            raise ValueError("one query database per reference database")
        for r, q in zip(refs, qrys):
            _check_pair(r, q)
    ref = refs[0]
    kmers, random_tbl, tbl_ptr, n_clu = _prep_tables(kmers, random_tbl, ref.nk)
    n_qry = qrys[0].n if qrys is not None else 0
    rows = rows_in_band(ref.n, n_qry, 0, n_qry if qrys is not None else ref.n)
    if cap is None:
        cap = min(rows, max(1 << 20, rows // 8))
    rh = (C.c_void_p * len(refs))(*[r._h.value for r in refs])
    qh = (C.c_void_p * len(refs))(*[q._h.value for q in qrys]) if qrys is not None else None
    llp = C.POINTER(C.c_longlong)
    out = np.empty((max(int(cap), 1), 2), dtype=np.int64)
    n_edges = C.c_size_t(0)
    n_failed = C.c_ulonglong(0)
    rc = launch(rh, qh, len(refs), kmers.ctypes.data_as(C.POINTER(C.c_int32)), tbl_ptr, n_clu,
                FLAG_RANDOM_CORRECT if random_correct else 0, out.ctypes.data_as(llp), int(cap), C.byref(n_edges),
                C.byref(n_failed))
    if rc == _lib.ERR_CAPACITY:
        out = np.empty((n_edges.value, 2), dtype=np.int64)
        rc = lib.ppk_parked_fetch(out.ctypes.data_as(llp), None, None, n_edges.value, None)
    _lib.check(rc, what)
    return out[:n_edges.value], int(n_failed.value)


def edges_host(refs, qrys=None, kmers=None, random_tbl=None, random_correct=True, slope=2, x_max=0.0,
               y_max=0.0, scale=(1.0, 1.0), inclusive=True, cap=None):
    lib = _lib.lib()
    return _host_edges(refs, qrys, kmers, random_tbl, random_correct, cap, "ppk_query_edges_dbs",
                       lambda rh, qh, nd, k, t, nc, fl, o, c, ne, nf: lib.ppk_query_edges_dbs(
                           rh, qh, nd, k, t, nc, fl, int(slope), float(x_max), float(y_max), float(scale[0]),
                           float(scale[1]), 1 if inclusive else 0, o, c, ne, nf))


def _check_dist_tensor(dist_t):
    torch = _torch()
    if not (dist_t.is_cuda and dist_t.dtype == torch.float32 and dist_t.is_contiguous()
            and dist_t.dim() == 2 and dist_t.shape[1] == 2):
        raise TypeError("distMat must be a C-contiguous float32 [n,2] CUDA tensor")


def bgmm_assign_dev(dist_t, model, labels=True, values=False):
    torch = _torch()
    _check_dist_tensor(dist_t)
    if not (labels or values):
        raise ValueError("ask for labels, responsibilities or both")
# ... 1927 lines not shown
```

Measured before the change: 50.61 billion.

## Shrink FOLDH streamed chunk from eight to four bit planes per block

The FOLDH coding now stores and streams four bit planes per k-mer block instead of eight. That halves the reference and query bytes moved by DMA into LDS on each chunk, and the hand-scheduled asm stream is reworked to issue two loads per wavefront instead of three. Host build, read API and Python accessor now use the chunk plane count. The risk is that the inner asm must still produce exact counts from fewer planes, and that the FOLDH path may not be the one selected for this workload.

New measurement: 57.64 billion, median of 6. 1.14x the previous value.

```diff
diff --git a/include/ppk.h b/include/ppk.h
--- a/include/ppk.h
+++ b/include/ppk.h
@@ -52,6 +52,7 @@
 int ppk_db_fold2_events_read(const ppk_db *db, uint32_t *off, size_t n_off, uint16_t *ev, size_t n_ev);
 size_t ppk_db_rank_counts(const ppk_db *db, uint32_t *out, size_t cap);
 unsigned ppk_db_foldh_holders(const ppk_db *db);
+int ppk_db_foldh_chunk_planes(const ppk_db *db);
 int ppk_db_foldh_stream_planes(const ppk_db *db, uint8_t *out, size_t cap);
 int ppk_db_foldh_position_order(const ppk_db *db, uint32_t *out, size_t cap);
 int ppk_db_foldh_read(const ppk_db *db, int which, uint64_t *out, size_t words);
diff --git a/poppunk_amd/_lib.py b/poppunk_amd/_lib.py
--- a/poppunk_amd/_lib.py
+++ b/poppunk_amd/_lib.py
@@ -166,6 +166,7 @@
     "ppk_db_fold2_events_read": (C.c_int, [_vp, _vp, _sz, _vp, _sz]),
     "ppk_db_rank_counts": (_sz, [_vp, _vp, _sz]),
     "ppk_db_foldh_holders": (C.c_uint, [_vp]),
+    "ppk_db_foldh_chunk_planes": (C.c_int, [_vp]),
     "ppk_db_foldh_stream_planes": (C.c_int, [_vp, _vp, _sz]),
     "ppk_db_foldh_position_order": (C.c_int, [_vp, _vp, _sz]),
     "ppk_db_foldh_read": (C.c_int, [_vp, C.c_int, _vp, _sz]),
diff --git a/poppunk_amd/csrc/ppk_block_asm.inc b/poppunk_amd/csrc/ppk_block_asm.inc
--- a/poppunk_amd/csrc/ppk_block_asm.inc
+++ b/poppunk_amd/csrc/ppk_block_asm.inc
@@ -5526,7 +5526,7 @@
   "v_bcnt_u32_b32 %[c15], v126, %[c15]\n" \
   ".Lppk_done_%=:\n" \
   ""
-#define PPK_BLOCK_DMA_SELH_ASM_Q32_P8 \
+#define PPK_BLOCK_DMA_SELH_ASM_Q32_P4 \
   "s_bitcmp1_b32 %[sh2], %[bk]\n" \
   "s_cbranch_scc1 .Lppk_two_%=\n" \
   "s_bitcmp1_b32 %[sh], %[bk]\n" \
@@ -5646,9 +5646,11 @@
   "v_bitop3_b32 v116, v116, v77, v85 bitop3:0x90\n" \
   "v_bitop3_b32 v119, v119, v76, v86 bitop3:0x90\n" \
   "v_bitop3_b32 v118, v118, v77, v87 bitop3:0x90\n" \
-  "s_add_u32 m0, %[m00], 8192\n" \
-  "s_nop 0\n" \
-  "global_load_lds_dwordx4 %[voa], %[sb1]\n" \
+  "s_mov_b32 m0, %[m03]\n" \
+  "s_mov_b32 exec_lo, %[xblo]\n" \
+  "s_mov_b32 exec_hi, %[xbhi]\n" \
+  "global_load_lds_dwordx4 %[vob], %[sb1]\n" \
+  "s_mov_b64 exec, -1\n" \
   "v_bitop3_b32 v121, v121, v78, v80 bitop3:0x90\n" \
   "v_bitop3_b32 v120, v120, v79, v81 bitop3:0x90\n" \
   "v_bitop3_b32 v123, v123, v78, v82 bitop3:0x90\n" \
@@ -5685,11 +5687,6 @@
   "v_bitop3_b32 v116, v116, v77, v93 bitop3:0x90\n" \
   "v_bitop3_b32 v119, v119, v76, v94 bitop3:0x90\n" \
   "v_bitop3_b32 v118, v118, v77, v95 bitop3:0x90\n" \
-  "s_mov_b32 m0, %[m03]\n" \
-  "s_mov_b32 exec_lo, %[xblo]\n" \
-  "s_mov_b32 exec_hi, %[xbhi]\n" \
-  "global_load_lds_dwordx4 %[vob], %[sb2]\n" \
-  "s_mov_b64 exec, -1\n" \
   "v_bitop3_b32 v121, v121, v78, v88 bitop3:0x90\n" \
   "v_bitop3_b32 v120, v120, v79, v89 bitop3:0x90\n" \
   "v_bitop3_b32 v123, v123, v78, v90 bitop3:0x90\n" \
@@ -5748,6 +5745,9 @@
   "v_xnor_b32 v100, v73, v85\n" \
   "v_xnor_b32 v103, v72, v86\n" \
   "v_xnor_b32 v102, v73, v87\n" \
+  "s_mov_b32 m0, %[m00]\n" \
+  "s_nop 0\n" \
+  "global_load_lds_dwordx4 %[voa], %[sb0]\n" \
   "v_xnor_b32 v105, v74, v80\n" \
   "v_xnor_b32 v104, v75, v81\n" \
   "v_xnor_b32 v107, v74, v82\n" \
@@ -5766,9 +5766,11 @@
   "v_xnor_b32 v116, v77, v85\n" \
   "v_xnor_b32 v119, v76, v86\n" \
   "v_xnor_b32 v118, v77, v87\n" \
-  "s_mov_b32 m0, %[m00]\n" \
-  "s_nop 0\n" \
-  "global_load_lds_dwordx4 %[voa], %[sb0]\n" \
+  "s_mov_b32 m0, %[m03]\n" \
+  "s_mov_b32 exec_lo, %[xblo]\n" \
+  "s_mov_b32 exec_hi, %[xbhi]\n" \
+  "global_load_lds_dwordx4 %[vob], %[sb1]\n" \
+  "s_mov_b64 exec, -1\n" \
   "v_xnor_b32 v121, v78, v80\n" \
   "v_xnor_b32 v120, v79, v81\n" \
   "v_xnor_b32 v123, v78, v82\n" \
@@ -5808,9 +5810,6 @@
   "v_bitop3_b32 v116, v116, v77, v93 bitop3:0x90\n" \
   "v_bitop3_b32 v119, v119, v76, v94 bitop3:0x90\n" \
   "v_bitop3_b32 v118, v118, v77, v95 bitop3:0x90\n" \
-  "s_add_u32 m0, %[m00], 8192\n" \
-  "s_nop 0\n" \
-  "global_load_lds_dwordx4 %[voa], %[sb1]\n" \
   "v_bitop3_b32 v121, v121, v78, v88 bitop3:0x90\n" \
   "v_bitop3_b32 v120, v120, v79, v89 bitop3:0x90\n" \
   "v_bitop3_b32 v123, v123, v78, v90 bitop3:0x90\n" \
@@ -5847,11 +5846,6 @@
   "v_bitop3_b32 v116, v116, v77, v85 bitop3:0x90\n" \
   "v_bitop3_b32 v119, v119, v76, v86 bitop3:0x90\n" \
   "v_bitop3_b32 v118, v118, v77, v87 bitop3:0x90\n" \
-  "s_mov_b32 m0, %[m03]\n" \
-  "s_mov_b32 exec_lo, %[xblo]\n" \
-  "s_mov_b32 exec_hi, %[xbhi]\n" \
-  "global_load_lds_dwordx4 %[vob], %[sb2]\n" \
-  "s_mov_b64 exec, -1\n" \
   "v_bitop3_b32 v121, v121, v78, v80 bitop3:0x90\n" \
   "v_bitop3_b32 v120, v120, v79, v81 bitop3:0x90\n" \
   "v_bitop3_b32 v123, v123, v78, v82 bitop3:0x90\n" \
@@ -5911,6 +5905,9 @@
   "v_xnor_b32 v100, v73, v85\n" \
   "v_xnor_b32 v103, v72, v86\n" \
   "v_xnor_b32 v102, v73, v87\n" \
+  "s_mov_b32 m0, %[m00]\n" \
+  "s_nop 0\n" \
+  "global_load_lds_dwordx4 %[voa], %[sb0]\n" \
   "v_xnor_b32 v105, v74, v80\n" \
   "v_xnor_b32 v104, v75, v81\n" \
   "v_xnor_b32 v107, v74, v82\n" \
@@ -5929,9 +5926,11 @@
   "v_xnor_b32 v116, v77, v85\n" \
   "v_xnor_b32 v119, v76, v86\n" \
   "v_xnor_b32 v118, v77, v87\n" \
-  "s_mov_b32 m0, %[m00]\n" \
-  "s_nop 0\n" \
-  "global_load_lds_dwordx4 %[voa], %[sb0]\n" \
+  "s_mov_b32 m0, %[m03]\n" \
+  "s_mov_b32 exec_lo, %[xblo]\n" \
+  "s_mov_b32 exec_hi, %[xbhi]\n" \
+  "global_load_lds_dwordx4 %[vob], %[sb1]\n" \
+  "s_mov_b64 exec, -1\n" \
   "v_xnor_b32 v121, v78, v80\n" \
   "v_xnor_b32 v120, v79, v81\n" \
   "v_xnor_b32 v123, v78, v82\n" \
@@ -5951,9 +5950,6 @@
   "v_bitop3_b32 v100, v100, v73, v93 bitop3:0x90\n" \
   "v_bitop3_b32 v103, v103, v72, v94 bitop3:0x90\n" \
   "v_bitop3_b32 v102, v102, v73, v95 bitop3:0x90\n" \
-  "s_add_u32 m0, %[m00], 8192\n" \
-  "s_nop 0\n" \
-  "global_load_lds_dwordx4 %[voa], %[sb1]\n" \
   "v_bitop3_b32 v105, v105, v74, v88 bitop3:0x90\n" \
   "v_bitop3_b32 v104, v104, v75, v89 bitop3:0x90\n" \
   "v_bitop3_b32 v107, v107, v74, v90 bitop3:0x90\n" \
@@ -5971,11 +5967,6 @@
   "v_bitop3_b32 v116, v116, v77, v93 bitop3:0x90\n" \
   "v_bitop3_b32 v119, v119, v76, v94 bitop3:0x90\n" \
   "v_bitop3_b32 v118, v118, v77, v95 bitop3:0x90\n" \
-  "s_mov_b32 m0, %[m03]\n" \
-  "s_mov_b32 exec_lo, %[xblo]\n" \
-  "s_mov_b32 exec_hi, %[xbhi]\n" \
-  "global_load_lds_dwordx4 %[vob], %[sb2]\n" \
-  "s_mov_b64 exec, -1\n" \
   "v_bitop3_b32 v121, v121, v78, v88 bitop3:0x90\n" \
   "v_bitop3_b32 v120, v120, v79, v89 bitop3:0x90\n" \
   "v_bitop3_b32 v123, v123, v78, v90 bitop3:0x90\n" \
@@ -6018,7 +6009,7 @@
   "v_bcnt_u32_b32 %[c15], v126, %[c15]\n" \
   ".Lppk_done_%=:\n" \
   ""
-#define PPK_BLOCK_HALF_H4_ASM_Q32_P8 \
+#define PPK_BLOCK_HALF_H4_ASM_Q32_P4 \
   "ds_read_b128 v[80:83], %[qp] offset:0\n" \
   "ds_read_b128 v[84:87], %[qp] offset:16\n" \
   "ds_read_b128 v[76:79], %[rp] offset:1024\n" \
diff --git a/poppunk_amd/csrc/ppk_coding.hip b/poppunk_amd/csrc/ppk_coding.hip
--- a/poppunk_amd/csrc/ppk_coding.hip
+++ b/poppunk_amd/csrc/ppk_coding.hip
@@ -630,7 +630,7 @@
 }
 int ppk_build_foldh(ppk_db *db, unsigned H, const unsigned *d_twice, const uint16_t *d_holders, size_t max_entries, hipStream_t s) {
   const size_t n = db->n, npad = db->npad, n_pos = db->nk * db->s64 * 64, n_kb = db->nk * db->s64;
-  const size_t copy_bytes = npad * n_kb * 8 * sizeof(uint64_t), tmp_bytes = npad * n_kb * (size_t)RANK_BB * sizeof(uint64_t);
+  const size_t copy_bytes = npad * n_kb * PPK_FOLDH_CHUNK_PLANES * sizeof(uint64_t), tmp_bytes = npad * n_kb * (size_t)RANK_BB * sizeof(uint64_t);
   const unsigned qt = (unsigned)(npad / 32), rt = (unsigned)(npad / 256);
   const size_t nb = (size_t)qt * rt, cap = max_entries ? max_entries : 1;
   size_t band_q = ((size_t)512 << 20) / (n * db->nk * 4) / 256 * 256;
@@ -670,7 +670,7 @@
   const dim3 grid_pos((unsigned)(n_kb * 8)), grid_slice((unsigned)(n_kb * 8), (unsigned)(npad / 256));
   hipLaunchKernelGGL(foldh_code_kernel, grid_pos, dim3(256), 0, s, db->d_skT, d_twice, d_holders, d_kept, d_owed, n, npad, H);
   hipLaunchKernelGGL(fold2_slice_kernel, grid_slice, dim3(256), 0, s, d_kept, d_order, reinterpret_cast<uint8_t *>(c.d_ref),
-                     reinterpret_cast<uint8_t *>(c.d_qry), n, npad, (int)db->s64, 8);
+                     reinterpret_cast<uint8_t *>(c.d_qry), n, npad, (int)db->s64, PPK_FOLDH_CHUNK_PLANES);
   hipLaunchKernelGGL(foldh_slice14_kernel, grid_slice, dim3(256), 0, s, d_owed, reinterpret_cast<uint8_t *>(d_tr),
                      reinterpret_cast<uint8_t *>(d_tq), n, npad);
   e = hipGetLastError();
@@ -992,8 +992,8 @@
 static int coding_read(const char *fn, const ppk_db *db, int kind, int which, uint64_t *out, size_t words) {
   if (int rc = coding_check(fn, db, out, kind, which)) return rc;
   const PpkCoding &c = db->coding[kind];
-  if (words != db->nk * db->s64 * (size_t)c.planes * db->npad)
-    return fail_in(fn, PPK_ERR_ARG, std::string("`words` is not nk * sketchsize64 * ") + (kind == PPK_CODING_FOLDH ? "8" : "planes") + " * padded samples");
+  if (words != db->nk * db->s64 * (size_t)c.chunk_planes() * db->npad)
+    return fail_in(fn, PPK_ERR_ARG, std::string("`words` is not nk * sketchsize64 * ") + (kind == PPK_CODING_FOLDH ? "chunk planes" : "planes") + " * padded samples");
   PPK_ENTER_DEVICE(guard, db->device);
   PPK_HIP(hipDeviceSynchronize());
   if (kind == PPK_CODING_RANK)
@@ -1073,6 +1073,7 @@
   return coding_list_read(__func__, db, PPK_CODING_FOLD2, off, n_off, ev, n_ev);
 }
 extern "C" unsigned ppk_db_foldh_holders(const ppk_db *db) { return db ? db->coding[PPK_CODING_FOLDH].holders : 0u; }
+extern "C" int ppk_db_foldh_chunk_planes(const ppk_db *db) { return db ? db->coding[PPK_CODING_FOLDH].chunk_planes() : 0; }
 extern "C" int ppk_db_foldh_read(const ppk_db *db, int which, uint64_t *out, size_t words) { return coding_read(__func__, db, PPK_CODING_FOLDH, which, out, words); }
 extern "C" int ppk_db_foldh_stream_planes(const ppk_db *db, uint8_t *out, size_t cap) { return coding_stream_planes(__func__, db, PPK_CODING_FOLDH, out, cap); }
 extern "C" int ppk_db_foldh_position_order(const ppk_db *db, uint32_t *out, size_t cap) { return coding_position_order(__func__, db, PPK_CODING_FOLDH, out, cap); }
diff --git a/poppunk_amd/csrc/ppk_dist_tile.inc b/poppunk_amd/csrc/ppk_dist_tile.inc
--- a/poppunk_amd/csrc/ppk_dist_tile.inc
+++ b/poppunk_amd/csrc/ppk_dist_tile.inc
@@ -9,13 +9,14 @@
   const int ablate = EXP ? p.ablate : 0;
   constexpr int R = V2_R, TQ = V2_TQ, BB = V2_BB;
   constexpr int V2_QT = NW * TQ;
-  constexpr int REF_U4 = PL * 128;
-  constexpr int QRY_U4 = PL * (V2_QT / 2);
+  constexpr int CPL = FOLDH ? PPK_FOLDH_CHUNK_PLANES : PL;
+  constexpr int REF_U4 = CPL * 128;
+  constexpr int QRY_U4 = CPL * (V2_QT / 2);
   constexpr int CHUNK_U4 = REF_U4 + QRY_U4;
   constexpr int LPP = V2_QT / 2;
   constexpr int PPP = 64 / LPP;
-  constexpr int NQP = (PL + PPP - 1) / PPP;
-  constexpr int NPIECE = 2 * PL + NQP;
+  constexpr int NQP = (CPL + PPP - 1) / PPP;
+  constexpr int NPIECE = 2 * CPL + NQP;
   constexpr int PW = (NPIECE + NW - 1) / NW;
   constexpr bool LDS_TABLE = NW == 8 && W == 2 && !WIDE && (MODE == MODE_DIST || ppk_is_mask(MODE) || MODE == MODE_KNN);
   constexpr int TAB_U4 = 5 * 1024;
@@ -112,16 +113,16 @@
     dbase[t] = nullptr;
     dstep[t] = 0;
     doff[t] = 0;
-    if (i < 2 * PL) {
+    if (i < 2 * CPL) {
       dkind[t] = 0;
-      dbase[t] = reinterpret_cast<const char *>(refT + ((size_t)k_first * ublocks * PL + (size_t)(i >> 1)) * p.npad_r + r0 + (i & 1) * 128);
-      dstep[t] = (size_t)PL * p.npad_r * 8;
+      dbase[t] = reinterpret_cast<const char *>(refT + ((size_t)k_first * ublocks * CPL + (size_t)(i >> 1)) * p.npad_r + r0 + (i & 1) * 128);
+      dstep[t] = (size_t)CPL * p.npad_r * 8;
       doff[t] = i * 64;
     } else if (i < NPIECE) {
-      const int j = i - 2 * PL;
+      const int j = i - 2 * CPL;
       dkind[t] = 1;
-      dbase[t] = reinterpret_cast<const char *>(qryT + ((size_t)k_first * ublocks * PL + (size_t)(PPP * j)) * p.npad_q + q0);
-      dstep[t] = (size_t)PL * p.npad_q * 8;
+      dbase[t] = reinterpret_cast<const char *>(qryT + ((size_t)k_first * ublocks * CPL + (size_t)(PPP * j)) * p.npad_q + q0);
+      dstep[t] = (size_t)CPL * p.npad_q * 8;
       doff[t] = REF_U4 + j * 64;
     } else {
       dkind[t] = 2;
@@ -129,7 +130,7 @@
   }
   const uint32_t voff_ref = lane * 16;
   const uint32_t voff_qry = (uint32_t)((lane / LPP) * p.npad_q * 8) + (lane % LPP) * 16;
-  const bool qlane_ok = (PPP * (NQP - 1) + lane / LPP) < PL;
+  const bool qlane_ok = (PPP * (NQP - 1) + lane / LPP) < CPL;
   auto issue_dma = [&](int buf, bool skip_first_half) {
     u32x4 *base = lds + buf * CHUNK_U4;
 #pragma unroll
@@ -230,15 +231,15 @@
   asm volatile(PPK_BLOCK_HALF_ASM_Q32##SUF : PPK_BLOCK_OPERANDS : [rp] "v"(rp), [qp] "v"(qp) \
                : "memory", PPK_BLOCK_CLOBBERS);
           if constexpr (FOLDH) {
-            asm volatile(PPK_BLOCK_HALF_H4_ASM_Q32_P8 : PPK_BLOCK_OPERANDS : [rp] "v"(rp), [qp] "v"(qp)
+            asm volatile(PPK_BLOCK_HALF_H4_ASM_Q32_P4 : PPK_BLOCK_OPERANDS : [rp] "v"(rp), [qp] "v"(qp)
                          : "memory", PPK_BLOCK_CLOBBERS);
           } else {
             PPK_BLOCK_BY_PLANES(PPK_HALF_STMT)
           }
 #undef PPK_HALF_STMT
         } else if constexpr (DMA_IN_STREAM) {
-          static_assert(NW != 8 || PW == (PL >= 12 ? 4 : 3), "DMA pieces per wavefront of the generated stream");
-          static_assert(2 * PL >= NW * (PW - 1), "every piece but a wavefront's last is a ref piece");
+          static_assert(NW != 8 || PW == (FOLDH ? 2 : PL >= 12 ? 4 : 3), "DMA pieces per wavefront of the generated stream");
+          static_assert(2 * CPL >= NW * (PW - 1), "every piece but a wavefront's last is a ref piece");
           constexpr int LT = PW - 1;
           const uint32_t lbase =
               (uint32_t)(size_t)(__attribute__((address_space(3))) void *)(lds + (buf ^ 1) * CHUNK_U4);
@@ -268,7 +269,7 @@
           if constexpr (PL < V2_BB) {
             if constexpr (PL == 12) { PPK_DMA_SEL_STMT(_P12, 2) }
             else if constexpr (PL == 10) { PPK_DMA_SEL_STMT(_P10, LT) }
-            else if constexpr (FOLDH) { PPK_DMA_SEL3_STMT_OF(PPK_BLOCK_DMA_SELH_ASM_Q32_P8, LT) }
+            else if constexpr (FOLDH) { PPK_DMA_SEL3_STMT_OF(PPK_BLOCK_DMA_SELH_ASM_Q32_P4, LT) }
             else if constexpr (FOLD2) { PPK_DMA_SEL3_STMT(_P8, LT) }
             else { PPK_DMA_SEL_STMT(_P8, LT) }
           } else {
diff --git a/poppunk_amd/csrc/ppk_internal.h b/poppunk_amd/csrc/ppk_internal.h
--- a/poppunk_amd/csrc/ppk_internal.h
+++ b/poppunk_amd/csrc/ppk_internal.h
@@ -32,11 +32,13 @@
   PPK_CODING_FOLDH = 3,
   PPK_CODINGS = 4
 };
+#define PPK_FOLDH_CHUNK_PLANES 4
 struct PpkCoding {
   PpkCodingKind kind = PPK_CODING_RANK;
   uint64_t *d_ref = nullptr, *d_qry = nullptr;
   int planes = 0;
   int stream_planes = 0;
+  int chunk_planes() const { return kind == PPK_CODING_FOLDH && planes ? PPK_FOLDH_CHUNK_PLANES : planes; }
   unsigned holders = 0;
   unsigned less1[PPK_RANK_SHORT_WORDS] = {}, less2[PPK_RANK_SHORT_WORDS] = {};
   std::vector<unsigned> order;
diff --git a/poppunk_amd/engine.py b/poppunk_amd/engine.py
--- a/poppunk_amd/engine.py
+++ b/poppunk_amd/engine.py
@@ -195,7 +195,8 @@
         return self._per_block("ppk_db_foldh_position_order", 64, np.uint32)
 
     def foldh_codes(self, which):
-        return self._codes("ppk_db_foldh_read", 8, which, self.foldh_position_order())
+        planes = int(_lib.lib().ppk_db_foldh_chunk_planes(self._h))
+        return self._codes("ppk_db_foldh_read", planes, which, self.foldh_position_order())
 
     def foldh_entries(self):
         return self._bucketed("ppk_db_foldh_entries", "ppk_db_foldh_entries_read", np.uint32)
```
